# ghar1821/Chronoclust

Hardware: AMD Instinct MI355X
Metric: points clustered/sec (20-dim) (higher is better)
Workload: dtype f64; 1 GPU; C2: 1 timepoint, 1000000x20 synthetic blobs (seed 42+rank), 5000 microclusters; exact sequential semantics; online + offline phases per step; one independent st; points=1000000, dim=20, microclusters=5000, clusters=5000, streams=1

## Files before the change

### chronoclust_amd/_lib.py

```python
import ctypes as C
import os

import numpy as np

from . import build as _build

PCORE, OUTLIER = 0, 1
MAX_DIM = 1024

_ERRORS = {-1: "no HIP device / HIP runtime error", -2: "bad argument", -3: "non-finite input", -4: "out of memory",
           -5: "internal error", -6: "exchange between ranks failed"}


class ChronoclustHipError(RuntimeError):
    pass


class CcParams(C.Structure):
    _fields_ = [("eps_sq", C.c_double), ("delta_sq", C.c_double), ("k", C.c_double), ("beta", C.c_double),
                ("mu", C.c_double), ("omicron", C.c_double), ("ups_eps", C.c_double), ("ups_eps_sq", C.c_double),
                ("delta", C.c_double), ("pi", C.c_int32), ("pad", C.c_int32)]


class CcTuning(C.Structure):
    _fields_ = [("window", C.c_int32), ("rounds", C.c_int32), ("segments", C.c_int32),
                ("windows_per_sync", C.c_int32), ("time_kernels", C.c_int32), ("dirty_segments", C.c_int32),
                ("early_window", C.c_int32), ("lookahead", C.c_int32), ("sequential", C.c_int32)]


class CcStats(C.Structure):
    _fields_ = [("points", C.c_int64), ("windows", C.c_int64), ("rounds", C.c_int64), ("truncated", C.c_int64),
                ("scan_launches", C.c_int64), ("scan_ms", C.c_double), ("scan_pair_dims", C.c_double),
                ("run_ms", C.c_double), ("rows", C.c_int64), ("table_rows_scanned", C.c_int64),
                ("lookahead_windows", C.c_int64), ("sharded_windows", C.c_int64), ("comm_launches", C.c_int64),
                ("comm_ms", C.c_double), ("seq_points", C.c_int64), ("scan_u_launches", C.c_int64),
                ("scan_p_launches", C.c_int64), ("pruned_scan_rows", C.c_int64), ("pruned_scan_full_rows", C.c_int64),
                ("window", C.c_int64), ("long_chains", C.c_int64), ("long_chain_launches", C.c_int64),
                ("tiles", C.c_int64), ("dirty_tiles", C.c_int64),
                ("scan_launches_pruned", C.c_int64), ("scan_ms_pruned", C.c_double), ("scan_pair_dims_pruned", C.c_double),
                ("scan_g_launches", C.c_int64), ("missed_points", C.c_int64), ("probe_launches", C.c_int64),
                ("seq_r_points", C.c_int64), ("heavy_launches", C.c_int64),
                ("scan_lean_launches", C.c_int64), ("long_prepared", C.c_int64), ("long_replayed", C.c_int64),
                ("seq_g_points", C.c_int64), ("link_launches", C.c_int64),
                ("scan_p2_launches", C.c_int64),
                ("calib_allgather_us", C.c_double), ("calib_scan_ns_per_row_dim", C.c_double),
                ("split_threshold_row_dims", C.c_int64), ("split_threshold_row_dims_pruned", C.c_int64),
                ("missed_plain_launches", C.c_int64), ("seed16_launches", C.c_int64),
                ("pad_rows_launches", C.c_int64), ("assign_points", C.c_int64), ("assign_launches", C.c_int64)]


POLICY_MAX_ROUNDS = 8


class CcPolicyConfig(C.Structure):
    _fields_ = [(k, C.c_int32) for k in ("window", "rounds_max", "windows_per_sync", "early_window", "lookahead",
                                         "allow_nodirty", "prune_mode", "prune_applicable", "can_shard", "d", "resume",
                                         "allow_sparse", "allow_guess", "allow_probe")] + \
               [("shard_min_row_dims", C.c_int64), ("n_end", C.c_int64), ("shard_min_row_dims_pruned", C.c_int64),
                ("lookahead_pruned", C.c_int32), ("force_prune_rows", C.c_int32)]


class CcPolicyCarry(C.Structure):
    _fields_ = [(k, C.c_int32) for k in ("adapt_win", "clean_batches", "since_shrink", "pad")]


class CcPolicyObs(C.Structure):
    _fields_ = [("cursor", C.c_int64), ("m_rows", C.c_int32), ("stall_b", C.c_int32)] + \
               [(k, C.c_int64) for k in ("stat_windows", "stat_truncated", "stat_trunc_unknown", "stat_tiles",
                                         "stat_dirty_tiles", "stat_unsafe", "stat_missed")] + \
               [("round_hist", C.c_int64 * (POLICY_MAX_ROUNDS + 2)), ("prune_rows", C.c_uint64), ("prune_full", C.c_uint64),
                ("after_sequential", C.c_int32), ("tg_ok", C.c_int32)]


class CcPolicyDecision(C.Structure):
    _fields_ = [(k, C.c_int32) for k in ("win_cfg", "want", "rounds", "batch_windows", "lookahead", "nodirty", "prune",
                                         "shard", "restart", "bad", "stalled", "sparse", "probe", "pad")] + \
               [(k, C.c_int64) for k in ("wins", "pts", "trunc", "unk", "tiles", "dtiles", "grew", "prune_rows", "prune_full")]


class CcSeqEvent(C.Structure):
    _fields_ = [(k, C.c_int32) for k in ("chunk_event", "bad", "possible", "more", "seq_r_applies", "use_g", "allow_seq_g", "wide")] + \
               [("got", C.c_int64), ("chunk", C.c_int64), ("rate", C.c_double), ("rate_guess", C.c_double)]


class CcBatchInputs(C.Structure):
    _fields_ = [(k, C.c_int32) for k in ("window", "win_cfg", "S_cfg", "n_cus", "prune_now", "prune_wgs_per_cu", "plain_wgs_per_cu",
                                         "decide_threads", "chain_threads", "commit_threads", "allow_claims", "allow_long",
                                         "allow_heavy", "allow_prep", "m_rows", "n_heavy", "long_seen", "long_few")] + \
               [("long_avg", C.c_int64), ("batch_windows", C.c_int32), ("pad", C.c_int32), ("points_left", C.c_int64)]


LONG_NONE, LONG_ROWS_SPLIT, LONG_ROWS_SMALL, LONG_LIST_SPLIT, LONG_LIST_SMALL = range(5)


class CcBatchGeometry(C.Structure):
    _fields_ = [(k, C.c_int32) for k in ("gw", "S", "sparse_cap", "dblocks", "cblocks", "rblocks", "scan_rows", "long_rows",
                                         "long_listed", "heavy_on", "long_cap", "windows_now", "prep", "prep_form", "long_form",
                                         "pad")]


class CcRelaxedStats(C.Structure):
    _fields_ = [("super_steps", C.c_int64), ("minibatch_points", C.c_int64), ("deferred_points", C.c_int64),
                ("reserved", C.c_int64 * 5)]


_dp = C.POINTER(C.c_double)
_i64p = C.POINTER(C.c_int64)
_i32p = C.POINTER(C.c_int32)
_i8p = C.POINTER(C.c_int8)

SYMBOLS = {
    "cc_create": (C.c_int, [C.c_int, C.POINTER(C.c_void_p)]),
    "cc_destroy": (None, [C.c_void_p]),
    "cc_last_error": (C.c_char_p, [C.c_void_p]),
    "cc_set_tuning": (C.c_int, [C.c_void_p, C.POINTER(CcTuning)]),
    "cc_reset": (C.c_int, [C.c_void_p]),
    "cc_set_params": (C.c_int, [C.c_void_p, C.POINTER(CcParams)]),
    "cc_decay_downgrade": (C.c_int, [C.c_void_p, C.c_double]),
    "cc_points_upload": (C.c_int, [C.c_void_p, _dp, C.c_int64, C.c_int32]),
    "cc_points_prefetch": (C.c_int, [C.c_void_p, _dp, C.c_int64, C.c_int32, _dp, _dp]),
    "cc_online_run": (C.c_int, [C.c_void_p]),
    "cc_col_minmax": (C.c_int, [C.c_void_p, _dp, C.c_int64, C.c_int32, _dp, _dp]),
    "cc_points_upload_scaled": (C.c_int, [C.c_void_p, _dp, C.c_int64, C.c_int32, _dp, _dp]),
    "cc_points_download": (C.c_int, [C.c_void_p, _dp, _dp, _dp]),
    "cc_labels_download": (C.c_int, [C.c_void_p, _i64p, _i8p]),
    "cc_online": (C.c_int, [C.c_void_p, _dp, C.c_int64, C.c_int32, _i64p, _i8p]),
    "cc_assign": (C.c_int, [C.c_void_p, _dp, C.c_int64, C.c_int32, _i64p, _i8p, _dp]),
    "cc_count": (C.c_int, [C.c_void_p, C.c_int]),
    "cc_dim": (C.c_int, [C.c_void_p]),
    "cc_counters": (C.c_int, [C.c_void_p, _i64p, _i64p]),
    "cc_set_counters": (C.c_int, [C.c_void_p, C.c_int64, C.c_int64]),
    "cc_export": (C.c_int, [C.c_void_p, C.c_int, _i64p, _i64p, _dp, _dp, _dp, _dp, _dp]),
    "cc_inject_mc": (C.c_int, [C.c_void_p, C.c_int, C.c_int32, _dp, _dp, _dp, _dp, C.c_double, C.c_int64,
                               C.c_int64]),
    "cc_inject_bulk": (C.c_int, [C.c_void_p, C.c_int, C.c_int32, C.c_int32, _dp, _dp, _dp, _dp, _dp, _i64p, _i64p]),
    "cc_offline": (C.c_int, [C.c_void_p, _i32p, _i8p, _i32p, _i32p, _i32p]),
    "cc_num_core": (C.c_int, [C.c_void_p]),
    "cc_cluster_size": (C.c_int, [C.c_void_p, C.c_int32]),
    "cc_cluster_export": (C.c_int, [C.c_void_p, C.c_int32, _i64p, _dp, _dp, _dp, _dp, _dp]),
    "cc_clusters_total_members": (C.c_int, [C.c_void_p]),
    "cc_clusters_export": (C.c_int, [C.c_void_p, _i64p, _i32p, _dp, _dp, _dp, _dp, _dp]),
    "cc_assoc_argmin": (C.c_int, [C.c_void_p, _dp, _dp, C.c_int32, _dp, C.c_int32, C.c_int32, _i32p, _dp]),
    "cc_get_stats": (C.c_int, [C.c_void_p, C.POINTER(CcStats)]),
    "cc_sync": (C.c_int, [C.c_void_p]),
    "cc_policy_replay": (C.c_int, [C.POINTER(CcPolicyConfig), C.POINTER(CcPolicyCarry), C.c_int64, C.c_int32,
                                   C.POINTER(CcPolicyObs), C.c_int32, C.POINTER(CcPolicyDecision)]),
    "cc_point_clusters": (C.c_int, [C.c_void_p, _i32p]),
    "cc_format_points_csv": (C.c_int64, [_dp, C.c_int64, C.c_int32, C.c_int64, _i32p, C.c_char_p, _i32p, C.c_int32,
                                         C.c_void_p, C.c_int64]),
    "cc_comm_unique_id": (C.c_int, [C.c_char_p]),
    "cc_comm_init_rccl": (C.c_int, [C.c_void_p, C.c_char_p, C.c_int, C.c_int]),
    "cc_comm_init_local": (C.c_int, [C.POINTER(C.c_void_p), C.c_int]),
    "cc_comm_calibrate": (C.c_int, [C.c_void_p]),
    "cc_comm_destroy": (C.c_int, [C.c_void_p]),
    "cc_comm_info": (C.c_int, [C.c_void_p, _i32p, _i32p, _i32p]),
    "cc_comm_set_relaxed": (C.c_int, [C.c_void_p, C.c_int32]),
    "cc_get_relaxed_stats": (C.c_int, [C.c_void_p, C.POINTER(CcRelaxedStats)]),
    "cc_policy_seq_rate_guess": (C.c_double, [C.c_int32, C.c_int32, C.c_int32, C.c_int32]),
    "cc_seq_handover_replay": (C.c_int, [C.c_int32, C.c_int32, C.c_int32, C.POINTER(CcSeqEvent), C.c_int32, _i32p, _i64p]),
    "cc_batch_plan": (C.c_int, [C.POINTER(CcBatchInputs), C.POINTER(CcBatchGeometry)]),
    "cc_scan_width": (C.c_int, [C.c_int32, C.c_int32, C.c_int32, _i32p, _i32p, _i32p]),
    "cc_shard_rows": (C.c_int, [C.c_int32, C.c_int32, C.c_int32, C.c_int32, _i32p, _i32p]),
    "cc_set_shard_thresholds": (C.c_int, [C.c_void_p, C.c_int64, C.c_int32]),
}

COMM_ID_BYTES = 128

_lib = None


def load():
    global _lib
    if _lib is None:
        path = os.environ.get("CHRONOCLUST_HIP_LIB") or _build.LIB_PATH
        if not os.path.exists(path):
            raise ChronoclustHipError(
                "HIP library %s not built; run `python -m chronoclust_amd.build` (needs hipcc). "
                "chronoclust_amd has no CPU fallback." % path)
        if _build.is_stale(path) and os.environ.get("CHRONOCLUST_HIP_ALLOW_STALE") != "1":
            raise ChronoclustHipError(
                "HIP library %s was not built from the sources beside it (csrc/ or include/chronoclust_hip.h changed since, or "
                "its .sha256 stamp is missing); run `python -m chronoclust_amd.build`." % path)
        lib = C.CDLL(path)
        for name, (res, args) in SYMBOLS.items():
            fn = getattr(lib, name)
            fn.restype = res
            fn.argtypes = args
        _lib = lib
    return _lib


HOST_ONLY_SYMBOLS = ("cc_policy_replay", "cc_policy_seq_rate_guess", "cc_seq_handover_replay", "cc_batch_plan", "cc_shard_rows",
                     "cc_format_points_csv", "cc_scan_width")


def load_host_only(path):
    global _lib
    lib = C.CDLL(path)
    for name in HOST_ONLY_SYMBOLS:
        fn = getattr(lib, name)
        fn.restype, fn.argtypes = SYMBOLS[name]
    _lib = lib
    return lib


def _f64(a):
    return np.ascontiguousarray(np.asarray(a, dtype=np.float64))


def _ptr(a, typ=_dp):
    return None if a is None else a.ctypes.data_as(typ)


def comm_unique_id():
    buf = C.create_string_buffer(COMM_ID_BYTES)
    rc = load().cc_comm_unique_id(buf)
    if rc != 0:
        raise ChronoclustHipError("cc_comm_unique_id failed (%s): is librccl available?" % _ERRORS.get(rc, rc))
    return buf.raw


def comm_init_local(handles):
    arr = (C.c_void_p * len(handles))(*[h._h for h in handles])
    rc = load().cc_comm_init_local(arr, len(handles))
    if rc != 0:
        raise ChronoclustHipError("cc_comm_init_local failed: %s" % _ERRORS.get(rc, rc))


def format_points_csv(values, first_id, label_idx, labels, threads=8, chunk=65536, out=None):
    from concurrent.futures import ThreadPoolExecutor
    lib = load()
    values = _f64(values)
    if values.ndim != 2:
        raise ValueError("values must be a [n, d] array, got shape %r" % (values.shape,))
    n, d = values.shape
    label_idx = np.ascontiguousarray(label_idx, dtype=np.int32)
    if label_idx.shape != (n,):
        raise ValueError("label_idx must hold one entry per row: shape %r for %d rows" % (label_idx.shape, n))
    if len(labels) < 1:
        raise ValueError("labels must not be empty")
    enc = [s.encode() for s in labels]
    offs = np.zeros(len(enc) + 1, np.int32)
    offs[1:] = np.cumsum([len(e) for e in enc])
    blob = b"".join(enc)
    per_row = 25 + max(len(e) for e in enc) + 33 * d + 2

    def work(a):
        b = min(n, a + chunk)
        buf = np.empty(per_row * (b - a), np.uint8)
        got = lib.cc_format_points_csv(values[a:b].ctypes.data_as(_dp), b - a, d, first_id + a,
                                       label_idx[a:b].ctypes.data_as(_i32p), blob, offs.ctypes.data_as(_i32p), len(enc),
                                       buf.ctypes.data, buf.size)
        if got < 0:
            raise ChronoclustHipError("cc_format_points_csv failed: %s" % _ERRORS.get(got, got))
        return memoryview(buf)[:got]

    if n == 0:
        return 0 if out is not None else b""
    starts = list(range(0, n, chunk))
    workers = max(1, threads)
    with ThreadPoolExecutor(max_workers=workers) as ex:
        if out is None:
            return b"".join(ex.map(work, starts))
        total, pending, nxt = 0, [], 0
        while nxt < len(starts) or pending:
            while nxt < len(starts) and len(pending) < 2 * workers:
                pending.append(ex.submit(work, starts[nxt]))
                nxt += 1
            part = pending.pop(0).result()
            out.write(part)
            total += len(part)
        return total


def policy_replay(config, carry, start, observations):
    cfg = CcPolicyConfig(**{k: int(v) for k, v in config.items()})
    car = CcPolicyCarry(int(carry[0]), int(carry[1]), int(carry[2]), 0)
    n = len(observations)
    obs = (CcPolicyObs * max(n, 1))()
    for i, o in enumerate(observations):
        for k, v in o.items():
            if k == "round_hist":
                for r, x in enumerate(v):
                    obs[i].round_hist[r] = int(x)
            else:
                setattr(obs[i], k, int(v))
    out = (CcPolicyDecision * (n + 1))()
    rc = load().cc_policy_replay(C.byref(cfg), C.byref(car), int(start[0]), int(start[1]), obs, n, out)
    if rc != 0:
        raise ValueError("cc_policy_replay: %s" % _ERRORS.get(rc, rc))
    keys = [k for k, _ in CcPolicyDecision._fields_ if k != "pad"]
    return [{k: getattr(d, k) for k in keys} for d in out], (car.adapt_win, car.clean_batches, car.since_shrink)


def seq_handover_replay(mode, possible, sticky, events):
    n = len(events)
    ev = (CcSeqEvent * max(n, 1))(*[CcSeqEvent(**e) for e in events])
    out, stint = (C.c_int32 * (n + 1))(), (C.c_int64 * (n + 1))()
    rc = load().cc_seq_handover_replay(int(mode), int(possible), int(sticky), ev, n, out, stint)
    if rc != 0:
        raise ValueError("cc_seq_handover_replay: %s" % _ERRORS.get(rc, rc))
    return list(out), list(stint)


def batch_plan(**inputs):
    out = CcBatchGeometry()
    rc = load().cc_batch_plan(C.byref(CcBatchInputs(**inputs)), C.byref(out))
    if rc != 0:
        raise ValueError("cc_batch_plan(%r): %s" % (inputs, _ERRORS.get(rc, rc)))
    return {k: getattr(out, k) for k, _ in CcBatchGeometry._fields_ if k != "pad"}


SCAN_CHAINS = ("none", "common", "general")


def scan_width(d, filter_on, k_pow2):
    padded, scan_u, chain = C.c_int32(), C.c_int32(), C.c_int32()
    rc = load().cc_scan_width(int(d), int(bool(filter_on)), int(bool(k_pow2)), C.byref(padded), C.byref(scan_u), C.byref(chain))
    if rc != 0:
        raise ValueError("cc_scan_width(%r, %r, %r): %s" % (d, filter_on, k_pow2, _ERRORS.get(rc, rc)))
    return padded.value, bool(scan_u.value), SCAN_CHAINS[chain.value]


def shard_rows(n, world, rank, unit=1):
    lo, hi = C.c_int32(), C.c_int32()
    rc = load().cc_shard_rows(int(n), int(world), int(rank), int(unit), C.byref(lo), C.byref(hi))
    if rc != 0:
        raise ValueError("cc_shard_rows(%r, %r, %r, %r): %s" % (n, world, rank, unit, _ERRORS.get(rc, rc)))
    return lo.value, hi.value


class Handle(object):

    def __init__(self, device=0):
        self._lib = load()
        h = C.c_void_p()
        rc = self._lib.cc_create(int(device), C.byref(h))
        if rc != 0:
            raise ChronoclustHipError("cc_create(device=%d) failed: %s. chronoclust_amd needs an MI355X-class HIP "
                                      "device; there is no CPU fallback." % (device, _ERRORS.get(rc, rc)))
        self._h = h
        self.device = device
        self._prefetched = None

    def close(self):
        if getattr(self, "_h", None):
            self._lib.cc_destroy(self._h)
            self._h = None

    def __del__(self):
        try:
            self.close()
        except Exception:
            pass

    def _check(self, rc):
        if rc < 0:
            msg = self._lib.cc_last_error(self._h)
            exc = ValueError if rc in (-2, -3) else ChronoclustHipError
            raise exc("%s: %s" % (_ERRORS.get(rc, rc), msg.decode() if msg else ""))
        return rc

    def set_tuning(self, window=0, rounds=0, segments=0, windows_per_sync=0, time_kernels=0, dirty_segments=0,
                   lookahead=0, early_window=0, sequential=0):
        t = CcTuning(window, rounds, segments, windows_per_sync, time_kernels, dirty_segments, int(early_window),
                     int(lookahead), int(sequential))
        self._check(self._lib.cc_set_tuning(self._h, C.byref(t)))

    def reset(self):
        self._check(self._lib.cc_reset(self._h))

    def set_params(self, eps_sq, delta_sq, k, beta, mu, omicron, ups_eps, ups_eps_sq, delta, pi):
        p = CcParams(eps_sq, delta_sq, k, beta, mu, omicron, ups_eps, ups_eps_sq, delta, int(pi), 0)
        self._check(self._lib.cc_set_params(self._h, C.byref(p)))

    def decay_downgrade(self, factor):
        self._check(self._lib.cc_decay_downgrade(self._h, float(factor)))

    def points_upload(self, x):
        x = _f64(x)
        if x.ndim != 2:
            raise ValueError("points must be a 2-d array")
        try:
            self._check(self._lib.cc_points_upload(self._h, _ptr(x), x.shape[0], x.shape[1]))
        finally:
            self._prefetched = None
        self._n = x.shape[0]

    def points_prefetch(self, x, scale=None, min_=None):
        if not (isinstance(x, np.ndarray) and x.dtype == np.float64 and x.flags["C_CONTIGUOUS"] and x.ndim == 2):
            raise ValueError("points_prefetch needs a C-contiguous float64 [n, d] array (it is not copied)")
        if x.shape[0] == 0:
            return
        scale = None if scale is None else _f64(scale)
        min_ = None if min_ is None else _f64(min_)
        self._prefetched = (x, scale, min_)
        self._check(self._lib.cc_points_prefetch(self._h, _ptr(x), x.shape[0], x.shape[1], _ptr(scale), _ptr(min_)))

    def col_minmax(self, x):
        x = _f64(x)
        mn = np.empty(x.shape[1], dtype=np.float64)
        mx = np.empty(x.shape[1], dtype=np.float64)
        self._check(self._lib.cc_col_minmax(self._h, _ptr(x), x.shape[0], x.shape[1], _ptr(mn), _ptr(mx)))
        return mn, mx

    def points_upload_scaled(self, x, scale, min_):
        x, scale, min_ = _f64(x), _f64(scale), _f64(min_)
        if x.ndim != 2 or scale.shape != (x.shape[1],) or min_.shape != (x.shape[1],):
            raise ValueError("points must be [n, d], scale and min_ [d]")
        try:
            self._check(self._lib.cc_points_upload_scaled(self._h, _ptr(x), x.shape[0], x.shape[1], _ptr(scale),
                                                          _ptr(min_)))
        finally:
            self._prefetched = None
        self._n = x.shape[0]

    def points_download(self, d, scale=None, min_=None):
        out = np.empty((self._n, d), dtype=np.float64)
        if scale is None:
            self._check(self._lib.cc_points_download(self._h, _ptr(out), None, None))
        else:
            scale, min_ = _f64(scale), _f64(min_)
            self._check(self._lib.cc_points_download(self._h, _ptr(out), _ptr(scale), _ptr(min_)))
        return out

    def online_run(self):
        self._check(self._lib.cc_online_run(self._h))

    def labels_download(self, want_path=True):
        uid = np.empty(self._n, dtype=np.int64)
        path = np.empty(self._n, dtype=np.int8) if want_path else None
        self._check(self._lib.cc_labels_download(self._h, _ptr(uid, _i64p), _ptr(path, _i8p)))
        return uid, path

    def online(self, x):
        self.points_upload(x)
        self.online_run()
        return self.labels_download()

    def assign(self, x, want_path=True, want_dist=False):
        x = _f64(x)
        if x.ndim != 2:
            raise ValueError("points must be a 2-d array")
        n = x.shape[0]
        uid = np.empty(n, dtype=np.int64)
        path = np.empty(n, dtype=np.int8) if want_path else None
        dist = np.empty(n, dtype=np.float64) if want_dist else None
        self._check(self._lib.cc_assign(self._h, _ptr(x), n, x.shape[1], _ptr(uid, _i64p), _ptr(path, _i8p), _ptr(dist)))
        return uid, path, dist

    def count(self, kind):
        return self._check(self._lib.cc_count(self._h, kind))

    def dim(self):
        return self._check(self._lib.cc_dim(self._h))

    def counters(self):
        a, b = C.c_int64(), C.c_int64()
        self._check(self._lib.cc_counters(self._h, C.byref(a), C.byref(b)))
        return a.value, b.value

    def set_counters(self, pcore_last_id, outlier_last_id):
        self._check(self._lib.cc_set_counters(self._h, int(pcore_last_id), int(outlier_last_id)))

    def export(self, kind):
        n, d = self.count(kind), self.dim()
        out = dict(id=np.empty(n, np.int64), uid=np.empty(n, np.int64), w=np.empty(n, np.float64),
                   cf1=np.empty((n, d)), cf2=np.empty((n, d)), cen=np.empty((n, d)), pref=np.empty((n, d)))
        self._check(self._lib.cc_export(self._h, kind, _ptr(out["id"], _i64p), _ptr(out["uid"], _i64p), _ptr(out["w"]),
                                        _ptr(out["cf1"]), _ptr(out["cf2"]), _ptr(out["cen"]), _ptr(out["pref"])))
        return out

    def inject(self, kind, cf1, cf2, cen, pref, w, id, uid):
        cf1, cf2, cen, pref = _f64(cf1), _f64(cf2), _f64(cen), _f64(pref)
        self._check(self._lib.cc_inject_mc(self._h, kind, len(cf1), _ptr(cf1), _ptr(cf2), _ptr(cen), _ptr(pref),
                                           float(w), int(id), int(uid)))
# ... 95 lines not shown
```

### chronoclust_amd/csrc/cc_batch.h

```cpp
#pragma once
#include <algorithm>
#include <cmath>
#include <cstdint>

#include "../../include/chronoclust_hip.h"

namespace cc {

using BatchInputs = cc_batch_inputs;
using BatchPlan = cc_batch_geometry;

constexpr int kMaxWindow = 49152;
constexpr int kLongCap = 512;

constexpr int kScanWidths[8] = {4, 8, 14, 16, 20, 32, 40, 64};
struct ScanWidth {
    int padded = 0;
    bool scan_u = false;
    int chain = CC_CHAIN_NONE;
};
inline ScanWidth scan_width(int d, bool filter, bool pow2)
{
    ScanWidth w;
    w.padded = kScanWidths[7];
    for (int i = 7; i >= 0; --i)
        if (d <= kScanWidths[i]) w.padded = kScanWidths[i];
    const bool compiled = d == w.padded, common = !filter && pow2;
    w.scan_u = common && (compiled || (d > 8 && d < w.padded));
    if (w.scan_u && w.padded > 8) w.chain = CC_CHAIN_COMMON;
    else if (!common && compiled && w.padded > 8 && w.padded <= 40) w.chain = CC_CHAIN_GENERAL;
    return w;
}

inline int scan_partials_for(int tiles, int S, int resident)
{
    int best = S;
    double best_eff = 0.0;
    for (int s = S; s >= std::max(1, S / 2); --s) {
        const double x = (double)tiles * s / (double)resident;
        const double eff = x / std::ceil(x);
        if (eff > best_eff + 1e-9) { best_eff = eff; best = s; }
    }
    return best;
}

inline BatchPlan batch_plan(const BatchInputs& in)
{
    BatchPlan p{};
    const int gw = p.gw = std::max(64, std::min(in.window, in.win_cfg));
    p.S = in.prune_now ? std::max(1, std::min(in.S_cfg, (in.n_cus * in.prune_wgs_per_cu) / std::max(1, (gw + 63) / 64)))
                       : scan_partials_for((gw + 63) / 64, in.S_cfg, in.n_cus * in.plain_wgs_per_cu);
    p.sparse_cap = std::min(kMaxWindow / 16, std::max(64, ((gw / 16 + 63) / 64) * 64));
    p.dblocks = (gw + in.decide_threads / 32 - 1) / (in.decide_threads / 32);
    p.cblocks = (gw + in.chain_threads / 32 - 1) / (in.chain_threads / 32);
    p.rblocks = std::min((gw + in.commit_threads / 32 - 1) / (in.commit_threads / 32), 1024 * (256 / in.commit_threads));
    p.scan_rows = (in.allow_claims && in.m_rows > 0 && in.m_rows <= 1024) ? in.m_rows : 0;
    p.long_rows = in.allow_long ? p.scan_rows : 0;
    p.long_listed = (in.allow_long && p.scan_rows == 0 && in.long_seen) ? 1 : 0;
    p.heavy_on = (in.allow_heavy && p.scan_rows == 0 && in.n_heavy > 0) ? 1 : 0;
    p.long_cap = in.long_few ? (int)std::min<long long>(kLongCap, 2 * in.long_avg + 8) : kLongCap;
    const long long w = std::max(1, in.win_cfg);
    p.windows_now = (int)std::max<long long>(1, std::min<long long>(in.batch_windows, (in.points_left + w - 1) / w));
    p.prep = (in.allow_prep && ((p.long_rows > 0 && p.long_rows <= 64) || (p.long_listed && in.long_few))) ? 1 : 0;
    p.prep_form = !p.prep ? CC_LONG_NONE : p.long_rows > 0 ? CC_LONG_ROWS_SPLIT : CC_LONG_LIST_SPLIT;
    p.long_form = p.long_rows > 0 ? (p.long_rows <= 256 ? CC_LONG_ROWS_SPLIT : CC_LONG_ROWS_SMALL)
                  : p.long_listed ? (in.long_few ? CC_LONG_LIST_SPLIT : CC_LONG_LIST_SMALL)
                                  : CC_LONG_NONE;
    return p;
}

struct LongChains {
    long long prev = 0;
    long long rounds_prev = 0;
    bool seen = false;
    bool few = true;
    long long avg = 1;

    void after_batch(long long stat_long, long long stat_rounds)
    {
        seen = stat_long > prev;
        avg = (stat_long - prev) / std::max<long long>(1, stat_rounds - rounds_prev) + 1;
        few = avg <= 64;
        prev = stat_long;
        rounds_prev = stat_rounds;
    }
};

inline bool link_after_batch(bool allowed, long long rows_created, long long points)
{
    return allowed && rows_created * 256 >= std::max<long long>(1, points);
}

}
```

### chronoclust_amd/csrc/cc_handle.h

```cpp
#pragma once
#include "cc_knobs.h"

namespace {

struct HipErr {
    hipError_t e;
    const char* what;
};

#define HIPCHK(call)                                  \
    do {                                              \
        hipError_t _e = (call);                       \
        if (_e != hipSuccess) throw HipErr{_e, #call}; \
    } while (0)

template <typename T>
struct DevBuf {
    T* p = nullptr;
    size_t n = 0;
    void ensure(size_t count)
    {
        if (count <= n && p) return;
        release();
        size_t want = std::max<size_t>(count, 1);
// ... 283 lines not shown
{
    f();
}
template <typename F, typename... Rest>
void with_bools(F&& f, bool b, Rest... rest)
{
    if (b) with_bools([&](auto... c) { f(std::true_type{}, c...); }, rest...);
    else with_bools([&](auto... c) { f(std::false_type{}, c...); }, rest...);
}

struct CapacityErr {
    std::string what;
};

int fail(cc_handle* h, int code, const std::string& msg)
{
    if (h) h->err = msg;
    return code;
}

void group_lost(cc_handle* h)
{
    if (h && h->comm.active()) h->comm.fail_group();
}

template <typename F>
int guarded(cc_handle* h, F&& f)
{
    try {
        if (h) HIPCHK(hipSetDevice(h->device));
        const int rc = f();
        if (rc < 0) group_lost(h);
        return rc;
    } catch (const HipErr& e) {
        char buf[512];
        snprintf(buf, sizeof buf, "HIP error %d (%s) in %s", (int)e.e, hipGetErrorString(e.e), e.what);
        group_lost(h);
        return fail(h, e.e == hipErrorOutOfMemory ? CC_ERR_OOM : CC_ERR_NO_DEVICE, buf);
    } catch (const cc::CommErr& e) {
        group_lost(h);
        return fail(h, CC_ERR_COMM, "exchange between ranks failed: " + e.what);
    } catch (const std::bad_alloc&) {
        group_lost(h);
        return fail(h, CC_ERR_OOM, "host allocation failed");
    } catch (const CapacityErr& e) {
        group_lost(h);
        return fail(h, CC_ERR_OOM, e.what);
    }
}

void sync_stream(cc_handle* h, hipStream_t st)
{
    if (h->comm.rccl() || h->comm.broken) h->comm.wait_stream(st);
    else HIPCHK(hipStreamSynchronize(st));
}

bool is_pow2(double k)
{
    if (!(k > 0.0) || !std::isfinite(k)) return false;
    int e;
    double m = std::frexp(k, &e);
    return m == 0.5 && e > -1000 && e < 1000;
}

void refresh_ctl_params(cc_handle* h)
{
    Ctl& c = h->hc;
    const cc_params& p = h->par;
    c.eps_sq = p.eps_sq;
    c.delta_sq = p.delta_sq;
    c.k = p.k;
    c.pow2 = (is_pow2(p.k) && !h->tainted) ? 1 : 0;
    c.inv_k = c.pow2 ? 1.0 / p.k : 0.0;
    c.beta_mu = p.beta * p.mu;
    c.mu = p.mu;
    c.omicron = p.omicron;
    c.pi = p.pi;
    c.filter = (h->d > 0 && p.pi < h->d) ? 1 : 0;
    c.d = h->d;
}

void push_ctl(cc_handle* h)
{
    memset(h->hc.pstat, 0, sizeof(h->hc.pstat));
    h->hc.n_missed_all[0] = h->hc.n_missed_all[1] = 0;
    HIPCHK(hipMemcpyAsync(h->ctl.p, &h->hc, sizeof(Ctl), hipMemcpyHostToDevice, h->stream));
}
void pull_ctl(cc_handle* h)
{
    HIPCHK(hipMemcpyAsync(&h->hc, h->ctl.p, sizeof(Ctl), hipMemcpyDeviceToHost, h->stream));
    sync_stream(h, h->stream);
}
void pull_ctl_pinned(cc_handle* h)
{
    if (!h->hc_pin) { pull_ctl(h); return; }
    HIPCHK(hipMemcpyAsync(h->hc_pin, h->ctl.p, sizeof(Ctl), hipMemcpyDeviceToHost, h->stream));
    sync_stream(h, h->stream);
    memcpy(&h->hc, h->hc_pin, sizeof(Ctl));
}
void push_ctl_pinned(cc_handle* h)
{
    if (!h->hc_pin) { push_ctl(h); return; }
    memset(h->hc.pstat, 0, sizeof(h->hc.pstat));
    h->hc.n_missed_all[0] = h->hc.n_missed_all[1] = 0;
    memcpy(h->hc_pin + 1, &h->hc, sizeof(Ctl));
    HIPCHK(hipMemcpyAsync(h->ctl.p, h->hc_pin + 1, sizeof(Ctl), hipMemcpyHostToDevice, h->stream));
}

#define CC_MAX_TABLE_ELEMS ((size_t)INT_MAX - 1023)

void ensure_table(cc_handle* h, size_t rows)
{
    if (h->tab.cap >= rows && h->tab.d == h->d) return;
    const size_t max_rows = CC_MAX_TABLE_ELEMS / (size_t)std::max(h->d, 1);
    if (rows > max_rows)
        throw CapacityErr{"a table of " + std::to_string(rows) + " rows of " + std::to_string(h->d) + " dimensions: more than " +
                          std::to_string(max_rows) + " rows (" + std::to_string(CC_MAX_TABLE_ELEMS) + " elements) at this width"};
    size_t want = std::min(max_rows, std::max<size_t>(rows, std::max<size_t>(1024, h->tab.cap * 2)));
    TableStore nt;
    nt.alloc(want, h->d);
    const size_t m = (size_t)h->hc.m_rows;
    TableStore& old = h->tab;
    TableStore::for_each_column(h->d, [&](auto col, size_t per_row, TableStore::Grow grow) {
        auto& to = nt.*col;
        const size_t elem = sizeof(*to.p);
        if (grow == TableStore::CLEARED || grow == TableStore::CLEARED_KEPT)
            HIPCHK(hipMemsetAsync(to.p, 0, want * per_row * elem, h->stream));
        if ((grow == TableStore::KEPT || grow == TableStore::CLEARED_KEPT) && m > 0)
            HIPCHK(hipMemcpyAsync(to.p, (old.*col).p, m * per_row * elem, hipMemcpyDeviceToDevice, h->stream));
    });
    sync_stream(h, h->stream);
    std::swap(h->tab, nt);
}

int set_dim(cc_handle* h, int d)
{
    if (d <= 0 || d > CC_MAX_DIM) return fail(h, CC_ERR_BAD_ARG, "d must be in 1.." + std::to_string(CC_MAX_DIM));
    if (h->d == 0) h->d = d;
    if (h->d != d) {
        if (h->hc.m_rows == 0) h->d = d;
        else return fail(h, CC_ERR_BAD_ARG, "dimensionality differs from the microclusters already held");
    }
    return CC_OK;
}

void ensure_window_buffers(cc_handle* h, int win, int seg)
{
    if (win <= h->win_alloc && seg <= h->seg_alloc && h->d <= h->d_alloc) return;
    win = std::max(win, h->win_alloc);
    seg = std::max(seg, h->seg_alloc);
    const size_t w = (size_t)win, d = (size_t)std::max(h->d, h->d_alloc);
    h->v_cf1.ensure(w * d); h->v_cf2.ensure(w * d); h->v_cen.ensure(w * d); h->v_pref.ensure(w * d); h->v_scl.ensure(w * d); h->v_w.ensure(w);
    h->v_kind.ensure(w); h->v_key.ensure(w); h->v_next.ensure(w); h->v_upg.ensure(w); h->v_acc.ensure(w);
    h->v_dsq.ensure(w); h->v_tau.ensure(CC_TAU_STRIDE * w); h->v_tile_dsq.ensure(CC_DSQ_STRIDE * (w / 16 + 2));
    h->v_tgt.ensure(w);
    h->v_skip.ensure(w / 64 + 2); h->v_skip_car.ensure(w / 64 + 2); h->v_unsafe.ensure(w);
    h->part_stride = w * seg * 4;
    h->spart_stride = w * seg * 2;
    h->thr_stride = w * 2;
    h->spart.ensure(2 * h->spart_stride);
    h->thr.ensure(2 * h->thr_stride);
    h->thr32.ensure(2 * h->thr_stride);
    h->cmax.ensure(2);
    h->found.ensure(2 * (CC_MAX_WINDOW / 64));
    h->missed.ensure(2 * CC_MISSED_CAP);
    h->part.ensure(2 * h->part_stride); h->dpart.ensure(w * seg * 2); h->dpart2.ensure(w * seg * 2);
    h->clean.ensure(w * 4); h->dseed.ensure(w * 4);
    h->c_cf1v.ensure(w * d); h->c_cf2v.ensure(w * d); h->c_cenv.ensure(w * d); h->c_prefv.ensure(w * d);
    h->c_sclv.ensure(w * d); h->c_wv.ensure(w); h->c_c0.ensure(w * d); h->c_w0.ensure(w * d);
    h->c_kind.ensure(w); h->c_key.ensure(w); h->c_slot.ensure(w); h->c_kind0.ensure(w); h->c_dsq.ensure(w); h->c_tile_dsq.ensure(CC_DSQ_STRIDE * (w / 16 + 2));
    h->T0.ensure(w + 128); h->T1.ensure(w + 128);
    h->long_list.ensure(2 * CC_LONG_CAP);
    h->lstat.ensure(2 * CC_LSTAT_ROWS + 2);
    h->lprev.ensure(CC_MAX_WINDOW);
    h->dpath.ensure(w); h->rk.ensure(w); h->rec.ensure(1); h->sp_list.ensure(w); h->link_near.ensure(w);
    h->win_alloc = win; h->seg_alloc = seg; h->d_alloc = (int)d;
}

Carry carry_view(cc_handle* h)
{
    return Carry{h->c_cf1v.p, h->c_cf2v.p, h->c_cenv.p, h->c_prefv.p, h->c_sclv.p, h->c_wv.p, h->c_kind.p, h->c_key.p,
                 h->c_slot.p, h->c_c0.p, h->c_w0.p, h->c_kind0.p, h->c_dsq.p, h->c_tile_dsq.p};
}

void scan_copy_sync(cc_handle* h, ScanCopy (&out)[2])
{
    const size_t cap = h->tab.cap, d = (size_t)h->d, m = (size_t)h->hc.m_rows;
    const bool filter = h->hc.filter != 0;
    const TableStore& t = h->tab;
    for (int q = 0; q < 2; ++q) {
        h->sh_cen[q].ensure(cap * d); h->sh_scl[q].ensure(cap * d); h->sh_kind[q].ensure(cap); h->sh_key[q].ensure(cap);
        if (filter) { h->sh_cf1[q].ensure(cap * d); h->sh_cf2[q].ensure(cap * d); h->sh_w[q].ensure(cap); }
        if (m > 0) {
            HIPCHK(hipMemcpyAsync(h->sh_cen[q].p, t.cen.p, m * d * 8, hipMemcpyDeviceToDevice, h->stream));
            HIPCHK(hipMemcpyAsync(h->sh_scl[q].p, t.scl.p, m * d * 8, hipMemcpyDeviceToDevice, h->stream));
            HIPCHK(hipMemcpyAsync(h->sh_kind[q].p, t.kind.p, m * 4, hipMemcpyDeviceToDevice, h->stream));
            HIPCHK(hipMemcpyAsync(h->sh_key[q].p, t.key.p, m * 4, hipMemcpyDeviceToDevice, h->stream));
            if (filter) {
                HIPCHK(hipMemcpyAsync(h->sh_cf1[q].p, t.cf1.p, m * d * 8, hipMemcpyDeviceToDevice, h->stream));
                HIPCHK(hipMemcpyAsync(h->sh_cf2[q].p, t.cf2.p, m * d * 8, hipMemcpyDeviceToDevice, h->stream));
                HIPCHK(hipMemcpyAsync(h->sh_w[q].p, t.w.p, m * 8, hipMemcpyDeviceToDevice, h->stream));
            }
        }
        out[q] = ScanCopy{h->sh_cen[q].p, h->sh_scl[q].p, h->sh_cf1[q].p, h->sh_cf2[q].p, h->sh_w[q].p, h->sh_kind[q].p,
                          h->sh_key[q].p};
    }
}

Versions versions_view(cc_handle* h)
{
    return Versions{h->v_cf1.p, h->v_cf2.p, h->v_cen.p, h->v_pref.p, h->v_scl.p, h->v_w.p, h->v_kind.p,
                    h->v_key.p, h->v_next.p, h->v_upg.p, h->v_acc.p, h->v_tgt.p, h->v_dsq.p, h->v_tile_dsq.p,
                    h->v_tau.p, h->v_skip.p, h->v_skip_car.p, h->v_unsafe.p};
}

void ensure_prefix16(cc_handle* h)
{
    const size_t a16_rows = h->tab.cap + 2 * CC_P16_TM;
    if (h->a16_stride >= a16_rows * 4) return;
    sync_stream(h, h->stream);
    sync_stream(h, h->stream2);
    h->a16.ensure(2 * a16_rows * 4);
    h->a16_stride = a16_rows * 4;
    h->hdr16.ensure(2);
}

void ensure_pad_rows(cc_handle* h, int dp)
{
    const size_t stride = (h->tab.cap + CC_SCAN_TM) * (size_t)dp;
    if (h->pad_stride >= stride) return;
    sync_stream(h, h->stream);
    sync_stream(h, h->stream2);
    h->pad_cen.ensure(2 * stride);
    h->pad_scl.ensure(2 * stride);
    h->pad_stride = stride;
}

hipEvent_t get_event(cc_handle* h, size_t i)
{
    while (h->ev_pool.size() <= i) {
        hipEvent_t e;
        HIPCHK(hipEventCreateWithFlags(&e, h->light_sync_events ? hipEventReleaseToDevice : hipEventDefault));
        h->ev_pool.push_back(e);
    }
    return h->ev_pool[i];
}

hipEvent_t get_sync_event(cc_handle* h, size_t i)
{
    if (!h->light_sync_events) return get_event(h, i);
    while (h->sync_pool.size() <= i) {
        hipEvent_t e;
        HIPCHK(hipEventCreateWithFlags(&e, hipEventDisableTiming | hipEventReleaseToDevice));
        h->sync_pool.push_back(e);
    }
    return h->sync_pool[i];
}


}
```

### chronoclust_amd/csrc/cc_host.h

```cpp
#pragma once
#include <stdint.h>

#if defined(__HIPCC__) || defined(__HIP__)
#define CC_HOSTDEV __host__ __device__
#else
#define CC_HOSTDEV
#endif

CC_HOSTDEV inline int cc_shard_share(int n, int world, int unit)
{
    const long long units = ((long long)n + unit - 1) / unit;
    const long long share = ((units + world - 1) / world) * unit;
    return (int)(share < 0x7fffffffLL ? share : 0x7fffffffLL);
}
CC_HOSTDEV inline void cc_shard_range(int n, int world, int rank, int unit, int* lo, int* hi)
{
    const int share = cc_shard_share(n, world, unit);
    const long long a = (long long)rank * share;
    *lo = (int)(a < n ? a : n);
    const long long b = a + share;
    *hi = (int)(b < n ? b : n);
}

#define CC_SEQ_DOUBLES 6600
CC_HOSTDEV inline int cc_seq_cap_rows(int d) { return CC_SEQ_DOUBLES / (4 * d + 5); }
```

### chronoclust_amd/csrc/cc_host_abi.inc

```

int cc_shard_rows(int32_t n, int32_t world, int32_t rank, int32_t unit, int32_t* lo, int32_t* hi)
{
    if (n < 0 || world < 1 || rank < 0 || rank >= world || unit < 1 || !lo || !hi) return CC_ERR_BAD_ARG;
    int a = 0, b = 0;
    cc_shard_range(n, world, rank, unit, &a, &b);
    *lo = a;
    *hi = b;
    return CC_OK;
}

int64_t cc_format_points_csv(const double* values, int64_t n, int32_t d, int64_t first_id, const int32_t* label_idx,
                             const char* label_bytes, const int32_t* label_offsets, int32_t n_labels, char* out,
                             int64_t cap)
{
    if (!values || n < 0 || d < 0 || !label_idx || !label_bytes || !label_offsets || n_labels < 1 || !out) return CC_ERR_BAD_ARG;
    char* o = out;
    char* const end = out + cap;
    int max_label = 0;
    for (int i = 0; i < n_labels; ++i) max_label = std::max(max_label, label_offsets[i + 1] - label_offsets[i]);
    const int64_t row_max = 24 + 1 + max_label + (int64_t)d * 33 + 2;
    for (int64_t r = 0; r < n; ++r) {
        if (end - o < row_max) return CC_ERR_OOM;
        o += cc::format_i64(first_id + r, o);
        *o++ = ',';
        int li = label_idx[r];
        if (li < 0 || li >= n_labels) li = n_labels - 1;
        const int ll = label_offsets[li + 1] - label_offsets[li];
        memcpy(o, label_bytes + label_offsets[li], (size_t)ll);
        o += ll;
        const double* v = values + r * d;
        for (int i = 0; i < d; ++i) {
            *o++ = ',';
            if (v[i] == v[i]) o += cc::format_repr(v[i], o);
        }
        *o++ = '\n';
    }
    return (int64_t)(o - out);
}

int cc_policy_replay(const cc_policy_config* cfg, cc_policy_carry* carry, int64_t start_cursor, int32_t start_rows,
                     const cc_policy_obs* obs, int32_t n, cc_policy_decision* out)
{
    if (!cfg || !carry || n < 0 || (n > 0 && !obs) || !out) return CC_ERR_BAD_ARG;
    cc::WindowPolicy policy(*cfg, *carry);
    out[0] = policy.start(start_cursor, start_rows);
    for (int i = 0; i < n; ++i)
        out[i + 1] = obs[i].after_sequential ? policy.after_sequential(obs[i].cursor, obs[i].m_rows) : policy.after_batch(obs[i]);
    *carry = policy.carry();
    return CC_OK;
}

double cc_policy_seq_rate_guess(int32_t d, int32_t m_rows, int32_t allow_seq_r, int32_t allow_seq_g)
{
    if (d < 1 || d > CC_MAX_DIM || m_rows < 0) return -1.0;
    const int seq_cap = d > CC_WINDOW_MAX_DIM ? 0 : cc_seq_cap_rows(d);
    return cc::seq_rate_guess(d, m_rows, seq_cap, allow_seq_r != 0, allow_seq_g != 0);
}

int cc_seq_handover_replay(int32_t mode, int32_t possible, int32_t sticky, const cc_seq_event* ev, int32_t n, int32_t* outcome,
                           int64_t* stint_len)
{
    if (mode < 0 || mode > 2 || n < 0 || (n > 0 && !ev) || !outcome || !stint_len) return CC_ERR_BAD_ARG;
    cc::SeqHandover rule;
    outcome[0] = rule.start(mode, possible != 0, sticky != 0) ? 1 : 0;
    stint_len[0] = rule.stint_len();
    for (int i = 0; i < n; ++i) {
        const cc_seq_event& e = ev[i];
        outcome[i + 1] = e.chunk_event
                             ? (int32_t)rule.after_chunk(e.got, e.rate, e.chunk, e.use_g != 0, e.allow_seq_g != 0, e.possible != 0,
                                                         e.more != 0, e.wide != 0)
                             : (rule.after_batch(e.bad != 0, e.rate, e.possible != 0, e.more != 0, e.seq_r_applies != 0, e.rate_guess) ? 1 : 0);
        stint_len[i + 1] = rule.stint_len();
    }
    return CC_OK;
}

int cc_batch_plan(const cc_batch_inputs* in, cc_batch_geometry* out)
{
    if (!in || !out) return CC_ERR_BAD_ARG;
    for (int t : {in->decide_threads, in->chain_threads, in->commit_threads})
        if (t != 64 && t != 128 && t != 256) return CC_ERR_BAD_ARG;
    if (in->window < 1 || in->win_cfg < 0 || in->S_cfg < 1 || in->n_cus < 1 || in->prune_wgs_per_cu < 1 || in->plain_wgs_per_cu < 1 ||
        in->m_rows < 0 || in->long_avg < 0 || in->points_left < 0)
        return CC_ERR_BAD_ARG;
    *out = cc::batch_plan(*in);
    return CC_OK;
}

int cc_scan_width(int32_t d, int32_t filter_on, int32_t k_pow2, int32_t* padded, int32_t* scan_u, int32_t* chain)
{
    if (d < 1 || d > CC_MAX_DIM || !padded || !scan_u || !chain) return CC_ERR_BAD_ARG;
    const cc::ScanWidth w = cc::scan_width(d, filter_on != 0, k_pow2 != 0);
    *padded = w.padded;
    *scan_u = w.scan_u ? 1 : 0;
    *chain = w.chain;
    return CC_OK;
}
```

### chronoclust_amd/csrc/cc_online_run.h

```cpp
#pragma once

namespace {

struct PolicyTrace {
    FILE* f = nullptr;
    static void obs_json(FILE* f, const cc_policy_obs& o)
    {
        fprintf(f, "{\"cursor\": %lld, \"m_rows\": %d, \"stall_b\": %d, \"stat_windows\": %lld, \"stat_truncated\": %lld, "
                   "\"stat_trunc_unknown\": %lld, \"stat_tiles\": %lld, \"stat_dirty_tiles\": %lld, \"stat_unsafe\": %lld, \"stat_missed\": %lld, \"tg_ok\": %d, \"round_hist\": [",
                (long long)o.cursor, o.m_rows, o.stall_b, (long long)o.stat_windows, (long long)o.stat_truncated,
                (long long)o.stat_trunc_unknown, (long long)o.stat_tiles, (long long)o.stat_dirty_tiles, (long long)o.stat_unsafe,
                (long long)o.stat_missed, o.tg_ok);
        for (int r = 0; r < CC_POLICY_MAX_ROUNDS + 2; ++r) fprintf(f, "%s%lld", r ? ", " : "", (long long)o.round_hist[r]);
        fprintf(f, "], \"prune_rows\": %llu, \"prune_full\": %llu, \"after_sequential\": %d}", (unsigned long long)o.prune_rows,
                (unsigned long long)o.prune_full, o.after_sequential);
    }
    static void dec_json(FILE* f, const cc_policy_decision& d)
    {
        fprintf(f, "{\"win_cfg\": %d, \"want\": %d, \"rounds\": %d, \"batch_windows\": %d, \"lookahead\": %d, \"nodirty\": %d, "
                   "\"prune\": %d, \"shard\": %d, \"restart\": %d, \"bad\": %d, \"stalled\": %d, \"sparse\": %d, \"probe\": %d}",
                d.win_cfg, d.want, d.rounds, d.batch_windows, d.lookahead, d.nodirty, d.prune, d.shard, d.restart, d.bad, d.stalled, d.sparse, d.probe);
    }
    PolicyTrace(const cc_policy_config& c, const cc_policy_carry& k, long long cursor, int rows, const cc_policy_decision& d0,
                int rank)
    {
        const char* path = getenv("CHRONOCLUST_HIP_POLICY_TRACE");
        if (!path || !path[0]) return;
        const std::string name = rank >= 0 ? std::string(path) + ".rank" + std::to_string(rank) : std::string(path);
        f = fopen(name.c_str(), "a");
        if (!f) return;
        fprintf(f, "{\"call\": {\"config\": {\"window\": %d, \"rounds_max\": %d, \"windows_per_sync\": %d, \"early_window\": %d, "
                   "\"lookahead\": %d, \"allow_nodirty\": %d, \"prune_mode\": %d, \"prune_applicable\": %d, \"can_shard\": %d, \"d\": %d, "
                   "\"resume\": %d, \"allow_sparse\": %d, \"allow_guess\": %d, \"allow_probe\": %d, \"shard_min_row_dims\": %lld, \"n_end\": %lld, \"shard_min_row_dims_pruned\": %lld, \"lookahead_pruned\": %d, \"force_prune_rows\": %d}, \"carry\": [%d, %d, %d], \"start\": [%lld, %d], \"dec\": ",
                c.window, c.rounds_max, c.windows_per_sync, c.early_window, c.lookahead, c.allow_nodirty, c.prune_mode,
                c.prune_applicable, c.can_shard, c.d, c.resume, c.allow_sparse, c.allow_guess, c.allow_probe, (long long)c.shard_min_row_dims, (long long)c.n_end, (long long)c.shard_min_row_dims_pruned, c.lookahead_pruned, c.force_prune_rows,
                k.adapt_win, k.clean_batches, k.since_shrink, cursor, rows);
        dec_json(f, d0);
        fprintf(f, "}}\n");
    }
    void batch(const cc_policy_obs& o, const cc_policy_decision& d)
    {
        if (!f) return;
        fprintf(f, "{\"obs\": ");
        obs_json(f, o);
        fprintf(f, ", \"dec\": ");
        dec_json(f, d);
        fprintf(f, "}\n");
    }
    void sequential(long long cursor, int rows, const cc_policy_decision& d)
    {
        cc_policy_obs o{};
        o.cursor = cursor;
        o.m_rows = rows;
        o.after_sequential = 1;
        batch(o, d);
    }
    ~PolicyTrace()
    {
        if (f) fclose(f);
    }
    PolicyTrace(const PolicyTrace&) = delete;
    PolicyTrace& operator=(const PolicyTrace&) = delete;
};

void launch_link_scan(cc_handle* h, hipStream_t st, int win)
{
    const dim3 grid((win + 63) / 64, (win + 4 * CC_LINK_SUB - 1) / (4 * CC_LINK_SUB)), block(256);
    const int d = h->d;
#define CC_LINK_DP(DP) hipLaunchKernelGGL((k_link_scan<DP>), grid, block, 0, st, (const Ctl*)h->ctl.p, (const double*)h->X.p, \
                                          (const double*)h->Xt.p, (const int*)h->T0.p, h->link_near.p)
    if (d <= 4) CC_LINK_DP(4);
    else if (d <= 8) CC_LINK_DP(8);
    else if (d <= 14) CC_LINK_DP(14);
    else if (d <= 16) CC_LINK_DP(16);
    else if (d <= 20) CC_LINK_DP(20);
    else if (d <= 32) CC_LINK_DP(32);
    else if (d <= 40) CC_LINK_DP(40);
    else CC_LINK_DP(64);
#undef CC_LINK_DP
}

static_assert(cc::kMaxWindow == CC_MAX_WINDOW && cc::kLongCap == CC_LONG_CAP, "cc_batch.h repeats two constants of cc_common.h");

Rows rows_of_table(const Table& t)
{
    Rows r{};
    r.cen = t.cen; r.scl = t.scl; r.pref = t.pref; r.cf1 = t.cf1; r.cf2 = t.cf2; r.w = t.w; r.kind = t.kind; r.key = t.key;
    return r;
}
Rows rows_of_versions(const Versions& v)
{
    Rows r{};
    r.cen = v.cen; r.scl = v.scl; r.pref = v.pref; r.cf1 = v.cf1; r.cf2 = v.cf2; r.w = v.w; r.kind = v.kind; r.key = v.key;
    r.next = v.next; r.tile_dsq = v.tile_dsq; r.dsq = v.dsq; r.tau = v.tau; r.skip = v.skip;
    return r;
}
Rows rows_of_carry(const Carry& c, const Versions& v, const Table& t)
{
    Rows r{};
    r.cen = c.cen; r.scl = c.scl; r.pref = c.pref; r.cf1 = c.cf1; r.cf2 = c.cf2; r.w = c.w; r.kind = c.kind; r.key = c.key;
    r.tile_dsq = c.tile_dsq; r.dsq = c.dsq; r.tau = v.tau; r.skip = v.skip_car;
    r.slot = c.slot; r.touch = t.touch; r.cap = t.cap;
    return r;
}
Rows rows_of_scan_copy(const ScanCopy& s)
{
    Rows r{};
    r.cen = s.cen; r.scl = s.scl; r.cf1 = s.cf1; r.cf2 = s.cf2; r.w = s.w; r.kind = s.kind; r.key = s.key;
    return r;
}
Rows sparse_rows(Rows r, const int* plist)
{
    r.skip = nullptr;
    r.plist = plist;
    return r;
}

void reset_call_counters(Ctl& c)
{
    c.last_round = 0;
    c.fc[0] = 0;
    for (int i = 1; i < CC_MAX_ROUNDS + 2; ++i) c.fc[i] = CC_IDX_INF;
    c.stat_windows = c.stat_rounds = c.stat_truncated = 0;
    c.stat_lookahead = 0;
    c.stat_tiles = c.stat_dirty_tiles = 0;
    c.stat_unprovable = c.stat_unsafe = 0;
    c.stat_long = 0;
    for (int i = 0; i < CC_MAX_ROUNDS + 2; ++i) c.n_long[i] = 0;
    c.stat_trunc_unknown = 0;
    c.stat_table_rows = 0;
    c.stat_seq_points = 0;
    c.stat_seq_r_points = 0;
#ifdef CC_LONG_TIMERS
    for (int i = 0; i < 8; ++i) c.dbg_long[i] = 0;
#endif
#ifdef CC_ROUND_DEBUG
    for (int i = 0; i < CC_MAX_ROUNDS + 2; ++i)
        for (int q = 0; q < 6; ++q) c.dbg_round[i][q] = 0;
#endif
    c.n_heavy = c.n_heavy_new = 0;
    c.stat_seq_clk = c.stat_seq_wall = 0;
    c.stat_prune_rows = c.stat_prune_full = 0;
    c.stat_missed = 0;
    c.seed_at = -1;
    for (int q = 0; q < 2; ++q) {
        c.n_missed[q] = 0;
        for (int K = 0; K < 2; ++K) { c.tg[q][K] = 0.0; c.tg_ok[q][K] = 0; }
    }
    c.cen_absmax = 0ull;
    c.stat_pair_rows = 0.0;
    for (int i = 0; i < CC_MAX_ROUNDS + 2; ++i) c.round_hist[i] = 0;
}

struct OnlineRun {
    cc_handle* const h;
    const long long range_a, N;
    const bool no_create, resume;
    Ctl& c;

    int win = 0, R = 0;
    int S_cfg = 1, Sd_full = 1, Sd = 1;
    int world = 1, myrank = 0;
    bool grouped = false;
    size_t batch_max = 2;
    bool timing = false;
    int seq_cap = 0;
    Versions ver{};
    Carry car{};
    hipStream_t sA = nullptr, sB = nullptr;
    static constexpr size_t ev_base = 4;

    std::optional<cc::WindowPolicy> policy;
    std::optional<PolicyTrace> ptrace;
    cc_policy_decision dec{};
    bool nodirty = false;
    bool sparse_now = false;
    bool la_on = false;
    bool shard_on = false;
    bool link_now = false;
    int Rcur = 1;
    int batch_windows = 2;

    long long done = 0;
    int m_known = 0;
    unsigned long long seq_host = 0;
    long long cursor_prev = 0;
    double batch_t0 = 0.0;

    hipEvent_t ev0 = nullptr, ev1 = nullptr, evCommit = nullptr, evScan = nullptr;
    size_t ev_used = 2, ev_sync = ev_base;
    std::vector<std::pair<size_t, double>> timed;
    std::vector<size_t> timed_comm;
    double pair_rows_eff = 0.0, pair_rows_prev = 0.0;
    double pair_rows_pruned = 0.0;
    long long sharded_windows = 0;

    cc::SeqHandover seq;
    cc::LongChains longs;
    long long long_launches = 0;

    cc::BatchPlan bp{};
    Table tab{};
    Rows trows{}, vrows{}, crows{}, vrows_sp{}, crows_sp{}, srows[2] = {};
    ScanCopy scopy[2] = {};
    int* long_list = nullptr;
    int probe_left = 0;
    hipEvent_t scan_end = nullptr;

    OnlineRun(cc_handle* handle, long long a, long long e, bool no_create_, bool resume_)
        : h(handle), range_a(a), N(e), no_create(no_create_), resume(resume_), c(handle->hc) {}

    static double now_ms()
    {
        return std::chrono::duration<double, std::milli>(std::chrono::steady_clock::now().time_since_epoch()).count();
    }
    bool seq_r_applies() const { return h->allow_seq_r && h->d >= 2 && h->d <= 4; }
    bool wide() const { return h->d > CC_WINDOW_MAX_DIM; }
    size_t window_rows() const { return wide() ? 0 : (size_t)win * batch_max; }
    bool seq_g_applies() const { return h->allow_seq_g && h->hc.m_rows >= seq_cap; }
    double seq_rate_guess() const { return cc::seq_rate_guess(h->d, h->hc.m_rows, seq_cap, h->allow_seq_r, h->allow_seq_g); }
    bool seq_possible() const { return !h->comm.active() && !no_create && (h->hc.m_rows < seq_cap || h->allow_seq_g); }

    void set_lookahead(bool on)
    {
        la_on = on;
        c.la_on = on ? 1 : 0;
        c.stall_b = 0;
        c.mode = 0;
        c.car_n = 0;
        const int q = (int)((c.window_seq + 1ull) & 1ull);
        const long long c1 = c.cursor + c.win_b;
        const long long left1 = c.n_points - c1;
        c.la_cursor[q] = c1;
        c.la_b[q] = (on && left1 > 0) ? (int)std::min<long long>(left1, c.win_cfg) : 0;
        c.la_rows[q] = c.m_rows;
// ... 161 lines not shown
        in.prune_now = h->prune_now ? 1 : 0;
        in.decide_threads = h->decide_threads; in.chain_threads = h->chain_threads; in.commit_threads = h->commit_threads;
        in.allow_claims = h->allow_claims ? 1 : 0; in.allow_long = h->allow_long ? 1 : 0;
        in.allow_heavy = h->allow_heavy ? 1 : 0; in.allow_prep = h->allow_prep ? 1 : 0;
        in.m_rows = h->hc.m_rows; in.n_heavy = h->hc.n_heavy;
        in.long_seen = longs.seen ? 1 : 0; in.long_few = longs.few ? 1 : 0; in.long_avg = longs.avg;
        return in;
    }


    int* claims_of(int round) const { return (round & 1) ? h->T1.p : h->T0.p; }
    const ScanCopy& sc_now() const { return scopy[seq_host & 1ull]; }
    int quiet_ok() const { return h->allow_quiet ? 1 : 0; }
    bool sparse_round() const { return nodirty && sparse_now; }

    void exchange_missed(hipStream_t st, const Rows& rws, int mode, int round, int q, int srank, int sworld)
    {
        launch_scan<false>(h, st, bp.gw, rws, nullptr, h->part.p, bp.S, round, mode, srank, sworld, 1);
        Cand* const send2 = h->gsend2.p + (size_t)q * CC_MISSED_CAP * 4;
        Cand* const recv2 = h->gpart2.p + (size_t)q * sworld * CC_MISSED_CAP * 4;
        hipLaunchKernelGGL(k_merge_partials, dim3((CC_MISSED_CAP + 255) / 256), dim3(256), 0, st, h->ctl.p,
                           h->part.p, h->part_stride, bp.S, send2, (size_t)0, round, mode,
                           (const unsigned long long*)nullptr, 0, (const int*)h->missed.p);
        h->comm.all_gather(send2, recv2, (size_t)CC_MISSED_CAP * 4 * sizeof(Cand), st, st == h->stream2 ? 1 : 0);
        hipLaunchKernelGGL(k_scatter_missed, dim3((CC_MISSED_CAP * sworld + 255) / 256), dim3(256), 0, st,
                           (const Ctl*)h->ctl.p, (const int*)h->missed.p, (const Cand*)recv2, sworld,
                           h->gpart.p, h->gpart_stride, (size_t)bp.gw * 4 + 4, round, mode);
    }

    void snapshot_scan(hipStream_t st, int mode, int round)
    {
        const int gw = bp.gw, S = bp.S;
        const int q = (mode == 1) ? (round & 1) : (int)(seq_host & 1ull);
        const Rows& src = (mode == 1) ? srows[round & 1] : trows;
        const Rows rws = h->scan_plan.pad_rows ? padded_rows(h, st, src, q, round, mode) : src;
        h->probe_now = probe_left > 0 && !h->prune_now;
        if (h->probe_now) --probe_left;
        const int srank = shard_on ? myrank : 0, sworld = shard_on ? world : 1;
        h->group_guess_now = shard_on && (sworld > 1 || h->group_guess_always);
        scan_end = nullptr;
        if (timing) {
            hipEvent_t a = get_event(h, ev_used), b = get_event(h, ev_used + 1);
            HIPCHK(hipEventRecord(a, st));
            launch_scan<false>(h, st, gw, rws, nullptr, h->part.p, S, round, mode, srank, sworld);
            HIPCHK(hipEventRecord(b, st));
            timed.push_back({ev_used, h->prune_now ? 1.0 : 0.0});
            ev_used += 2;
            if (!shard_on) scan_end = b;
        } else {
            launch_scan<false>(h, st, gw, rws, nullptr, h->part.p, S, round, mode, srank, sworld);
        }
        if (!shard_on) return;
        if (timing) HIPCHK(hipEventRecord(get_event(h, ev_used), st));
        hipLaunchKernelGGL(k_merge_partials, dim3((gw + 255) / 256), dim3(256), 0, st, h->ctl.p, h->part.p,
                           h->part_stride, S, h->gsend.p, h->gsend_stride, round, mode,
                           (const unsigned long long*)h->pstat_p(), gw * 4,
                           (const int*)nullptr);
        h->comm.all_gather(h->gsend.p + (size_t)q * h->gsend_stride, h->gpart.p + (size_t)q * h->gpart_stride,
                           ((size_t)gw * 4 + 4) * sizeof(Cand), st, st == h->stream2 ? 1 : 0);
        if (h->prune_now && h->guess_now && h->group_guess_now && h->lean_now) ++h->stats.scan_lean_launches;
        if (h->prune_now && h->guess_now && h->group_guess_now && !h->lean_now) exchange_missed(st, rws, mode, round, q, srank, sworld);
        if (timing) {
            HIPCHK(hipEventRecord(get_event(h, ev_used + 1), st));
            timed_comm.push_back(ev_used);
            ev_used += 2;
        }
    }

    void launch_snapshot_scans(bool first_window)
    {
        if (!la_on) return snapshot_scan(sA, 0, 0);
        if (evScan) HIPCHK(hipStreamWaitEvent(sA, evScan, 0));
        HIPCHK(hipStreamWaitEvent(sB, evCommit, 0));
        snapshot_scan(sB, 1, (int)((seq_host + 1ull) & 1ull));
        if (scan_end) evScan = scan_end;
        else {
            evScan = get_sync_event(h, ev_sync++);
            HIPCHK(hipEventRecord(evScan, sB));
        }
        if (first_window && h->hc.mode == 0) snapshot_scan(sA, 0, 0);
    }

    void launch_decide(int round)
    {
        const bool first = round == 0;
        const Cand* const dec_part = shard_on ? h->gpart.p : h->part.p;
        const size_t dec_stride = shard_on ? h->gpart_stride : h->part_stride;
        const int dec_S = shard_on ? world : bp.S, dec_inner = shard_on ? 1 : bp.S;
        const size_t dec_outer = shard_on ? (size_t)bp.gw * 4 + 4 : 0;
        const int dec_tail = (first && shard_on) ? bp.gw * 4 : -1;
        const int ac_blocks = (first && la_on) ? bp.rblocks : 0;
        const int dirty_mode = (first || !nodirty) ? 0 : (sparse_round() ? 2 : 1);
        const int group = (h->d <= 32 && h->decide_group == 16) ? 16 : 32;
        const int per_wg = h->decide_threads / group;
        const dim3 grid((bp.gw + per_wg - 1) / per_wg + ac_blocks);
        hipLaunchKernelGGL(group == 16 ? k_decide<16> : k_decide<32>, grid, dim3(h->decide_threads), 0, sA, h->ctl.p, h->X.p, tab, ver, car,
                           dec_part, dec_stride, h->clean.p, h->dpart.p, h->dpart2.p, h->dseed.p,
                           first ? (const int*)nullptr : (const int*)claims_of(round - 1), claims_of(round), h->dpath.p, dec_S, Sd,
                           round, dirty_mode, bp.scan_rows, dec_inner, dec_outer,
                           first ? (const CommitRec*)h->rec.p : (const CommitRec*)nullptr, first ? sc_now() : ScanCopy{}, ac_blocks,
                           long_list, bp.long_cap, dec_tail, (!first && round == Rcur) ? 1 : 0, bp.heavy_on ? 1 : 0,
                           first ? 0 : quiet_ok(), (first && link_now) ? h->link_near.p : (int*)nullptr);
    }

    void launch_link()
    {
        launch_link_scan(h, sA, bp.gw);
        hipLaunchKernelGGL(k_link_apply, dim3((bp.gw + 255) / 256), dim3(256), 0, sA, h->ctl.p, tab, h->T0.p,
                           (const int*)h->link_near.p, h->dpath.p);
        ++h->stats.link_launches;
    }

    void launch_claims(int round)
    {
        if (bp.scan_rows > 0)
            hipLaunchKernelGGL(k_claims, dim3(bp.scan_rows), dim3(256), 0, sA, h->ctl.p, tab, (const int*)claims_of(round), round,
                               bp.scan_rows, round ? quiet_ok() : 0);
    }
    void launch_claims_heavy(int round)
    {
        if (!bp.heavy_on) return;
        ++h->stats.heavy_launches;
        hipLaunchKernelGGL(k_claims_heavy, dim3(CC_HEAVY_CAP), dim3(256), 0, sA, h->ctl.p, tab, (const int*)claims_of(round), round,
                           long_list, bp.long_cap, round ? quiet_ok() : 0);
    }

    void launch_chain_long(int form, bool prep_kernel, int round)
    {
        if (form == CC_LONG_NONE) return;
        const bool by_list = form == CC_LONG_LIST_SPLIT || form == CC_LONG_LIST_SMALL;
        const bool split = form == CC_LONG_ROWS_SPLIT || form == CC_LONG_LIST_SPLIT;
        if (prep_kernel) h->prep_launched = true;
        else if (by_list) ++long_launches;
        auto launch = [&](auto kernel) {
            hipLaunchKernelGGL(kernel, dim3(by_list ? bp.long_cap : bp.long_rows), dim3(split ? CC_LONG_THREADS : 256), 0, sA, h->ctl.p,
                               h->X.p, tab, ver, car, (const int*)claims_of(round - 1), round, by_list ? 0 : bp.long_rows,
                               by_list ? (const int*)long_list : (const int*)nullptr, bp.prep ? h->lstat.p : nullptr,
                               bp.prep ? h->lprev.p : nullptr);
        };
        if (prep_kernel) launch(k_chain_long<true, true>);
        else if (split) launch(k_chain_long<true, false>);
        else launch(k_chain_long<false, false>);
    }

    void launch_chain(int round)
    {
        hipLaunchKernelGGL(k_chain, dim3(bp.cblocks), dim3(h->chain_threads), 0, sA, h->ctl.p, h->X.p, tab, ver, car,
                           (const int*)claims_of(round - 1), round, bp.long_rows, (const unsigned long long*)(bp.prep ? h->lprev.p : nullptr),
                           bp.prep ? h->lstat.p : nullptr);
    }

    void launch_dseed(int round)
    {
        hipLaunchKernelGGL(k_dseed, dim3((bp.gw + 63) / 64), dim3(64), 0, sA, h->ctl.p, h->X.p, tab, ver, car,
                           h->clean.p, h->dseed.p, (const int*)claims_of(round - 1), round, (const int8_t*)h->dpath.p, h->sp_list.p,
                           sparse_round() ? bp.sparse_cap : 0);
    }

    void launch_dirty_scans(int round)
    {
        if (nodirty && !sparse_round()) return;
        const bool sp = nodirty;
        const int pts = sp ? bp.sparse_cap : bp.gw;
        launch_scan<true>(h, sA, pts, sp ? vrows_sp : vrows, h->dseed.p, h->dpart.p, Sd, round, 0);
        if (la_on) launch_scan<true>(h, sA, pts, sp ? crows_sp : crows, h->dseed.p, h->dpart2.p, Sd, round, 1);
    }

    void launch_commit()
    {
        hipLaunchKernelGGL(k_commit_a, dim3(1), dim3(1024), 0, sA, h->ctl.p, tab, ver, car, h->T0.p, h->T1.p,
                           h->rk.p, h->rec.p, (const Cand*)h->clean.p, (const int8_t*)h->dpath.p);
        hipLaunchKernelGGL(k_commit_b, dim3(bp.rblocks), dim3(h->commit_threads), 0, sA, h->rec.p, tab, ver, car, h->rk.p, h->dpath.p,
                           h->lab_uid.p, h->lab_path.p, h->d, sc_now(), h->hc.filter);
    }

    void enqueue_batch()
    {
        batch_t0 = now_ms();
        bp = cc::batch_plan(batch_inputs());
        trows = rows_of_table(tab);
        vrows = rows_of_versions(ver);
        crows = rows_of_carry(car, ver, tab);
        vrows_sp = sparse_rows(vrows, h->sp_list.p);
        crows_sp = sparse_rows(crows, h->sp_list.p);
        long_list = bp.long_listed ? h->long_list.p : nullptr;
        ev_sync = ev_base;
        scopy[0] = scopy[1] = ScanCopy{};
        if (la_on) scan_copy_sync(h, scopy);
        for (int q = 0; q < 2; ++q) srows[q] = rows_of_scan_copy(scopy[q]);
        evScan = nullptr;
        if (la_on) HIPCHK(hipEventRecord(evCommit, sA));
        probe_left = (dec.probe != 0) ? 1 : 0;
        for (int wv = 0; wv < bp.windows_now; ++wv, ++seq_host) {
            launch_snapshot_scans(wv == 0);
            launch_decide(0);
            if (link_now) launch_link();
            launch_claims(0);
            launch_claims_heavy(0);
            for (int r = 1; r <= Rcur; ++r) {
                if (bp.prep) launch_chain_long(bp.prep_form, true, r);
                launch_chain(r);
                launch_chain_long(bp.long_form, false, r);
                launch_dseed(r);
                launch_dirty_scans(r);
                launch_decide(r);
                if (r < Rcur) {
                    launch_claims(r);
                    launch_claims_heavy(r);
                }
            }
            launch_commit();
            if (la_on) {
                evCommit = get_sync_event(h, ev_sync++);
                HIPCHK(hipEventRecord(evCommit, sA));
            }
        }
    }

    int after_batch()
    {
        HIPCHK(hipGetLastError());
        pull_ctl_pinned(h);
        if (la_on) sync_stream(h, sB);
        seq_host = h->hc.window_seq;
        done = h->hc.cursor;
        const double dt = now_ms() - batch_t0;
        const long long pts_b = h->hc.cursor - cursor_prev;
        link_now = cc::link_after_batch(h->allow_link && !no_create, h->hc.m_rows - m_known, pts_b);
        m_known = h->hc.m_rows;
        cursor_prev = h->hc.cursor;
        longs.after_batch(h->hc.stat_long, h->hc.stat_rounds);
        const bool shard_was = shard_on;
        cc_policy_obs o{};
        o.cursor = h->hc.cursor;
        o.m_rows = h->hc.m_rows;
        o.stall_b = h->hc.stall_b;
        o.stat_windows = h->hc.stat_windows;
        o.stat_truncated = h->hc.stat_truncated;
        o.stat_trunc_unknown = h->hc.stat_trunc_unknown;
        o.stat_tiles = h->hc.stat_tiles;
        o.stat_dirty_tiles = h->hc.stat_dirty_tiles;
        o.stat_unsafe = h->hc.stat_unsafe;
        o.stat_missed = h->hc.stat_missed;
        o.tg_ok = (h->hc.tg_ok[0][0] != 0 && h->hc.tg_ok[1][0] != 0) ? 1 : 0;
        for (int r = 0; r < CC_MAX_ROUNDS + 2; ++r) o.round_hist[r] = h->hc.round_hist[r];
        o.prune_rows = h->hc.stat_prune_rows;
        o.prune_full = h->hc.stat_prune_full;
        dec = policy->after_batch(o);
        ptrace->batch(o, dec);
        const cc_policy_carry& k = policy->carry();
        h->adapt_win = k.adapt_win; h->clean_batches = k.clean_batches; h->since_shrink = k.since_shrink;
        if (dec.stalled)
            return fail(h, CC_ERR_INTERNAL, "the online phase made no progress in five consecutive batches of windows");
        if (h->trace && dec.prune_rows > 0)
            fprintf(stderr, "[cc] pruned scans of the batch%s (sample): %lld (wave, row) pairs, %.1f %% evaluated in full; points missed by guessed thresholds so far: %lld\n",
                    h->guess_now ? ", guessed thresholds" : "", (long long)dec.prune_rows,
                    100.0 * (double)dec.prune_full / (double)dec.prune_rows, (long long)h->hc.stat_missed);
        pair_rows_eff += (h->hc.stat_pair_rows - pair_rows_prev) / (shard_was ? (double)world : 1.0);
        if (h->prune_now) pair_rows_pruned += (h->hc.stat_pair_rows - pair_rows_prev) / (shard_was ? (double)world : 1.0);
        pair_rows_prev = h->hc.stat_pair_rows;
        if (shard_was) sharded_windows += dec.wins;
        Rcur = dec.rounds;
        Sd = Sd_full;
        nodirty = dec.nodirty != 0;
        sparse_now = dec.sparse != 0;
        shard_on = dec.shard != 0;
        h->set_prune(dec.prune);
        if (dec.restart) {
            h->hc.win_cfg = dec.win_cfg;
            h->hc.win_b = (int)std::min<long long>(dec.win_cfg, N - done);
            set_lookahead(dec.lookahead != 0);
            push_ctl_pinned(h);
        }
#ifdef CC_ROUND_DEBUG
        for (int r = 1; r <= CC_MAX_ROUNDS; ++r)
            if (h->hc.dbg_round[r][5] != 0)
                fprintf(stderr, "[cc]    round %d so far: %llu decisions, %llu refused, create->join new %llu, create->join row %llu, join->create %llu, other MC %llu | windows ended in round %d: %lld\n",
                        r, h->hc.dbg_round[r][5], h->hc.dbg_round[r][0], h->hc.dbg_round[r][1], h->hc.dbg_round[r][2], h->hc.dbg_round[r][3],
                        h->hc.dbg_round[r][4], r, (long long)h->hc.round_hist[r]);
#endif
        if (h->trace)
            fprintf(stderr, "[cc] %.2f ms done %lld rows %d | batch: %lld windows %lld points trunc %lld (%lld at an undecidable point) lookahead %lld dirty tiles %lld / %lld (points so far: %lld unlocated, %lld unsafe) | next window %d rounds %d\n",
                    now_ms() - batch_t0, done, h->hc.m_rows, (long long)dec.wins, (long long)dec.pts, (long long)dec.trunc, (long long)dec.unk, (long long)h->hc.stat_lookahead, (long long)dec.dtiles, (long long)dec.tiles,
                    (long long)h->hc.stat_unprovable, (long long)h->hc.stat_unsafe, dec.want, Rcur);
        batch_windows = dec.batch_windows;
        seq.after_batch(dec.bad != 0, pts_b > 0 ? (double)pts_b / std::max(dt, 1e-3) : 0.0, seq_possible(), done < N, seq_r_applies(),
                        seq_rate_guess());
        return (int)CC_OK;
    }

    void finish()
    {
        HIPCHK(hipEventRecord(ev1, h->stream));
        HIPCHK(hipEventSynchronize(ev1));
        float ms = 0.f;
        HIPCHK(hipEventElapsedTime(&ms, ev0, ev1));
        h->stats.run_ms += ms;
        h->stats.points += N - range_a;
        h->stats.windows += h->hc.stat_windows;
        h->stats.rounds += h->hc.stat_rounds;
        h->stats.truncated += h->hc.stat_truncated;
        h->stats.rows = h->hc.m_rows;
        h->stats.scan_pair_dims += pair_rows_eff * (double)h->d;
        h->stats.scan_pair_dims_pruned += pair_rows_pruned * (double)h->d;
        h->stats.sharded_windows += sharded_windows;
        h->stats.seq_points += h->hc.stat_seq_points;
        h->stats.seq_r_points += h->hc.stat_seq_r_points;
// ... 82 lines not shown
```

### chronoclust_amd/csrc/cc_validate.h

```cpp
#pragma once


#define CC_LSTAT_ROWS 1024

template <int GW = 32>
__device__ __forceinline__ unsigned cc_group_ballot(bool p)
{
    static_assert(GW == 16 || GW == 32, "groups of 16 or 32 lanes");
    const unsigned long long b = __builtin_amdgcn_ballot_w64(p);
    return (unsigned)(b >> (threadIdx.x & (64 - GW))) & (GW == 32 ? 0xFFFFFFFFu : 0xFFFFu);
}

template <int CTRL>
__device__ __forceinline__ double cc_dpp_f64(double x)
{
    int lo = __double2loint(x), hi = __double2hiint(x);
    lo = __builtin_amdgcn_update_dpp(0, lo, CTRL, 0xF, 0xF, false);
    hi = __builtin_amdgcn_update_dpp(0, hi, CTRL, 0xF, 0xF, false);
    return __hiloint2double(hi, lo);
}
__device__ __forceinline__ double cc_group_sum_any_order(double x)
{
    x += cc_dpp_f64<0xB1>(x);
    x += cc_dpp_f64<0x4E>(x);
    x += cc_dpp_f64<0x141>(x);
    x += cc_dpp_f64<0x140>(x);
    const int lo = __double2loint(x), hi = __double2hiint(x);
    const double r16 = __hiloint2double(__builtin_amdgcn_readlane(hi, 16), __builtin_amdgcn_readlane(lo, 16));
    const double r48 = __hiloint2double(__builtin_amdgcn_readlane(hi, 48), __builtin_amdgcn_readlane(lo, 48));
    return x + ((threadIdx.x & 32) ? r48 : r16);
}

struct GroupAdd {
    double c1[2], c2[2], pr[2];
    double cen[2];
    double r2;
    int gt1, ne1;
};

template <int GW = 32>
__device__ inline GroupAdd cc_group_add_regs(const double (&b1)[2], const double (&b2)[2], double bw,
                                             const double (&px)[2], int d, const Par& c)
{
    const int gl = threadIdx.x & (GW - 1);
    GroupAdd g;
    const double w1 = bw + 1.0;
    double term[2];
    bool gt[2], ne[2];
#pragma unroll
    for (int h = 0; h < 2; ++h) {
        const int i = gl + GW * h;
        g.c1[h] = 0.0; g.c2[h] = 0.0; g.pr[h] = 1.0; g.cen[h] = 0.0;
        term[h] = 0.0; gt[h] = false; ne[h] = false;
        if (i < d) {
            const double x = px[h];
            g.c1[h] = b1[h] + x;
            g.c2[h] = b2[h] + x * x;
            const double qa = g.c2[h] / w1;
            const double qb = g.c1[h] / w1;
            g.cen[h] = qb;
            const double var = qa - qb * qb;
            const double pr = (var <= c.delta_sq) ? c.k : 1.0;
            g.pr[h] = pr;
            term[h] = cc_div_pref(var, pr, c);
            gt[h] = pr > 1.0;
            ne[h] = pr != 1.0;
        }
    }
    g.gt1 = __builtin_popcount(cc_group_ballot<GW>(gt[0])) + __builtin_popcount(cc_group_ballot<GW>(gt[1]));
    g.ne1 = __builtin_popcount(cc_group_ballot<GW>(ne[0])) + __builtin_popcount(cc_group_ballot<GW>(ne[1]));
    __shared__ double s_term[(CC_GROUP_THREADS / GW)][2 * GW];
    double* const row = s_term[(threadIdx.x / GW) % (CC_GROUP_THREADS / GW)];
    CC_WAVE_SYNC();
    row[gl] = term[0];
    row[gl + GW] = term[1];
    CC_WAVE_SYNC();
    double r2 = 0.0;
    const int d8 = (d + 7) & ~7;
    for (int i = 0; i < d8; ++i) r2 = r2 + row[i];
    g.r2 = r2;
    return g;
}

template <int GW = 32>
__device__ inline GroupAdd cc_group_add(const double* bcf1, const double* bcf2, double bw, const double* p, int d,
                                        const Par& c)
{
    const int gl = threadIdx.x & (GW - 1);
    double b1[2] = {0.0, 0.0}, b2[2] = {0.0, 0.0}, px[2] = {0.0, 0.0};
#pragma unroll
    for (int h = 0; h < 2; ++h) {
        const int i = gl + GW * h;
        if (i < d) {
            px[h] = p[i];
            if (bcf1) { b1[h] = bcf1[i]; b2[h] = bcf2[i]; }
        }
    }
    return cc_group_add_regs<GW>(b1, b2, bw, px, d, c);
}

template <int CTRL>
__device__ __forceinline__ Cand cc_dpp_cand(const Cand& c)
{
    Cand o;
    o.dist = cc_dpp_f64<CTRL>(c.dist);
    o.key = __builtin_amdgcn_update_dpp(0, c.key, CTRL, 0xF, 0xF, false);
    o.slot = __builtin_amdgcn_update_dpp(0, c.slot, CTRL, 0xF, 0xF, false);
    return o;
}
template <typename F>
__device__ __forceinline__ void cc_row16_exchanges(F&& f)
{
    f(std::integral_constant<int, 0xB1>{});
    f(std::integral_constant<int, 0x4E>{});
    f(std::integral_constant<int, 0x141>{});
    f(std::integral_constant<int, 0x140>{});
}


__device__ __forceinline__ void cc_dsq_window_max(const unsigned long long* __restrict__ tile_dsq, int n,
                                                  unsigned long long (&m)[3])
{
    static_assert(CC_DSQ_STRIDE == 4, "a record is two 16-byte loads");
    constexpr int AHEAD = 8;
    const ulonglong2* const rec = reinterpret_cast<const ulonglong2*>(tile_dsq);
    for (int i0 = threadIdx.x; i0 < n; i0 += 64 * AHEAD) {
        ulonglong2 a[AHEAD], b[AHEAD];
#pragma unroll
        for (int q = 0; q < AHEAD; ++q) {
            const int i = min(i0 + 64 * q, n - 1);
            a[q] = rec[(size_t)i * 2];
            b[q] = rec[(size_t)i * 2 + 1];
        }
#pragma unroll
        for (int q = 0; q < AHEAD; ++q) {
            m[0] = a[q].x > m[0] ? a[q].x : m[0];
            m[1] = a[q].y > m[1] ? a[q].y : m[1];
            m[2] = b[q].x > m[2] ? b[q].x : m[2];
        }
    }
}

__global__ __launch_bounds__(64) void k_dseed(Ctl* __restrict__ ctl, const double* __restrict__ X, Table tab,
                                              Versions ver, Carry car, const Cand* __restrict__ clean,
                                              Cand* __restrict__ seed, const int* __restrict__ T, int round,
                                              const int8_t* __restrict__ dpath, int* __restrict__ sparse_list, int sparse_cap)
{
    CC_LATENCY_KERNEL();
    const int B = ctl->win_b;
    if (B == 0) return;
    if (ctl->fc[round - 1] >= B) return;
    const int j = blockIdx.x * blockDim.x + threadIdx.x;
    if (blockIdx.x * blockDim.x >= B) return;
    const bool la_mode = ctl->mode != 0;
    unsigned long long maxd[3] = {0ull, 0ull, 0ull}, maxd_car[3] = {0ull, 0ull, 0ull};
    {
        cc_dsq_window_max(ver.tile_dsq, (B + 15) / 16, maxd);
        if (la_mode) cc_dsq_window_max(car.tile_dsq, (ctl->car_n + 15) / 16, maxd_car);
#pragma unroll
        for (int K = 0; K < 3; ++K)
            for (int off = 32; off >= 1; off >>= 1) {
                const unsigned long long o = __shfl_xor(maxd[K], off), oc = __shfl_xor(maxd_car[K], off);
                maxd[K] = o > maxd[K] ? o : maxd[K];
                maxd_car[K] = oc > maxd_car[K] ? oc : maxd_car[K];
            }
    }
    bool flag_unprov = false, flag_unsafe = false, flag_n1skip = false;
    bool repeats = false;
    int flag_word = 0;
    double tau_w[3] = {CC_INF, CC_INF, CC_INF};
    bool need_ver = false, need_car = false;
    if (j < B) {
    const Par par = cc_load_par(ctl);
    const int d = par.d;
    const bool filter = par.filter != 0;
    const unsigned long long stamp = ctl->window_seq * 16ull + (unsigned long long)round;
    const double* p = X + (ctl->cursor + j) * d;
    Cand first0 = Cand{CC_INF, CC_IDX_INF, -1}, first1 = Cand{CC_INF, CC_IDX_INF, -1};
    double cap[2] = {CC_INF, CC_INF};
    bool lk_ok[2] = {par.k > 0.0, par.k > 0.0}, lbound[2] = {false, false};
    const double K = 1.0;

    const unsigned long long wseq = ctl->window_seq;
    Cand cq[4];
#pragma unroll
    for (int q = 0; q < 4; ++q) cq[q] = clean[(size_t)j * 4 + q];
    double d2v[2] = {CC_INF, CC_INF};
    bool have1[2];
    bool look[4];
#pragma unroll
    for (int kd = 0; kd < 2; ++kd) {
        if (cq[kd * 2 + 1].slot != -1) d2v[kd] = cq[kd * 2 + 1].dist;
        have1[kd] = cq[kd * 2].slot >= 0;
        lbound[kd] = cq[kd * 2].slot == CC_SLOT_BOUND;
        if (lbound[kd]) d2v[kd] = cq[kd * 2].dist;
        look[kd * 2] = have1[kd];
        look[kd * 2 + 1] = have1[kd] && cq[kd * 2 + 1].slot >= 0;
    }
    unsigned long long tcq[4], cwq[4], coq[4];
#pragma unroll
    for (int q = 0; q < 4; ++q) {
        const size_t sl = (size_t)(look[q] ? cq[q].slot : 0);
        tcq[q] = look[q] ? tab.touch[(size_t)(round & 1) * tab.cap + sl] : 0ull;
        cwq[q] = look[q] ? tab.cnt[sl] : 0ull;
        coq[q] = (look[q] && la_mode) ? tab.carry_of[sl] : 0ull;
    }
    int lv[4], n_memb[4];
    bool walk[4];
    int max_list = 0;
#pragma unroll
    for (int q = 0; q < 4; ++q) {
        const int head = 0xFFFFF - (int)(tcq[q] & 0xFFFFFull);
        lv[q] = -1;
        walk[q] = false;
        n_memb[q] = 0;
        if (!look[q]) continue;
        if ((tcq[q] >> 20) != stamp || head >= j) {
            if (la_mode && (coq[q] >> 20) == wseq) lv[q] = CC_CAR_BASE + (int)(coq[q] & 0xFFFFFull);
        } else {
            lv[q] = head;
            walk[q] = true;
            n_memb[q] = ((cwq[q] >> 24) == stamp) ? (int)(cwq[q] & 0xFFFFFFull) : 0;
            const int n_list = n_memb[q] < CC_CHAIN_MEMB ? n_memb[q] : CC_CHAIN_MEMB;
            max_list = n_list > max_list ? n_list : max_list;
        }
    }
    for (int pos = 0; pos * 4 < max_list; ++pos) {
        int4 mm[4];
#pragma unroll
        for (int q = 0; q < 4; ++q) {
            const bool on = walk[q] && pos * 4 < n_memb[q];
            mm[q] = on ? reinterpret_cast<const int4*>(tab.memb + (size_t)cq[q].slot * CC_CHAIN_MEMB)[pos] : make_int4(0, 0, 0, 0);
        }
#pragma unroll
        for (int q = 0; q < 4; ++q) {
            const int n_list = n_memb[q] < CC_CHAIN_MEMB ? n_memb[q] : CC_CHAIN_MEMB;
            const int e[4] = {mm[q].x, mm[q].y, mm[q].z, mm[q].w};
#pragma unroll
            for (int c = 0; c < 4; ++c) {
                const int m = e[c];
                if (walk[q] && pos * 4 + c < n_list && m < j && m > lv[q]) lv[q] = m;
            }
        }
    }
#pragma unroll
    for (int q = 0; q < 4; ++q)
        if (walk[q] && n_memb[q] > CC_CHAIN_MEMB) {
            const int clen = tab.clen[cq[q].slot];
            const int n = clen > CC_CHAIN_MEMB ? clen : CC_CHAIN_MEMB + 1;
            const int gap = B / n;
            const bool scan_first = (n - CC_CHAIN_MEMB) > gap / 8;
            int v = lv[q];
            int res = -2;
            for (int attempt = 0; attempt < 2 && res == -2; ++attempt) {
                if ((attempt == 0) == scan_first) {
                    const int want = cq[q].slot;
                    const int budget = min(16384, 16 * gap + 64);
                    for (int hi = j - 1, scanned = 0; res == -2 && scanned < budget; hi -= 32, scanned += 32) {
                        int tv[32];
#pragma unroll
                        for (int c = 0; c < 32; ++c) tv[c] = (hi - c > v) ? T[hi - c] : CC_T_UNKNOWN;
                        int hit = -1;
#pragma unroll
                        for (int c = 31; c >= 0; --c)
                            if (tv[c] == want) hit = hi - c;
                        if (hit < 0 && hi - 32 <= v) hit = v;
                        if (hit >= 0) res = hit;
                    }
                } else {
                    int w = v;
                    for (int steps = 0; steps < 64; ++steps) {
                        const int nxv = ver.next[w];
                        if (nxv >= j) { res = w; break; }
                        w = nxv;
                    }
                }
            }
            lv[q] = res;
        }
#pragma unroll
    for (int kd = 0; kd < 2; ++kd) {
        if (!have1[kd]) continue;
        const int v1 = lv[kd * 2];
        if (v1 == -1) cap[kd] = cq[kd * 2].dist;
        else {
            cap[kd] = d2v[kd];
            if (v1 < 0) lk_ok[kd] = false;
        }
        if (look[kd * 2 + 1] && lv[kd * 2 + 1] == -2) lk_ok[kd] = false;
    }
    bool sd[4];
    int kvq[4], keyq[4];
    const double* vcen[4];
    const double* vpref[4];
#pragma unroll
    for (int q = 0; q < 4; ++q) {
        sd[q] = look[q] && lv[q] >= 0;
        const bool cr = sd[q] && lv[q] >= CC_CAR_BASE;
        const size_t r = sd[q] ? (size_t)(cr ? lv[q] - CC_CAR_BASE : lv[q]) : 0;
        kvq[q] = sd[q] ? (cr ? car.kind[r] : ver.kind[r]) : CC_KIND_DEAD;
        keyq[q] = sd[q] ? (cr ? car.key[r] : ver.key[r]) : 0;
        vcen[q] = (cr ? car.cen : ver.cen) + r * d;
        vpref[q] = (cr ? car.pref : ver.pref) + r * d;
    }
#pragma unroll
    for (int q = 0; q < 4; ++q) sd[q] = sd[q] && kvq[q] != CC_KIND_DEAD;
    double accq[4] = {0.0, 0.0, 0.0, 0.0};
    for (int i0 = 0; i0 < d; i0 += 4) {
        double pv[4], cv[4][4], fv[4][4];
#pragma unroll
        for (int c = 0; c < 4; ++c) {
            const int i = (i0 + c < d) ? i0 + c : d - 1;
            pv[c] = p[i];
#pragma unroll
            for (int q = 0; q < 4; ++q) {
                cv[q][c] = sd[q] ? vcen[q][i] : 0.0;
                fv[q][c] = sd[q] ? vpref[q][i] : 1.0;
            }
        }
#pragma unroll
        for (int c = 0; c < 4; ++c) {
            if (i0 + c < d) {
#pragma unroll
                for (int q = 0; q < 4; ++q) {
                    double x = pv[c] - cv[q][c];
                    x = x * x;
                    accq[q] = accq[q] + cc_div_pref(x, fv[q][c], par);
                }
            }
        }
    }
#pragma unroll
    for (int q = 0; q < 4; ++q) {
        if (!sd[q]) continue;
        if (kvq[q] == 0 && filter) {
            const bool cr = lv[q] >= CC_CAR_BASE;
            const size_t r = (size_t)(cr ? lv[q] - CC_CAR_BASE : lv[q]);
            int ne1 = 0;
            cc_tentative_radius((cr ? car.cf1 : ver.cf1) + r * d, (cr ? car.cf2 : ver.cf2) + r * d,
                                cr ? car.w[r] : ver.w[r], p, d, par, nullptr, &ne1);
            if (ne1 > par.pi) continue;
        }
        if (kvq[q] == 0) {
            if (cand_less(accq[q], keyq[q], first0.dist, first0.key)) first0 = Cand{accq[q], keyq[q], lv[q]};
        } else {
            if (cand_less(accq[q], keyq[q], first1.dist, first1.key)) first1 = Cand{accq[q], keyq[q], lv[q]};
        }
    }
    seed[(size_t)j * 4 + 0] = first0;
    seed[(size_t)j * 4 + 1] = Cand{cap[0], 0, 0};
    seed[(size_t)j * 4 + 2] = first1;
    seed[(size_t)j * 4 + 3] = Cand{cap[1], 0, 0};

    double tau[3];
    for (int kd = 0; kd < 3; ++kd) {
        double t;
        const int list = (kd == 1) ? 1 : 0;
        const int from = (kd == 0) ? 0 : 1;
        if (list == 0 && filter) t = -CC_INF;
        else if (kd != 2 && !have1[kd]) t = CC_INF;
        else {
            const double fb = (list == 0) ? first0.dist : first1.dist;
            const double ce = fb < cap[list] ? fb : cap[list];
            t = (d2v[from] == CC_INF) ? CC_INF : (sqrt(d2v[from]) - sqrt(K * ce));
        }
        if (!lk_ok[list] || lbound[list] || (kd == 2 && !lk_ok[1])) t = -CC_INF;
        t = (t == CC_INF) ? CC_INF : t * (1.0 - 1e-9) - 1e-290;
        tau[kd] = t;
    }
    const bool need0 = true;
    const bool need1 = !(T[j] >= 0 && dpath[j] == 0);
    int flags = 0;
    if (!(cc_dsq_below(maxd[0], tau[0]) && cc_dsq_below(maxd[2], tau[2]))) flags |= CC_FLAG_U0;
    if (!cc_dsq_below(maxd[1], tau[1])) flags |= CC_FLAG_U1;
    if (la_mode && !(cc_dsq_below(maxd_car[0], tau[0]) && cc_dsq_below(maxd_car[2], tau[2]))) flags |= CC_FLAG_C0;
    if (la_mode && !cc_dsq_below(maxd_car[1], tau[1])) flags |= CC_FLAG_C1;
    need_ver = (need0 && (flags & CC_FLAG_U0)) || (need1 && (flags & CC_FLAG_U1));
    need_car = (need0 && (flags & CC_FLAG_C0)) || (need1 && (flags & CC_FLAG_C1));
    flag_unprov = !(lk_ok[0] && lk_ok[1]);
    flag_unsafe = need_ver || need_car;
    flag_n1skip = !need1;
    flag_word = flags;
#pragma unroll
    for (int kd = 0; kd < 3; ++kd) tau_w[kd] = tau[kd];
    {
        const int t = T[j];
        const Cand c1 = cq[0], c2 = cq[1];
        if (flags == 0 && t >= 0 && dpath[j] == 0 && c1.slot >= 0 && ver.tgt[j] == t && ver.acc[j] != 0) {
            const int head0 = 0xFFFFF - (int)(tcq[0] & 0xFFFFFull);
            const bool dirty0 = ((tcq[0] >> 20) == stamp && head0 < j) || (la_mode && (coq[0] >> 20) == wseq);
            if (!dirty0) {
                repeats = c1.slot == t && !(first0.slot >= 0 && cand_less(first0.dist, first0.key, c1.dist, c1.key));
            } else if (first0.slot >= 0 && (c2.slot == -1 || cand_less(first0.dist, first0.key, c2.dist, c2.key))) {
                if (first0.slot >= CC_CAR_BASE) repeats = car.slot[first0.slot - CC_CAR_BASE] == t;
                else repeats = ver.tgt[first0.slot] == t && ver.next[first0.slot] == j;
            }
        }
    }
    }
    if (sparse_cap > 0) {
        const unsigned long long m = __builtin_amdgcn_ballot_w64(flag_unsafe);
        if (m != 0ull) {
            int base = 0;
            if (threadIdx.x == (unsigned)__builtin_ctzll(m)) base = atomicAdd(&ctl->n_sparse, __builtin_popcountll(m));
            base = __shfl(base, __builtin_ctzll(m));
            const int idx = base + __builtin_popcountll(m & ((1ull << threadIdx.x) - 1ull));
            if (flag_unsafe && idx < sparse_cap) {
                sparse_list[idx] = j;
                flag_word |= CC_FLAG_SPARSE;
                flag_n1skip = false;
            }
        }
    }
    const unsigned long long any_v = __builtin_amdgcn_ballot_w64(need_ver), any_c = __builtin_amdgcn_ballot_w64(need_car);
    if (j < B) {
        if (flag_n1skip && any_v == 0ull && any_c == 0ull) { tau_w[1] = CC_INF; flag_word |= CC_FLAG_N1SKIP; }
#pragma unroll
        for (int kd = 0; kd < 3; ++kd) ver.tau[(size_t)j * CC_TAU_STRIDE + kd] = tau_w[kd];
        ver.unsafe[j] = flag_word;
    }
    if (__builtin_amdgcn_ballot_w64(j < B && !(repeats && any_v == 0ull && any_c == 0ull)) != 0ull && threadIdx.x == 0)
        ctl->rdiff[round] = 1;
    {
        const unsigned long long b1 = __builtin_amdgcn_ballot_w64(flag_unprov), b2 = __builtin_amdgcn_ballot_w64(flag_unsafe);
        if (threadIdx.x == 0 && b1) atomicAdd((unsigned long long*)&ctl->stat_unprovable, (unsigned long long)__builtin_popcountll(b1));
        if (threadIdx.x == 0 && b2) atomicAdd((unsigned long long*)&ctl->stat_unsafe, (unsigned long long)__builtin_popcountll(b2));
    }
    if (threadIdx.x == 0) {
        ver.skip[blockIdx.x] = any_v == 0ull ? 1 : 0;
        ver.skip_car[blockIdx.x] = (!la_mode || any_c == 0ull) ? 1 : 0;
    }
}

struct ScanCopy {
    double* cen;
    double* scl;
    double* cf1;
    double* cf2;
    double* w;
    int* kind;
    int* key;
};

struct CommitRec {
    int n;
    int M0;
    int pk0, ok0;
    long long pid0, oid0;
    const int* T;
    long long cursor;
    int carry;
    unsigned long long next_seq;
};

__device__ __forceinline__ void cc_apply_carry(const CommitRec* __restrict__ rec, const Carry& car, const ScanCopy& sc, int d,
                                               int filter, int part, int parts)
{
    if (rec->carry == 0) return;
    const int n = rec->n;
    const int gl = threadIdx.x & 31;
    const int groups = (parts * (int)blockDim.x) >> 5;
    for (int j = (part * (int)blockDim.x + (int)threadIdx.x) >> 5; j < n; j += groups) {
        const int kind = car.kind[j];
        if (kind == CC_KIND_DEAD) continue;
        const size_t row = (size_t)car.slot[j];
#pragma unroll
        for (int h = 0; h < 2; ++h) {
            const int i = gl + 32 * h;
            if (i >= d) continue;
            const size_t e = row * d + i, v = (size_t)j * d + i;
            sc.cen[e] = car.cen[v];
            sc.scl[e] = car.scl[v];
            if (filter) { sc.cf1[e] = car.cf1[v]; sc.cf2[e] = car.cf2[v]; }
        }
        if (gl == 0) {
            sc.kind[row] = kind;
            sc.key[row] = car.key[j];
            if (filter) sc.w[row] = car.w[j];
        }
    }
}


template <int GW>
__global__ __launch_bounds__(256) void k_decide(Ctl* __restrict__ ctl, const double* __restrict__ X, Table tab,
                                                Versions ver, Carry car, const Cand* __restrict__ part,
                                                size_t part_stride, Cand* __restrict__ clean,
                                                const Cand* __restrict__ dpart, const Cand* __restrict__ dpart2,
                                                const Cand* __restrict__ dseed,
                                                const int* __restrict__ Told, int* __restrict__ Tnew,
                                                int8_t* __restrict__ dpath, int S, int Sd, int round, int nodirty,
                                                int scan_rows, int part_inner, size_t part_outer,
                                                const CommitRec* __restrict__ ac_rec, ScanCopy ac_sc, int ac_blocks,
                                                int* __restrict__ long_list, int long_cap, int stat_tail, int last_round,
                                                int heavy_on, int quiet_ok, int* __restrict__ link_near)
{
    CC_LATENCY_KERNEL();
    if (ac_blocks > 0 && (int)blockIdx.x >= (int)gridDim.x - ac_blocks) {
        cc_apply_carry(ac_rec, car, ac_sc, ctl->d, ctl->filter, (int)blockIdx.x - ((int)gridDim.x - ac_blocks), ac_blocks);
        return;
    }
    const int B = ctl->win_b;
    if (B == 0) return;
    if (round == 0 && blockIdx.x == 0 && threadIdx.x == 0) {
        const int q = (int)(ctl->window_seq & 1ull);
        unsigned long long rows = 0ull, full = 0ull;
        if (stat_tail >= 0) {
            const Cand* g = part + (size_t)q * part_stride + (size_t)stat_tail;
            for (int r = 0; r < S; ++r) {
                rows += (unsigned long long)(unsigned)g[(size_t)r * part_outer].key;
                full += (unsigned long long)(unsigned)g[(size_t)r * part_outer].slot;
            }
        } else {
            rows = ctl->pstat[q][0];
            full = ctl->pstat[q][1];
        }
        ctl->pstat[q][0] = 0ull;
        ctl->pstat[q][1] = 0ull;
        ctl->stat_prune_rows += rows;
        ctl->stat_prune_full += full;
        if (ctl->n_missed_all[q] != 0) atomicAdd((unsigned long long*)&ctl->stat_missed, (unsigned long long)ctl->n_missed_all[q]);
        ctl->n_missed_all[q] = 0;
    }
    if (round > 0 && ctl->fc[round - 1] >= B) return;
    if (round > 0 && quiet_ok != 0 && ctl->rdiff[round] == 0) return;
    const int gl = threadIdx.x & (GW - 1);
    const int j = blockIdx.x * (blockDim.x / GW) + threadIdx.x / GW;
    if (j >= B) return;
    const Par par = cc_load_par(ctl);
    const int d = par.d;
    const Cand none = Cand{CC_INF, CC_IDX_INF, -1};

    Cand p1 = none, p2 = none, o1 = none, o2 = none;
    const unsigned long long wseq = ctl->window_seq;
    const bool la_mode = ctl->mode != 0;
    if (round == 0) {
        part += (size_t)(wseq & 1ull) * part_stride;
        for (int s = gl & 15; s < S; s += 16) {
            const Cand* q = part + (size_t)(s / part_inner) * part_outer + ((size_t)j * part_inner + (s % part_inner)) * 4;
            cc_top2_push(p1, p2, q[0]);
            cc_top2_push(p1, p2, q[1]);
            cc_top2_push(o1, o2, q[2]);
            cc_top2_push(o1, o2, q[3]);
        }
        cc_row16_exchanges([&](auto CT) {
            constexpr int C = decltype(CT)::value;
            const Cand a0 = cc_dpp_cand<C>(p1), a1 = cc_dpp_cand<C>(p2);
            const Cand a2 = cc_dpp_cand<C>(o1), a3 = cc_dpp_cand<C>(o2);
            cc_top2_push(p1, p2, a0);
            cc_top2_push(p1, p2, a1);
            cc_top2_push(o1, o2, a2);
            cc_top2_push(o1, o2, a3);
        });
        if (gl == 0) {
            Cand* out = clean + (size_t)j * 4;
            out[0] = p1; out[1] = p2; out[2] = o1; out[3] = o2;
        }
    } else {
        const Cand* in = clean + (size_t)j * 4;
        p1 = in[0]; p2 = in[1]; o1 = in[2]; o2 = in[3];
    }
    Cand dvp = none, dvo = none;
    const int flags = (round > 0) ? ver.unsafe[j] : 0;
    const bool on_list = nodirty == 2 && (flags & CC_FLAG_SPARSE) != 0;
    const bool ran = round > 0 && ((nodirty == 0 && ver.skip[j >> 6] == 0) || on_list);
    const bool ran_car = round > 0 && la_mode && ((nodirty == 0 && ver.skip_car[j >> 6] == 0) || on_list);
    if (round > 0) {
        Cand dummy = none;
        if (!ran && !ran_car) {
            dvp = dseed[(size_t)j * 4 + 0];
            dvo = dseed[(size_t)j * 4 + 2];
        } else {
        if ((gl & 15) == 0 && !(ran && (ran_car || !la_mode))) {
            dvp = dseed[(size_t)j * 4 + 0];
            dvo = dseed[(size_t)j * 4 + 2];
        }
        for (int s = gl & 15; s < Sd; s += 16) {
            if (ran) {
                const Cand* q = dpart + ((size_t)j * Sd + s) * 2;
                cc_top2_push(dvp, dummy, q[0]);
                cc_top2_push(dvo, dummy, q[1]);
            }
            if (ran_car) {
                const Cand* q2 = dpart2 + ((size_t)j * Sd + s) * 2;
                cc_top2_push(dvp, dummy, q2[0]);
                cc_top2_push(dvo, dummy, q2[1]);
            }
        }
        cc_row16_exchanges([&](auto CT) {
            constexpr int C = decltype(CT)::value;
            const Cand b0 = cc_dpp_cand<C>(dvp), b1 = cc_dpp_cand<C>(dvo);
            cc_top2_push(dvp, dummy, b0);
            cc_top2_push(dvo, dummy, b1);
        });
        }
    }

    const unsigned long long stamp = ctl->window_seq * 16ull + (unsigned long long)round;
    auto dirty = [&](int slot) -> bool {
        if (round == 0) return false;
        const unsigned long long t = tab.touch[(size_t)(round & 1) * tab.cap + slot];
        if ((t >> 20) == stamp && (0xFFFFF - (int)(t & 0xFFFFFull)) < j) return true;
        return la_mode && (tab.carry_of[slot] >> 20) == wseq;
    };

    const int M0 = ctl->m_rows;
    const double* p = X + (ctl->cursor + j) * d;
    int T = -1;
    int path = 2;
    auto run_stage = [&](const Cand& c1, const Cand& c2, const Cand& dd, int stage) {
        int state;
        Cand cb = none;
        if (c1.slot == -1) state = 0;
        else if (c1.slot == CC_SLOT_BOUND) {
            if (gl == 0 && round == 0) atomicAdd((unsigned long long*)&ctl->stat_missed, 1ull);
            T = CC_T_UNKNOWN;
            return;
        }
        else if (!dirty(c1.slot)) { state = 1; cb = c1; }
        else if (c2.slot == -1) state = 0;
        else if (c2.slot == CC_SLOT_BOUND) { state = 2; cb = c2; }
        else if (!dirty(c2.slot)) { state = 1; cb = c2; }
        else { state = 2; cb = c2; }

        int wkind = 0;
        int wrow = -1;
        if (state == 0) {
            if (dd.slot >= 0) { wkind = 2; wrow = dd.slot; }
        } else if (state == 1) {
            if (dd.slot >= 0 && cand_less(dd.dist, dd.key, cb.dist, cb.key)) { wkind = 2; wrow = dd.slot; }
            else { wkind = 1; wrow = cb.slot; }
        } else {
            if (dd.slot >= 0 && cand_less(dd.dist, dd.key, cb.dist, cb.key)) { wkind = 2; wrow = dd.slot; }
            else { T = CC_T_UNKNOWN; return; }
        }
        if (wkind == 0) return;
        const double *bcf1, *bcf2;
        double bw;
        int target;
        if (wkind == 1) {
            bcf1 = tab.cf1 + (size_t)wrow * d; bcf2 = tab.cf2 + (size_t)wrow * d; bw = tab.w[wrow];
            target = wrow;
        } else if (wrow >= CC_CAR_BASE) {
            const size_t r = (size_t)(wrow - CC_CAR_BASE);
            bcf1 = car.cf1 + r * d; bcf2 = car.cf2 + r * d; bw = car.w[r];
            target = car.slot[r];
        } else {
            bcf1 = ver.cf1 + (size_t)wrow * d; bcf2 = ver.cf2 + (size_t)wrow * d; bw = ver.w[wrow];
            target = ver.tgt[wrow];
        }
        bool known = false, fits = false;
        if (round > 0 && Told[j] == target && ver.tgt[j] == target) {
            known = (wkind == 2 && wrow < CC_CAR_BASE) ? (ver.next[wrow] == j) : true;
            fits = ver.acc[j] != 0;
        }
        if (!known) {
            const GroupAdd g = cc_group_add<GW>(bcf1, bcf2, bw, p, d, par);
            fits = g.r2 <= par.eps_sq;
        }
        if (fits) {
            T = target;
            path = stage;
        }
    };
    {
        const bool missing = ((flags & CC_FLAG_U0) != 0 && !ran) || ((flags & CC_FLAG_C0) != 0 && la_mode && !ran_car);
        if (missing) T = CC_T_UNKNOWN;
        else run_stage(p1, p2, dvp, 0);
    }
    if (T == -1) {
        const bool covers1 = (flags & CC_FLAG_N1SKIP) == 0;
        const bool missing = ((flags & CC_FLAG_U1) != 0 && !(ran && covers1)) ||
                             ((flags & CC_FLAG_C1) != 0 && la_mode && !(ran_car && covers1));
        if (missing) T = CC_T_UNKNOWN;
        else run_stage(o1, o2, dvo, 1);
    }
    if (T == -1) {
        if (ctl->no_create != 0) {
            T = CC_T_NONE;
            path = 8;
        } else {
            T = M0 + j;
            path = 2;
            if (gl == 0) ctl->any_new[round] = 1;
        }
    }
    if (gl == 0) {
        Tnew[j] = T;
        dpath[j] = (int8_t)path;
        if (link_near != nullptr) link_near[j] = CC_IDX_INF;
        if (round > 0 && (T == CC_T_UNKNOWN || T != Told[j])) atomicMin(&ctl->fc[round], j);
#ifdef CC_ROUND_DEBUG
        if (round > 0) {
            const int to = Told[j];
            atomicAdd(&ctl->dbg_round[round][5], 1ull);
            if (T == CC_T_UNKNOWN) atomicAdd(&ctl->dbg_round[round][0], 1ull);
            else if (T != to) {
                const int c = (to == M0 + j) ? (T >= M0 ? 1 : 2) : (T == M0 + j ? 3 : 4);
                atomicAdd(&ctl->dbg_round[round][c], 1ull);
            }
        }
#endif
        if ((j & 15) == 0) {
            ver.tile_dsq[(size_t)(j >> 4) * CC_DSQ_STRIDE] = 0ull;
            ver.tile_dsq[(size_t)(j >> 4) * CC_DSQ_STRIDE + 1] = 0ull;
            ver.tile_dsq[(size_t)(j >> 4) * CC_DSQ_STRIDE + 2] = 0ull;
        }
        if (last_round == 0 && T >= 0 && !(T < M0 && T < scan_rows) && !(heavy_on != 0 && T < M0 && tab.heavy[T] != 0) &&
            !(link_near != nullptr && T == M0 + j)) {
            const unsigned long long sn = (stamp + 1ull) << 20;
            const size_t wr = (size_t)((round + 1) & 1) * tab.cap + (size_t)T;
            atomicMax(&tab.touch[wr], sn | (unsigned long long)(0xFFFFF - j));
            atomicMax(&tab.last[wr], sn | (unsigned long long)j);
            const unsigned long long sc = (stamp + 1ull) << 24;
            unsigned long long* cw = tab.cnt + T;
            const unsigned long long old = __hip_atomic_load(cw, __ATOMIC_RELAXED, __HIP_MEMORY_SCOPE_AGENT);
            int pos = CC_CHAIN_MEMB + 1;
            if ((old & ~0xFFFFFFull) == sc) {
                if ((int)(old & 0xFFFFFFull) <= CC_CHAIN_MEMB) pos = (int)(atomicAdd(cw, 1ull) & 0xFFFFFFull);
            } else if (atomicCAS(cw, old, sc | 1ull) == old) {
                pos = 0;
            } else {
                pos = (int)(atomicAdd(cw, 1ull) & 0xFFFFFFull);
            }
            if (pos < CC_CHAIN_MEMB) tab.memb[(size_t)T * CC_CHAIN_MEMB + pos] = j;
            else if (pos == CC_CHAIN_MEMB && T < M0) {
                atomicAdd((unsigned long long*)&ctl->stat_long, 1ull);
                if (tab.heavy[T] == 0) {
                    const int hn = atomicAdd(&ctl->n_heavy_new, 1);
                    if (hn < CC_HEAVY_NEW) ctl->heavy_new[hn] = T;
                }
                if (long_list != nullptr) {
                    const int idx = atomicAdd(&ctl->n_long[round + 1], 1);
                    if (idx < long_cap) {
                        long_list[(size_t)((round + 1) & 1) * CC_LONG_CAP + idx] = T;
                        atomicOr(cw, CC_LONG_LISTED);
                    }
                }
            }
        }
    }
}


__global__ __launch_bounds__(256) void k_claims(const Ctl* __restrict__ ctl, Table tab, const int* __restrict__ T,
                                                int round, int scan_rows, int quiet_ok)
{
    CC_LATENCY_KERNEL();
    const int B = ctl->win_b;
    if (B == 0) return;
    if (round > 0 && ctl->fc[round - 1] >= B) return;
    if (round > 0 && quiet_ok != 0 && ctl->rdiff[round] == 0) return;
    const int M0 = ctl->m_rows;
    const int m = blockIdx.x;
    if (m >= M0 || m >= scan_rows) return;
    __shared__ int s_pos, s_cnt, s_first, s_last;
    if (threadIdx.x == 0) { s_pos = 0; s_cnt = 0; s_first = CC_IDX_INF; s_last = -1; }
    __syncthreads();
    int lmin = CC_IDX_INF, lmax = -1, mine = 0;
    volatile int* const pos_now = &s_pos;
    const int4* T4 = reinterpret_cast<const int4*>(T);
    constexpr int AHEAD = 8;
    for (int base0 = (int)threadIdx.x * 4; base0 < B; base0 += 256 * 4 * AHEAD) {
        int4 v[AHEAD];
#pragma unroll
        for (int q = 0; q < AHEAD; ++q) {
            const int base = base0 + q * 256 * 4;
            v[q] = T4[(base < B ? base : 0) >> 2];
        }
#pragma unroll
        for (int q = 0; q < AHEAD; ++q) {
            const int base = base0 + q * 256 * 4;
            const int e[4] = {v[q].x, v[q].y, v[q].z, v[q].w};
#pragma unroll
            for (int c = 0; c < 4; ++c) {
                const int j = base + c;
                if (j < B && e[c] == m) {
                    lmin = j < lmin ? j : lmin;
                    lmax = j > lmax ? j : lmax;
                    ++mine;
                    if (*pos_now < CC_CHAIN_MEMB) {
                        const int pos = atomicAdd(&s_pos, 1);
                        if (pos < CC_CHAIN_MEMB) tab.memb[(size_t)m * CC_CHAIN_MEMB + pos] = j;
                    }
                }
            }
        }
    }
    if (lmax >= 0) { atomicMin(&s_first, lmin); atomicMax(&s_last, lmax); atomicAdd(&s_cnt, mine); }
    __syncthreads();
    if (threadIdx.x == 0 && s_cnt > 0) {
        const unsigned long long stamp = ctl->window_seq * 16ull + (unsigned long long)round;
        const unsigned long long sn = (stamp + 1ull) << 20;
        const size_t wr = (size_t)((round + 1) & 1) * tab.cap + (size_t)m;
        tab.touch[wr] = sn | (unsigned long long)(0xFFFFF - s_first);
        tab.last[wr] = sn | (unsigned long long)s_last;
        tab.cnt[m] = ((stamp + 1ull) << 24) | (unsigned long long)s_cnt;
    }
}

__global__ __launch_bounds__(256) void k_claims_heavy(Ctl* __restrict__ ctl, Table tab, const int* __restrict__ T, int round,
                                                      int* __restrict__ long_list, int long_cap, int quiet_ok)
{
    CC_LATENCY_KERNEL();
    const int B = ctl->win_b;
    if (B == 0) return;
    if (round > 0 && ctl->fc[round - 1] >= B) return;
    if (round > 0 && quiet_ok != 0 && ctl->rdiff[round] == 0) return;
    if ((int)blockIdx.x >= ctl->n_heavy) return;
    const int m = ctl->heavy_list[blockIdx.x];
    if (m < 0 || m >= ctl->m_rows) return;
    __shared__ int s_pos, s_cnt, s_first, s_last;
    if (threadIdx.x == 0) { s_pos = 0; s_cnt = 0; s_first = CC_IDX_INF; s_last = -1; }
    __syncthreads();
    int lmin = CC_IDX_INF, lmax = -1, mine = 0;
    volatile int* const pos_now = &s_pos;
    const int4* T4 = reinterpret_cast<const int4*>(T);
    constexpr int AHEAD = 8;
    for (int base0 = (int)threadIdx.x * 4; base0 < B; base0 += 256 * 4 * AHEAD) {
        int4 v[AHEAD];
#pragma unroll
        for (int q = 0; q < AHEAD; ++q) {
            const int base = base0 + q * 256 * 4;
            v[q] = T4[(base < B ? base : 0) >> 2];
        }
#pragma unroll
        for (int q = 0; q < AHEAD; ++q) {
            const int base = base0 + q * 256 * 4;
            const int e[4] = {v[q].x, v[q].y, v[q].z, v[q].w};
#pragma unroll
            for (int c = 0; c < 4; ++c) {
                const int j = base + c;
                if (j < B && e[c] == m) {
                    lmin = j < lmin ? j : lmin;
                    lmax = j > lmax ? j : lmax;
                    ++mine;
                    if (*pos_now < CC_CHAIN_MEMB) {
                        const int pos = atomicAdd(&s_pos, 1);
                        if (pos < CC_CHAIN_MEMB) tab.memb[(size_t)m * CC_CHAIN_MEMB + pos] = j;
                    }
                }
            }
        }
    }
    if (lmax >= 0) { atomicMin(&s_first, lmin); atomicMax(&s_last, lmax); atomicAdd(&s_cnt, mine); }
    __syncthreads();
    if (threadIdx.x != 0) return;
    const int n_claims = s_cnt;
    if (n_claims > 0) {
        const unsigned long long stamp = ctl->window_seq * 16ull + (unsigned long long)round;
        const unsigned long long sn = (stamp + 1ull) << 20;
        const size_t wr = (size_t)((round + 1) & 1) * tab.cap + (size_t)m;
        tab.touch[wr] = sn | (unsigned long long)(0xFFFFF - s_first);
        tab.last[wr] = sn | (unsigned long long)s_last;
        unsigned long long cw = ((stamp + 1ull) << 24) | (unsigned long long)n_claims;
        if (n_claims > CC_CHAIN_MEMB) {
            atomicAdd((unsigned long long*)&ctl->stat_long, 1ull);
            if (long_list != nullptr) {
                const int idx = atomicAdd(&ctl->n_long[round + 1], 1);
                if (idx < long_cap) {
                    long_list[(size_t)((round + 1) & 1) * CC_LONG_CAP + idx] = m;
                    cw |= CC_LONG_LISTED;
                }
            }
        }
        tab.cnt[m] = cw;
    }
    if (round == 0 && n_claims <= CC_CHAIN_MEMB / 2) tab.heavy[m] = 2;
}


__global__ __launch_bounds__(256) void k_chain(Ctl* __restrict__ ctl, const double* __restrict__ X, Table tab,
                                               Versions ver, Carry car, const int* __restrict__ T, int round,
                                               int long_rows, const unsigned long long* __restrict__ lprev,
                                               unsigned long long* __restrict__ lstat)
{
    CC_LATENCY_KERNEL();
    const int B = ctl->win_b;
    if (B == 0) return;
    if (ctl->fc[round - 1] >= B) return;
    if (blockIdx.x == 0 && threadIdx.x == 0) {
        ctl->last_round = round;
        ctl->n_sparse = 0;
        ctl->rdiff[round] = 0;
    }
    const int gl = threadIdx.x & 31;
    const int j = blockIdx.x * (blockDim.x >> 5) + (threadIdx.x >> 5);
    if (j >= B) return;
    const int t = T[j];
    if (t < 0) {
        if (gl == 0) {
            ver.kind[j] = CC_KIND_DEAD; ver.next[j] = j; ver.tgt[j] = t; ver.acc[j] = 0; ver.upg[j] = -1;
        }
        return;
    }
    const unsigned long long stamp = ctl->window_seq * 16ull + (unsigned long long)round;
    if (lprev != nullptr) {
        const unsigned long long lp = lprev[j];
        if ((lp >> 27) == stamp) {
            const int pv = (int)(lp & 0x1FFFFull) - 1;
            const size_t lslot = (size_t)(round & 1) * CC_LSTAT_ROWS + (size_t)((lp >> 17) & 0x3FFull);
            const Par par = cc_load_par(ctl);
            const int d = par.d;
            double bc1[2] = {0.0, 0.0}, bc2[2] = {0.0, 0.0}, px[2] = {0.0, 0.0}, c0[2] = {0.0, 0.0}, w0[2] = {1.0, 1.0};
#pragma unroll
            for (int h = 0; h < 2; ++h) {
                const int i = gl + 32 * h;
                if (i < d) {
                    bc1[h] = (pv < 0) ? tab.cf1[(size_t)t * d + i] : ver.cf1[(size_t)pv * d + i];
                    bc2[h] = (pv < 0) ? tab.cf2[(size_t)t * d + i] : ver.cf2[(size_t)pv * d + i];
                    px[h] = X[(ctl->cursor + j) * d + i];
                    c0[h] = tab.cen[(size_t)t * d + i];
                    w0[h] = 1.0 / tab.pref[(size_t)t * d + i];
                }
            }
            const double bw = (pv < 0) ? tab.w[t] : ver.w[pv];
            const int bkind = tab.kind[t];
            int kind0 = bkind;
            if (ctl->mode != 0) {
                const unsigned long long co = tab.carry_of[t];
                if ((co >> 20) == ctl->window_seq) {
                    const size_t r = (size_t)(co & 0xFFFFFull);
                    kind0 = car.kind0[r];
#pragma unroll
                    for (int h = 0; h < 2; ++h) {
                        const int i = gl + 32 * h;
                        if (i < d) { c0[h] = car.c0[r * d + i]; w0[h] = car.w0[r * d + i]; }
                    }
                }
            }
            const GroupAdd g = cc_group_add_regs(bc1, bc2, bw, px, d, par);
            if (!(g.r2 <= par.eps_sq)) {
                if (gl == 0) atomicMin(&lstat[lslot], (stamp << 20) | (unsigned long long)j);
                return;
            }
            double dq = 0.0;
            bool mv = false;
#pragma unroll
            for (int h = 0; h < 2; ++h) {
                const int i = gl + 32 * h;
                if (i < d) {
                    ver.cen[(size_t)j * d + i] = g.cen[h]; ver.pref[(size_t)j * d + i] = g.pr[h];
                    ver.scl[(size_t)j * d + i] = par.pow2 ? (g.pr[h] == 1.0 ? 1.0 : par.inv_k) : g.pr[h];
                }
                const double df = g.cen[h] - c0[h];
                dq += df * df * w0[h];
                mv = mv || (1.0 / g.pr[h] != w0[h]);
            }
            dq = cc_group_sum_any_order(dq);
            const bool promoted = bkind == CC_KIND_PCORE && kind0 == CC_KIND_OUTLIER;
            if ((bkind != kind0 && !promoted) || !(dq >= 0.0) || cc_group_ballot(mv) != 0u) dq = CC_INF;
            if (gl == 0) {
                ver.tgt[j] = t; ver.kind[j] = bkind; ver.key[j] = tab.key[t]; ver.upg[j] = -1; ver.acc[j] = 1;
                int cls;
                ver.dsq[j] = cc_dsq_store(dq, bkind, kind0, &cls);
                atomicMax(&ver.tile_dsq[(size_t)(j >> 4) * CC_DSQ_STRIDE + cls], cc_dsq_code(dq));
            }
            return;
        }
    }
    const size_t rd = (size_t)(round & 1) * tab.cap + (size_t)t;
    const unsigned long long ft = tab.touch[rd], lt = tab.last[rd];
    if ((ft >> 20) != stamp || 0xFFFFF - (int)(ft & 0xFFFFFull) != j) return;
    const int last_j = ((lt >> 20) == stamp) ? (int)(lt & 0xFFFFFull) : j;
    const unsigned long long cw = tab.cnt[t];
    const int n_memb = ((cw >> 24) == stamp) ? (int)(cw & 0xFFFFFFull) : 0;
    const bool listed = n_memb <= CC_CHAIN_MEMB;
    if (!listed && ((t < long_rows && t < ctl->m_rows) || (cw & CC_LONG_LISTED) != 0ull)) return;
    int sorted_memb = CC_IDX_INF;
    if (listed) {
        const int mine = (gl < n_memb) ? tab.memb[(size_t)t * CC_CHAIN_MEMB + gl] : CC_IDX_INF;
        int rank = 0;
        for (int q = 0; q < n_memb; ++q) rank += (__shfl(mine, q, 32) < mine) ? 1 : 0;
        for (int q = 0; q < n_memb; ++q) {
            const int v = __shfl(mine, q, 32), r = __shfl(rank, q, 32);
            if (r == gl) sorted_memb = v;
        }
    }
    const int4* T4 = reinterpret_cast<const int4*>(T);
    int step = 0;
    int blk = -1;
    bool have_nb = false;
    int4 vb = make_int4(0, 0, 0, 0), vn = make_int4(0, 0, 0, 0);

    const Par par = cc_load_par(ctl);
    const int d = par.d;
    const int M0 = ctl->m_rows;
    const long long cursor = ctl->cursor;
    const int pk_base = ctl->n_pkeys;
    const bool isnew = t >= M0;
    const bool valid_chain = !isnew || (t == M0 + j);

    double bc1[2] = {0.0, 0.0}, bc2[2] = {0.0, 0.0}, bce[2] = {0.0, 0.0}, bpr[2] = {1.0, 1.0};
    double bw = 0.0;
    int bkind = CC_KIND_OUTLIER, bkey = ctl->n_okeys + j, bupg = -1;
    if (!isnew) {
#pragma unroll
        for (int h = 0; h < 2; ++h) {
            const int i = gl + 32 * h;
            if (i < d) {
                bc1[h] = tab.cf1[(size_t)t * d + i]; bc2[h] = tab.cf2[(size_t)t * d + i];
                bce[h] = tab.cen[(size_t)t * d + i]; bpr[h] = tab.pref[(size_t)t * d + i];
            }
        }
        bw = tab.w[t]; bkind = tab.kind[t]; bkey = tab.key[t];
    }
    double c0[2] = {bce[0], bce[1]};
    double w0[2] = {1.0 / bpr[0], 1.0 / bpr[1]};
    double binv[2] = {w0[0], w0[1]};
    int kind0 = bkind;
    if (!isnew && ctl->mode != 0) {
        const unsigned long long co = tab.carry_of[t];
        if ((co >> 20) == ctl->window_seq) {
            const size_t r = (size_t)(co & 0xFFFFFull);
            kind0 = car.kind0[r];
#pragma unroll
            for (int h = 0; h < 2; ++h) {
                const int i = gl + 32 * h;
                if (i < d) { c0[h] = car.c0[r * d + i]; w0[h] = car.w0[r * d + i]; }
            }
        }
    }
    constexpr int NB = CC_CHAIN_AHEAD;
    auto find_next = [&](const int after) -> int {
        int nx = CC_IDX_INF;
        for (int base = (after + 1) & ~127; base <= last_j && after < last_j; base += 128) {
            const int i = base + gl * 4;
            if (base != blk) {
                vb = (have_nb && base == blk + 128) ? vn : T4[(base >> 2) + gl];
                blk = base;
                have_nb = base + 128 <= last_j;
                if (have_nb) vn = T4[((base + 128) >> 2) + gl];
            }
            const int4 v = vb;
            const unsigned mm = ((i > after && i < B && v.x == t) ? 1u : 0u) | ((i + 1 > after && i + 1 < B && v.y == t) ? 2u : 0u) |
                                ((i + 2 > after && i + 2 < B && v.z == t) ? 4u : 0u) | ((i + 3 > after && i + 3 < B && v.w == t) ? 8u : 0u);
            const unsigned b = cc_group_ballot(mm != 0u);
            if (b) {
                const int l = __builtin_ctz(b);
                const unsigned ml = __shfl(mm, l, 32);
                nx = base + l * 4 + __builtin_ctz(ml);
                break;
            }
        }
        return nx;
    };
    int first = j;
    int walked = 0;
    while (first != CC_IDX_INF) {
        int mem[NB + 1];
        mem[0] = first;
#pragma unroll
        for (int q = 1; q <= NB; ++q) {
            int m = CC_IDX_INF;
            if (mem[q - 1] != CC_IDX_INF) {
                if (listed) m = (step + q < n_memb) ? __shfl(sorted_memb, (step + q) & 31, 32) : CC_IDX_INF;
                else m = find_next(mem[q - 1]);
            }
            mem[q] = m;
        }
        step += NB;
        double pxb[NB][2];
#pragma unroll
        for (int q = 0; q < NB; ++q)
#pragma unroll
            for (int h = 0; h < 2; ++h) {
                const int i = gl + 32 * h;
                pxb[q][h] = (valid_chain && mem[q] != CC_IDX_INF && i < d) ? X[(cursor + mem[q]) * d + i] : 0.0;
            }
        __builtin_amdgcn_s_waitcnt(0x0F70);
#pragma unroll
        for (int q = 0; q < NB; ++q) {
            if (mem[q] == CC_IDX_INF) break;
            ++walked;
            const int cur = mem[q];
            const int nx = mem[q + 1];
            const double px[2] = {pxb[q][0], pxb[q][1]};
            if (!valid_chain) {
                if (gl == 0) {
                    ver.tgt[cur] = t; ver.kind[cur] = CC_KIND_DEAD; ver.next[cur] = cur; ver.acc[cur] = 0; ver.upg[cur] = -1;
                }
            } else {
                const double w1 = bw + 1.0;
                const GroupAdd g = cc_group_add_regs(bc1, bc2, bw, px, d, par);
                const bool creates = isnew && cur == j;
                const bool ok = creates || (g.r2 <= par.eps_sq);
                if (ok) {
                    if (bkind == CC_KIND_OUTLIER && !creates && w1 >= par.beta_mu && g.gt1 <= par.pi) {
                        bkind = CC_KIND_PCORE; bkey = pk_base + cur; bupg = cur;
                        if (gl == 0) ctl->any_up[round] = 1;
                    }
#pragma unroll
                    for (int h = 0; h < 2; ++h) {
                        bc1[h] = g.c1[h]; bc2[h] = g.c2[h];
                        bce[h] = g.cen[h];
                        if (g.pr[h] != bpr[h]) binv[h] = 1.0 / g.pr[h];
                        bpr[h] = g.pr[h];
                    }
                    bw = w1;
                }
#pragma unroll
                for (int h = 0; h < 2; ++h) {
                    const int i = gl + 32 * h;
                    if (i < d) {
                        ver.cf1[(size_t)cur * d + i] = bc1[h]; ver.cf2[(size_t)cur * d + i] = bc2[h];
                        ver.cen[(size_t)cur * d + i] = bce[h]; ver.pref[(size_t)cur * d + i] = bpr[h];
                        ver.scl[(size_t)cur * d + i] = par.pow2 ? (bpr[h] == 1.0 ? 1.0 : par.inv_k) : bpr[h];
                    }
                }
                double dq = 0.0;
#pragma unroll
                for (int h = 0; h < 2; ++h) {
                    const double df = bce[h] - c0[h];
                    dq += df * df * w0[h];
                }
                dq = cc_group_sum_any_order(dq);
                bool mv = false;
#pragma unroll
                for (int h = 0; h < 2; ++h) mv = mv || (binv[h] != w0[h]);
                const bool promoted = bkind == CC_KIND_PCORE && kind0 == CC_KIND_OUTLIER;
                if (isnew || (bkind != kind0 && !promoted) || !(dq >= 0.0) || cc_group_ballot(mv) != 0u) dq = CC_INF;
                if (gl == 0) {
                    ver.w[cur] = bw;
                    ver.tgt[cur] = t; ver.kind[cur] = bkind; ver.key[cur] = bkey; ver.upg[cur] = bupg;
                    ver.acc[cur] = ok ? 1 : 0; ver.next[cur] = nx;
                    int cls;
                    ver.dsq[cur] = cc_dsq_store(dq, bkind, isnew ? CC_KIND_DEAD : kind0, &cls);
                    atomicMax(&ver.tile_dsq[(size_t)(cur >> 4) * CC_DSQ_STRIDE + cls], cc_dsq_code(dq));
                }
            }
        }
        first = mem[NB];
    }
    if (gl == 0 && !isnew) tab.clen[t] = walked;
}


#define CC_LONG_XY_DOUBLES 6144
#define CC_LONG_PAD_DIM 128
#define CC_LONG_QUEUE 2048
#define CC_LONG_THREADS 1024

#define CC_LPREV(stamp, slot, prev) (((unsigned long long)(stamp) << 27) | ((unsigned long long)(slot) << 17) | (unsigned long long)((prev) + 1))
template <bool SPLIT, bool PREP>
__global__ __launch_bounds__(SPLIT ? CC_LONG_THREADS : 256) void k_chain_long(Ctl* __restrict__ ctl, const double* __restrict__ X, Table tab,
                                                    Versions ver, Carry car, const int* __restrict__ T, int round,
                                                    int scan_rows, const int* __restrict__ long_list,
                                                    unsigned long long* __restrict__ lstat, unsigned long long* __restrict__ lprev)
{
    CC_LATENCY_KERNEL();
    const int B = ctl->win_b;
    if (B == 0) return;
    if (ctl->fc[round - 1] >= B) return;
    const int M0 = ctl->m_rows;
    int t;
    if (long_list == nullptr) {
        t = blockIdx.x;
        if (t >= scan_rows) return;
    } else {
        const int n_listed = min(ctl->n_long[round], (int)gridDim.x);
        if ((int)blockIdx.x >= n_listed) return;
        t = long_list[(size_t)(round & 1) * CC_LONG_CAP + blockIdx.x];
    }
    if (t >= M0) return;
    const unsigned long long stamp = ctl->window_seq * 16ull + (unsigned long long)round;
    const size_t rd = (size_t)(round & 1) * tab.cap + (size_t)t;
    const unsigned long long ft = tab.touch[rd], lt = tab.last[rd];
    if ((ft >> 20) != stamp) return;
    const unsigned long long cw = tab.cnt[t];
    const int n_memb = ((cw >> 24) == stamp) ? (int)(cw & 0xFFFFFFull) : 0;
    if (n_memb <= CC_CHAIN_MEMB) return;
    int head = 0xFFFFF - (int)(ft & 0xFFFFFull);
    const int last_j = ((lt >> 20) == stamp) ? (int)(lt & 0xFFFFFull) : head;
    const size_t lslot = (size_t)(round & 1) * CC_LSTAT_ROWS + (size_t)blockIdx.x;
    int resume_prev = -1;
    bool resumed = false;
    if constexpr (PREP) {
        if (tab.kind[t] != CC_KIND_PCORE) return;
        if (threadIdx.x == 0) {
            lstat[lslot] = (stamp << 20) | 0xFFFFFull;
            atomicAdd(&lstat[2 * CC_LSTAT_ROWS], 1ull);
        }
    } else {
        if (lstat != nullptr) {
            const unsigned long long ls = lstat[lslot];
            if ((ls >> 20) == stamp) {
                const int f = (int)(ls & 0xFFFFFull);
                if (f == 0xFFFFF) return;
                if (threadIdx.x == 0) atomicAdd(&lstat[2 * CC_LSTAT_ROWS + 1], 1ull);
                resumed = true;
                head = f;
                resume_prev = (int)(lprev[f] & 0x1FFFFull) - 1;
            }
        }
    }

    const Par par = cc_load_par(ctl);
    const int d = par.d;
    const int tid = threadIdx.x;
    const long long cursor = ctl->cursor;
    const int pk_base = ctl->n_pkeys;
    const int K = min(256, (CC_LONG_XY_DOUBLES / (2 * d)) & ~7);

    __shared__ __attribute__((aligned(16))) double s_xy[CC_LONG_XY_DOUBLES + 2 * CC_LONG_PAD_DIM];
    __shared__ double s_w[256], s_dq[256];
    __shared__ __attribute__((aligned(16))) double s_xy2[PREP && SPLIT ? CC_LONG_XY_DOUBLES + 2 * CC_LONG_PAD_DIM : 1];
    __shared__ double s_w2[PREP && SPLIT ? 256 : 1];
    __shared__ unsigned long long s_mask[256];
    __shared__ int s_flag[256];
    constexpr int PASS = (SPLIT ? CC_LONG_THREADS : 256) * 4;
    constexpr int QUEUE = SPLIT ? 4 * CC_LONG_QUEUE : CC_LONG_QUEUE;
    constexpr int SCAN_WAVES = PASS / 256;
    __shared__ int s_queue[QUEUE];
    __shared__ double s_b1[64], s_b2[64], s_bcen[64], s_bpref[64], s_c0[64], s_w0[64];
    __shared__ double s_bw, s_bdq;
    __shared__ unsigned long long s_m0, s_bmask;
    __shared__ int s_wsum[SCAN_WAVES];
    __shared__ int s_first_fail, s_first_up;
    __shared__ double s_term[SPLIT && !PREP ? CC_LONG_XY_DOUBLES / 2 : 1], s_dqt[SPLIT && !PREP ? CC_LONG_XY_DOUBLES / 2 : 1];
    __shared__ unsigned char s_pf[SPLIT && !PREP ? CC_LONG_XY_DOUBLES / 2 : 1];
    const int NT = (int)blockDim.x;
    const int Kp = K | 1;
    const bool one_wave = d <= 31;
    double* const xs = s_xy;
    double* const ys = s_xy + (size_t)Kp * d;
    auto at = [&](int k, int i) { return i * Kp + k; };

    int bkind = tab.kind[t], bkey = tab.key[t], bupg = -1;
    if (tid < d) {
        s_b1[tid] = tab.cf1[(size_t)t * d + tid]; s_b2[tid] = tab.cf2[(size_t)t * d + tid];
        s_bcen[tid] = tab.cen[(size_t)t * d + tid]; s_bpref[tid] = tab.pref[(size_t)t * d + tid];
    }
    if (tid == 0) s_bw = tab.w[t];
    __syncthreads();
    int kind0 = bkind;
    {
        bool from_carry = false;
        size_t r = 0;
        if (ctl->mode != 0) {
            const unsigned long long co = tab.carry_of[t];
            if ((co >> 20) == ctl->window_seq) {
                from_carry = true;
                r = (size_t)(co & 0xFFFFFull);
                kind0 = car.kind0[r];
            }
        }
        if (tid < d) {
            s_c0[tid] = from_carry ? car.c0[r * d + tid] : s_bcen[tid];
            s_w0[tid] = from_carry ? car.w0[r * d + tid] : 1.0 / s_bpref[tid];
        }
    }
    __syncthreads();
    if (resume_prev >= 0) {
        if (tid < d) {
            const size_t o = (size_t)resume_prev * d + tid;
            s_b1[tid] = ver.cf1[o]; s_b2[tid] = ver.cf2[o]; s_bcen[tid] = ver.cen[o]; s_bpref[tid] = ver.pref[o];
        }
        if (tid == 0) s_bw = ver.w[resume_prev];
        __syncthreads();
    }
    if (tid == 0) {
        double dq = 0.0;
        for (int i = 0; i < d; ++i) {
            const double df = s_bcen[i] - s_c0[i];
            dq += df * df * s_w0[i];
        }
        s_bdq = dq;
        unsigned long long m0 = 0ull, bm = 0ull;
        for (int i = 0; i < d; ++i) {
            m0 |= (s_w0[i] != 1.0) ? (1ull << i) : 0ull;
            bm |= (s_bpref[i] != 1.0) ? (1ull << i) : 0ull;
        }
        s_m0 = m0;
        s_bmask = bm;
    }

    const int4* T4 = reinterpret_cast<const int4*>(T);
    int qhead = 0, qcount = 0;
    int scan_pos = head & ~(PASS - 1);
    bool scan_done = false;
    int walked = 0;
// ... 214 lines not shown
            prefix_chain(xs + (size_t)tid * Kp, s_b1[tid], n);
        } else if (tid >= 64 && tid < 64 + d) {
            prefix_chain(ys + (size_t)(tid - 64) * Kp, s_b2[tid - 64], n);
        } else if (tid == 128) {
            double w = s_bw;
            int k = 0;
            for (; k + 16 <= n; k += 16) {
                double v[16];
#pragma unroll
                for (int u = 0; u < 16; ++u) {
                    w = w + 1.0;
                    v[u] = w;
                }
#pragma unroll
                for (int u = 0; u < 16; ++u) s_w[k + u] = v[u];
            }
            for (; k < n; ++k) {
                w = w + 1.0;
                s_w[k] = w;
            }
        }
        __syncthreads();
        CC_TICK(2);

        if constexpr (PREP) {
            for (int e = tid; e < n * d; e += NT) {
                const int k = e / d, i = e - k * d;
                const size_t o = (size_t)s_queue[(qhead + k) & (QUEUE - 1)] * d + i;
                ver.cf1[o] = xs[at(k, i)]; ver.cf2[o] = ys[at(k, i)];
            }
            if (tid < n) {
                const int k = tid;
                const int m = s_queue[(qhead + k) & (QUEUE - 1)];
                const int pv = (k > 0) ? s_queue[(qhead + k - 1) & (QUEUE - 1)] : prev_last;
                ver.w[m] = s_w[k];
                ver.next[m] = (k + 1 < qcount) ? s_queue[(qhead + k + 1) & (QUEUE - 1)] : CC_IDX_INF;
                lprev[m] = CC_LPREV(stamp, blockIdx.x, pv);
            }
            prev_last = s_queue[(qhead + n - 1) & (QUEUE - 1)];
            __syncthreads();
            CC_TICK(5);
            const int l = n - 1;
            if (tid < d) { s_b1[tid] = xs[at(l, tid)]; s_b2[tid] = ys[at(l, tid)]; }
            if (tid == 64) s_bw = s_w[l];
            qhead = (qhead + n) & (QUEUE - 1);
            qcount -= n;
            walked += n;
            pre_elems = pre_next;
            __syncthreads();
            CC_TICK(6);
#ifdef CC_LONG_TIMERS
            tk_acc[7] += 1ull;
#endif
            continue;
        }

        if constexpr (SPLIT) {
        for (int e = tid; e < n * d; e += NT) {
            const int k = e / d, i = e - k * d;
            const double w1 = s_w[k];
            const double qa = ys[at(k, i)] / w1;
            const double qb = xs[at(k, i)] / w1;
            const double var = qa - qb * qb;
            const bool prefd = var <= par.delta_sq;
            const double pr = prefd ? par.k : 1.0;
            s_term[e] = cc_div_pref(var, pr, par);
            s_pf[e] = prefd ? (unsigned char)1 : (unsigned char)0;
            const double df = qb - s_c0[i];
            s_dqt[e] = df * df * s_w0[i];
        }
        __syncthreads();
        CC_TICK(3);
        }
        if (tid < n) {
            const int k = tid;
            const double w1 = s_w[k];
            double r2 = 0.0, dq = 0.0;
            int gt1 = 0;
            unsigned long long mask = 0ull;
            for (int i = 0; i < d; ++i) {
                if constexpr (SPLIT) {
                    r2 = r2 + s_term[k * d + i];
                    dq += s_dqt[k * d + i];
                    const bool prefd = s_pf[k * d + i] != 0;
                    gt1 += (prefd && par.k > 1.0) ? 1 : 0;
                    mask |= prefd ? (1ull << i) : 0ull;
                } else {
                    const double qa = ys[at(k, i)] / w1;
                    const double qb = xs[at(k, i)] / w1;
                    const double var = qa - qb * qb;
                    const bool prefd = var <= par.delta_sq;
                    const double pr = prefd ? par.k : 1.0;
                    r2 = r2 + cc_div_pref(var, pr, par);
                    gt1 += (pr > 1.0) ? 1 : 0;
                    mask |= prefd ? (1ull << i) : 0ull;
                    const double df = qb - s_c0[i];
                    dq += df * df * s_w0[i];
                }
            }
            const bool ok = r2 <= par.eps_sq;
            const bool up = w1 >= par.beta_mu && gt1 <= par.pi;
            s_flag[k] = (ok ? 1 : 0) | (up ? 2 : 0);
            s_mask[k] = mask;
            s_dq[k] = dq;
            if (!ok) atomicMin(&s_first_fail, k);
            if (up) atomicMin(&s_first_up, k);
        }
        __syncthreads();
        CC_TICK(4);
        const int f = s_first_fail;
        const int n_ok = f < n ? f : n;
        const int n_rows = f < n ? f + 1 : n;
        int u = -1;
        if (bkind == CC_KIND_OUTLIER && s_first_up < n_ok) u = s_first_up;
        const int up_point = (u >= 0) ? s_queue[(qhead + u) & (QUEUE - 1)] : -1;

        for (int e = tid; e < n_rows * d; e += NT) {
            const int k = e / d, i = e - k * d;
            const int m = s_queue[(qhead + k) & (QUEUE - 1)];
            const int src = (k < n_ok) ? k : k - 1;
            double c1, c2, ce, pr;
            if (src >= 0) {
                c1 = xs[at(src, i)]; c2 = ys[at(src, i)];
                ce = c1 / s_w[src];
                pr = ((s_mask[src] >> i) & 1ull) ? par.k : 1.0;
            } else {
                c1 = s_b1[i]; c2 = s_b2[i]; ce = s_bcen[i]; pr = s_bpref[i];
            }
            const size_t o = (size_t)m * d + i;
            ver.cf1[o] = c1; ver.cf2[o] = c2; ver.cen[o] = ce; ver.pref[o] = pr;
            ver.scl[o] = par.pow2 ? (pr == 1.0 ? 1.0 : par.inv_k) : pr;
        }
        if (tid < n_rows) {
            const int k = tid;
            const int m = s_queue[(qhead + k) & (QUEUE - 1)];
            const int src = (k < n_ok) ? k : k - 1;
            const bool promoted = u >= 0 && k >= u;
            const int kind = promoted ? CC_KIND_PCORE : bkind;
            double dq = (src >= 0) ? s_dq[src] : s_bdq;
            const unsigned long long vmask = (src >= 0) ? s_mask[src] : s_bmask;
            const bool was_outlier = kind == CC_KIND_PCORE && kind0 == CC_KIND_OUTLIER;
            if ((kind != kind0 && !was_outlier) || !(dq >= 0.0) || vmask != s_m0) dq = CC_INF;
            const int nx = (k + 1 < qcount) ? s_queue[(qhead + k + 1) & (QUEUE - 1)] : CC_IDX_INF;
            ver.w[m] = (src >= 0) ? s_w[src] : s_bw;
            ver.tgt[m] = t;
            ver.kind[m] = kind;
            ver.key[m] = promoted ? pk_base + up_point : bkey;
            ver.upg[m] = promoted ? up_point : bupg;
            ver.acc[m] = (k < n_ok) ? 1 : 0;
            ver.next[m] = nx;
            int cls;
            ver.dsq[m] = cc_dsq_store(dq, kind, kind0, &cls);
            atomicMax(&ver.tile_dsq[(size_t)(m >> 4) * CC_DSQ_STRIDE + cls], cc_dsq_code(dq));
        }
        __syncthreads();
        CC_TICK(5);

        if (n_ok > 0) {
            const int l = n_ok - 1;
            if (tid < d) {
                s_b1[tid] = xs[at(l, tid)]; s_b2[tid] = ys[at(l, tid)];
                s_bcen[tid] = xs[at(l, tid)] / s_w[l];
                s_bpref[tid] = ((s_mask[l] >> tid) & 1ull) ? par.k : 1.0;
            }
            if (tid == 64) { s_bw = s_w[l]; s_bdq = s_dq[l]; s_bmask = s_mask[l]; }
        }
        if (u >= 0) {
            bkind = CC_KIND_PCORE; bkey = pk_base + up_point; bupg = up_point;
            promoted_any = true;
        }
        qhead = (qhead + n_rows) & (QUEUE - 1);
        qcount -= n_rows;
        walked += n_rows;
        pre_elems = (n_rows == n) ? pre_next : 0;
        __syncthreads();
        CC_TICK(6);
#ifdef CC_LONG_TIMERS
        tk_acc[7] += 1ull;
#endif
    }
#ifdef CC_LONG_TIMERS
    if (tid == 0 && blockIdx.x == 0)
        for (int i = 0; i < 8; ++i) atomicAdd(&ctl->dbg_long[i], tk_acc[i]);
#endif
    if (tid == 0) {
        if (!resumed) tab.clen[t] = walked;
        if (promoted_any) ctl->any_up[round] = 1;
    }
}


__global__ __launch_bounds__(1024) void k_commit_a(Ctl* __restrict__ ctl, Table tab, Versions ver, Carry car,
                                                   const int* __restrict__ Tbuf0, const int* __restrict__ Tbuf1,
                                                   int* __restrict__ rk, CommitRec* __restrict__ rec,
                                                   const Cand* __restrict__ clean, const int8_t* __restrict__ dpath)
{
    CC_LATENCY_KERNEL();
    const int B = ctl->win_b;
    if (B == 0) {
        if (threadIdx.x == 0) rec->n = 0;
        return;
    }
    __shared__ unsigned wsum[16];
    __shared__ unsigned tot;
    __shared__ int dirty_tiles;
    if (threadIdx.x >= 960 && (ctl->n_heavy > 0 || ctl->n_heavy_new > 0)) {
        const int lane = (int)threadIdx.x - 960;
        const unsigned long long below = (1ull << lane) - 1ull;
        const int n_h = min(ctl->n_heavy, CC_HEAVY_CAP);
        const int row = lane < n_h ? ctl->heavy_list[lane] : -1;
        const bool keep = row >= 0 && tab.heavy[row] == 1;
        if (row >= 0 && !keep) tab.heavy[row] = 0;
        const unsigned long long km = __builtin_amdgcn_ballot_w64(keep);
        const int n_keep = __builtin_popcountll(km);
        const int n_new = min(ctl->n_heavy_new, CC_HEAVY_NEW);
        const int nr = lane < n_new ? ctl->heavy_new[lane] : -1;
        bool add = nr >= 0 && atomicExch(&tab.heavy[nr], 1) == 0;
        const unsigned long long am = __builtin_amdgcn_ballot_w64(add);
        const int apos = n_keep + __builtin_popcountll(am & below);
        if (add && apos >= CC_HEAVY_CAP) {
            tab.heavy[nr] = 0;
            add = false;
        }
        if (keep) ctl->heavy_list[__builtin_popcountll(km & below)] = row;
        if (add) ctl->heavy_list[apos] = nr;
        if (lane == 0) {
            ctl->n_heavy = min(n_keep + __builtin_popcountll(am), CC_HEAVY_CAP);
            ctl->n_heavy_new = 0;
        }
    }
    const int r = ctl->last_round;
    const bool la_win = ctl->mode != 0;
    if (threadIdx.x == 0) dirty_tiles = 0;
    __syncthreads();
    const int n_tiles = (r >= 1) ? (B + 63) / 64 : 0;
    for (int i = threadIdx.x; i < n_tiles; i += 1024)
        if (ver.skip[i] == 0 || (la_win && ver.skip_car[i] == 0)) atomicAdd(&dirty_tiles, 1);
    const int* T = ((r - 1) & 1) ? Tbuf1 : Tbuf0;
    const int fcv = ctl->fc[r];
    const int n = fcv < B ? fcv : B;
    const int M0 = ctl->m_rows;
    const int tid = threadIdx.x;
    const long long cursor = ctl->cursor;
    const long long oid0 = ctl->outlier_last_id, pid0 = ctl->pcore_last_id;
    const int pk0 = ctl->n_pkeys, ok0 = ctl->n_okeys;
    const long long n_points = ctl->n_points;
    const int win_cfg = ctl->win_cfg;

    __shared__ unsigned char sflag[CC_MAX_WINDOW];
    const bool events = ctl->any_new[r - 1] != 0 || ctl->any_up[r] != 0;
    if (threadIdx.x == 0) tot = 0u;
    if (events) {
    for (int j = tid; j < B; j += 1024)
        sflag[j] = (j < n) ? (unsigned char)(((T[j] == M0 + j) ? 1 : 0) | ((ver.upg[j] == j) ? 2 : 0)) : (unsigned char)0;
    __syncthreads();
    const int per = (B + 1023) >> 10;
    unsigned mine = 0u;
    for (int q = 0; q < per; ++q) {
        const int j = tid * per + q;
        const unsigned f = (j < B) ? (unsigned)sflag[j] : 0u;
        mine += (f & 1u) | ((f & 2u) << 15);
    }
    unsigned v = mine;
    const int lane = tid & 63, wid = tid >> 6;
    for (int off = 1; off < 64; off <<= 1) {
        const unsigned o = __shfl_up(v, off);
        if (lane >= off) v += o;
    }
    if (lane == 63) wsum[wid] = v;
    __syncthreads();
    if (tid == 0) {
        unsigned run = 0u;
        for (int i = 0; i < 16; ++i) { const unsigned x = wsum[i]; wsum[i] = run; run += x; }
        tot = run;
    }
    __syncthreads();
    unsigned run = v - mine + wsum[wid];
    for (int q = 0; q < per; ++q) {
        const int j = tid * per + q;
        if (j < B) {
            rk[j] = (int)run;
            const unsigned f = (unsigned)sflag[j];
            run += (f & 1u) | ((f & 2u) << 15);
        }
    }
    }
    __syncthreads();
    const int tot_new = (int)(tot & 0xFFFFu), tot_up = (int)(tot >> 16);
    const unsigned long long seq = ctl->window_seq;
    const long long next_cursor = cursor + n;
    const long long left = n_points - next_cursor;
    const int next_b = (int)(left < (long long)win_cfg ? left : (long long)win_cfg);
    const int qn = (int)((seq + 1ull) & 1ull);
    const bool la_ok = ctl->la_on != 0 && n == B && next_b > 0 && ctl->la_b[qn] == next_b &&
                       ctl->la_cursor[qn] == next_cursor;
    if (la_ok)
        for (int i = tid; i < CC_DSQ_STRIDE * ((B + 15) / 16 + 1); i += 1024) car.tile_dsq[i] = 0ull;
    __shared__ double s_sum[2][16];
    __shared__ int s_cnt[2][16];
    {
        double sm[2] = {0.0, 0.0};
        int cn[2] = {0, 0};
        for (int j = tid * 8; j < n; j += 8192) {
            const int pth = dpath[j];
            if (T[j] >= 0 && (pth == 0 || pth == 1)) {
                const double dist = clean[(size_t)j * 4 + pth * 2].dist;
                if (dist < CC_INF) { sm[pth] += dist; cn[pth] += 1; }
            }
        }
#pragma unroll
        for (int K = 0; K < 2; ++K) {
            for (int off = 32; off >= 1; off >>= 1) {
                sm[K] += __shfl_xor(sm[K], off);
                cn[K] += __shfl_xor(cn[K], off);
            }
            if ((tid & 63) == 0) { s_sum[K][tid >> 6] = sm[K]; s_cnt[K][tid >> 6] = cn[K]; }
        }
    }
    __syncthreads();
    if (tid == 0) {
        const int slot = (int)(seq & 1ull);
        for (int K = 0; K < 2; ++K) {
            double sm = 0.0;
            int cn = 0;
            for (int i = 0; i < 16; ++i) { sm += s_sum[K][i]; cn += s_cnt[K][i]; }
            if (cn > 0) { ctl->tg[slot][K] = sm / (double)cn; ctl->tg_ok[slot][K] = 1; }
            else { ctl->tg[slot][K] = ctl->tg[slot ^ 1][K]; ctl->tg_ok[slot][K] = ctl->tg_ok[slot ^ 1][K]; }
        }
        rec->n = n; rec->M0 = M0; rec->pk0 = pk0; rec->ok0 = ok0; rec->pid0 = pid0; rec->oid0 = oid0; rec->T = T;
        rec->carry = la_ok ? 1 : 0;
        rec->cursor = cursor;
        rec->next_seq = seq + 1ull;
        ctl->mode = la_ok ? 1 : 0;
        ctl->car_n = la_ok ? B : 0;
        ctl->stat_lookahead += la_ok ? 1 : 0;
        const int q2 = (int)(seq & 1ull);
        const long long c2 = next_cursor + next_b;
        const long long left2 = n_points - c2;
        ctl->la_cursor[q2] = c2;
        ctl->la_b[q2] = (ctl->la_on != 0 && left2 > 0) ? (int)(left2 < (long long)win_cfg ? left2 : (long long)win_cfg) : 0;
        ctl->la_rows[q2] = M0 + tot_new;
        ctl->m_rows = M0 + tot_new;
        ctl->n_okeys = ok0 + tot_new;
        ctl->outlier_last_id = oid0 + tot_new;
        ctl->n_pkeys = pk0 + tot_up;
        ctl->pcore_last_id = pid0 + tot_up;
        ctl->cursor = cursor + n;
        ctl->stat_windows += 1;
        ctl->stat_rounds += r;
        ctl->round_hist[r] += 1;
        ctl->stat_truncated += (n < B) ? 1 : 0;
        ctl->stat_tiles += n_tiles;
        ctl->stat_dirty_tiles += dirty_tiles;
        ctl->stat_trunc_unknown += (n < B && T[n] == CC_T_UNKNOWN) ? 1 : 0;
        ctl->seed_at = (n < B && T[n] == CC_T_UNKNOWN) ? cursor + n : -1ll;
        ctl->stat_table_rows += M0;
        ctl->stat_pair_rows += (double)B * (double)M0;
        ctl->window_seq = seq + 1ull;
        if ((ctl->la_on != 0 && !la_ok && next_b > 0) || n == 0) {
            ctl->stall_b = next_b;
            ctl->win_b = 0;
            ctl->la_b[0] = 0;
            ctl->la_b[1] = 0;
        } else {
            ctl->win_b = next_b;
        }
        ctl->last_round = 0;
        ctl->fc[0] = 0;
        for (int i = 1; i < CC_MAX_ROUNDS + 2; ++i) ctl->fc[i] = CC_IDX_INF;
        for (int i = 0; i < CC_MAX_ROUNDS + 2; ++i) { ctl->any_new[i] = 0; ctl->any_up[i] = 0; ctl->n_long[i] = 0; }
    }
}

__global__ __launch_bounds__(256) void k_commit_b(const CommitRec* __restrict__ rec, Table tab, Versions ver,
                                                  Carry car, const int* __restrict__ rk,
                                                  const int8_t* __restrict__ dpath, long long* __restrict__ lab_uid,
                                                  int8_t* __restrict__ lab_path, int d, ScanCopy sc, int filter)
{
    CC_LATENCY_KERNEL();
    const int n = rec->n;
    if (n == 0) return;
    const int M0 = rec->M0;
    const int* T = rec->T;
    const bool carry = rec->carry != 0;
    const int gl = threadIdx.x & 31;
    const int groups = (gridDim.x * blockDim.x) >> 5;
    for (int j = (blockIdx.x * blockDim.x + threadIdx.x) >> 5; j < n; j += groups) {
        if (gl == 0) {
            const int tj = T[j];
            lab_uid[rec->cursor + j] = (tj < 0) ? -1ll : ((tj < M0) ? tab.uid[tj] : rec->oid0 + (rk[tj - M0] & 0xFFFF));
            lab_path[rec->cursor + j] = (int8_t)(dpath[j] | ((ver.upg[j] == j) ? 4 : 0));
        }
        if (ver.next[j] < n) {
            if (carry && gl == 0) { car.kind[j] = CC_KIND_DEAD; car.slot[j] = 0; }
            continue;
        }
        const int t = T[j];
        const int c = t - M0;
        const size_t row = (t < M0) ? (size_t)t : (size_t)(M0 + (rk[c] & 0xFFFF));
        const int u = ver.upg[j];
        const int kind = ver.kind[j];
        int key;
        if (u >= 0) key = rec->pk0 + (int)((unsigned)rk[u] >> 16);
        else if (t >= M0) key = rec->ok0 + (rk[c] & 0xFFFF);
        else key = tab.key[row];
        const int kind0 = (t < M0) ? tab.kind[row] : CC_KIND_DEAD;
        double dq = 0.0;
        bool metric_moved = false;
#pragma unroll
        for (int h = 0; h < 2; ++h) {
            const int i = gl + 32 * h;
            if (i >= d) continue;
            const size_t e = row * d + i, v = (size_t)j * d + i;
            const double ncen = ver.cen[v], npref = ver.pref[v], nscl = ver.scl[v], n1 = ver.cf1[v], n2 = ver.cf2[v];
            if (carry) {
                const double oc = (t < M0) ? tab.cen[e] : 0.0;
                const double ow = (t < M0) ? 1.0 / tab.pref[e] : 0.0;
                metric_moved = metric_moved || (t < M0 && npref != tab.pref[e]);
                car.c0[v] = oc; car.w0[v] = ow;
                car.cf1[v] = n1; car.cf2[v] = n2; car.cen[v] = ncen; car.pref[v] = npref; car.scl[v] = nscl;
                const double df = ncen - oc;
                dq += df * df * ow;
            }
            tab.cf1[e] = n1; tab.cf2[e] = n2; tab.cen[e] = ncen; tab.pref[e] = npref; tab.scl[e] = nscl;
            if (sc.cen) {
                sc.cen[e] = ncen; sc.scl[e] = nscl;
                if (filter) { sc.cf1[e] = n1; sc.cf2[e] = n2; }
            }
        }
        if (carry) {
            for (int off = 16; off >= 1; off >>= 1) dq += __shfl_xor(dq, off, 32);
            const bool promoted = kind == CC_KIND_PCORE && kind0 == CC_KIND_OUTLIER;
            if (kind0 == CC_KIND_DEAD || (kind != kind0 && !promoted) || !(dq >= 0.0) || cc_group_ballot(metric_moved) != 0u) dq = CC_INF;
        }
        if (gl == 0) {
            tab.w[row] = ver.w[j];
            tab.kind[row] = kind;
            if (u >= 0) {
                tab.key[row] = key;
                tab.id[row] = rec->pid0 + (long long)((unsigned)rk[u] >> 16);
            } else if (t >= M0) {
                tab.key[row] = key;
                tab.id[row] = rec->oid0 + (rk[c] & 0xFFFF);
            }
            if (t >= M0) tab.uid[row] = rec->oid0 + (rk[c] & 0xFFFF);
            if (sc.cen) {
                sc.kind[row] = kind;
                sc.key[row] = key;
                if (filter) sc.w[row] = ver.w[j];
            }
            if (carry) {
                car.w[j] = ver.w[j];
                car.kind[j] = kind;
                car.key[j] = key;
                car.slot[j] = (int)row;
                car.kind0[j] = kind0;
                int cls;
                car.dsq[j] = cc_dsq_store(dq, kind, kind0, &cls);
                atomicMax(&car.tile_dsq[(size_t)(j >> 4) * CC_DSQ_STRIDE + cls], cc_dsq_code(dq));
                tab.carry_of[row] = (rec->next_seq << 20) | (unsigned long long)j;
            }
        }
    }
}
```

### include/chronoclust_hip.h

```cpp
#ifndef CHRONOCLUST_HIP_H
#define CHRONOCLUST_HIP_H

#include <stdint.h>

#ifdef __cplusplus
extern "C" {
#endif

typedef struct cc_handle cc_handle;

enum cc_status {
    CC_OK = 0,
    CC_ERR_NO_DEVICE = -1,
    CC_ERR_BAD_ARG = -2,
    CC_ERR_NONFINITE = -3,
    CC_ERR_OOM = -4,
    CC_ERR_INTERNAL = -5,
    CC_ERR_COMM = -6
};

enum cc_kind { CC_PCORE = 0, CC_OUTLIER = 1 };

#define CC_MAX_DIM 1024
#define CC_WINDOW_MAX_DIM 64
// ... 101 lines not shown
int cc_inject_mc(cc_handle* h, int kind, int32_t d, const double* cf1, const double* cf2, const double* cen,
                 const double* pref, double w, int64_t id, int64_t uid);

int cc_inject_bulk(cc_handle* h, int kind, int32_t d, int32_t n, const double* cf1, const double* cf2,
                   const double* cen, const double* pref, const double* w, const int64_t* id, const int64_t* uid);

int cc_offline(cc_handle* h, int32_t* n_clusters, int8_t* out_core, int32_t* out_pdim, int32_t* out_nn,
               int32_t* out_nw);
int cc_num_core(cc_handle* h);
int cc_cluster_size(cc_handle* h, int32_t c);
int cc_cluster_export(cc_handle* h, int32_t c, int64_t* members, double* w, double* cf1, double* cf2,
                      double* cen, double* pref);

int cc_clusters_total_members(cc_handle* h);
int cc_clusters_export(cc_handle* h, int64_t* members, int32_t* offsets, double* w, double* cf1, double* cf2,
                       double* cen, double* pref);

int cc_col_minmax(cc_handle* h, const double* x, int64_t n, int32_t d, double* out_min, double* out_max);
int cc_points_upload_scaled(cc_handle* h, const double* x, int64_t n, int32_t d, const double* scale,
                            const double* min_);
int cc_points_download(cc_handle* h, double* out, const double* scale, const double* min_);

int cc_assoc_argmin(cc_handle* h, const double* cur_cen, const double* cur_pref, int32_t mc,
                    const double* prev_cen, int32_t mp, int32_t d, int32_t* out_idx, double* out_dist);

#define CC_COMM_ID_BYTES 128
int cc_comm_unique_id(void* out_id);
int cc_comm_init_rccl(cc_handle* h, const void* id_bytes, int rank, int world);
int cc_comm_init_local(cc_handle** handles, int world);
int cc_comm_calibrate(cc_handle* h);
int cc_comm_destroy(cc_handle* h);
int cc_comm_info(cc_handle* h, int32_t* rank, int32_t* world, int32_t* transport);
int cc_comm_set_relaxed(cc_handle* h, int32_t minibatch_points);
typedef struct cc_relaxed_stats {
    int64_t super_steps;
    int64_t minibatch_points;
    int64_t deferred_points;
    int64_t reserved[5];
} cc_relaxed_stats;
int cc_get_relaxed_stats(cc_handle* h, cc_relaxed_stats* out);
int cc_shard_rows(int32_t n, int32_t world, int32_t rank, int32_t unit, int32_t* lo, int32_t* hi);
int cc_set_shard_thresholds(cc_handle* h, int64_t min_row_dims, int32_t offline_min_rows);

int cc_point_clusters(cc_handle* h, int32_t* out_idx);

int64_t cc_format_points_csv(const double* values, int64_t n, int32_t d, int64_t first_id, const int32_t* label_idx,
                             const char* label_bytes, const int32_t* label_offsets, int32_t n_labels, char* out,
                             int64_t cap);

int cc_sync(cc_handle* h);

int cc_get_stats(cc_handle* h, cc_stats* out);

#define CC_POLICY_MAX_ROUNDS 8
typedef struct cc_policy_config {
    int32_t window, rounds_max, windows_per_sync, early_window;
    int32_t lookahead;
    int32_t allow_nodirty;
    int32_t prune_mode;
    int32_t prune_applicable;
    int32_t can_shard;
    int32_t d;
    int32_t resume;
    int32_t allow_sparse;
    int32_t allow_guess;
    int32_t allow_probe;
    int64_t shard_min_row_dims;
    int64_t n_end;
    int64_t shard_min_row_dims_pruned;
    int32_t lookahead_pruned;
    int32_t force_prune_rows;
} cc_policy_config;
typedef struct cc_policy_carry {
    int32_t adapt_win, clean_batches, since_shrink, pad;
} cc_policy_carry;
typedef struct cc_policy_obs {
    int64_t cursor;
    int32_t m_rows, stall_b;
    int64_t stat_windows, stat_truncated, stat_trunc_unknown, stat_tiles, stat_dirty_tiles;
    int64_t stat_unsafe;
    int64_t stat_missed;
    int64_t round_hist[CC_POLICY_MAX_ROUNDS + 2];
    uint64_t prune_rows, prune_full;
    int32_t after_sequential;
    int32_t tg_ok;
} cc_policy_obs;
typedef struct cc_policy_decision {
    int32_t win_cfg;
    int32_t want;
    int32_t rounds, batch_windows, lookahead, nodirty;
    int32_t prune;
    int32_t shard;
    int32_t restart;
    int32_t bad;
    int32_t stalled;
    int32_t sparse;
    int32_t probe;
    int32_t pad;
    int64_t wins, pts, trunc, unk, tiles, dtiles, grew, prune_rows, prune_full;
} cc_policy_decision;
int cc_policy_replay(const cc_policy_config* cfg, cc_policy_carry* carry, int64_t start_cursor, int32_t start_rows,
                     const cc_policy_obs* obs, int32_t n, cc_policy_decision* out);
double cc_policy_seq_rate_guess(int32_t d, int32_t m_rows, int32_t allow_seq_r, int32_t allow_seq_g);
typedef struct cc_seq_event {
    int32_t chunk_event;
    int32_t bad;
    int32_t possible;
    int32_t more;
    int32_t seq_r_applies;
    int32_t use_g;
    int32_t allow_seq_g, wide;
    int64_t got, chunk;
    double rate;
    double rate_guess;
} cc_seq_event;
int cc_seq_handover_replay(int32_t mode, int32_t possible, int32_t sticky, const cc_seq_event* ev, int32_t n, int32_t* outcome,
                           int64_t* stint_len);

typedef struct cc_batch_inputs {
    int32_t window, win_cfg;
    int32_t S_cfg;
    int32_t n_cus, prune_now;
    int32_t prune_wgs_per_cu, plain_wgs_per_cu;
    int32_t decide_threads, chain_threads, commit_threads;
    int32_t allow_claims, allow_long, allow_heavy, allow_prep;
    int32_t m_rows, n_heavy;
    int32_t long_seen, long_few;
    int64_t long_avg;
    int32_t batch_windows, pad;
    int64_t points_left;
} cc_batch_inputs;
enum { CC_LONG_NONE = 0, CC_LONG_ROWS_SPLIT = 1, CC_LONG_ROWS_SMALL = 2, CC_LONG_LIST_SPLIT = 3, CC_LONG_LIST_SMALL = 4 };
typedef struct cc_batch_geometry {
    int32_t gw;
    int32_t S;
    int32_t sparse_cap;
    int32_t dblocks, cblocks, rblocks;
    int32_t scan_rows;
    int32_t long_rows;
    int32_t long_listed;
    int32_t heavy_on;
    int32_t long_cap;
    int32_t windows_now;
    int32_t prep;
    int32_t prep_form;
    int32_t long_form;
    int32_t pad;
} cc_batch_geometry;
int cc_batch_plan(const cc_batch_inputs* in, cc_batch_geometry* out);

enum { CC_CHAIN_NONE = 0, CC_CHAIN_COMMON = 1, CC_CHAIN_GENERAL = 2 };
int cc_scan_width(int32_t d, int32_t filter_on, int32_t k_pow2, int32_t* padded, int32_t* scan_u, int32_t* chain);

#ifdef __cplusplus
}
#endif
#endif
```

Before: 77.02 million points/s.

## Add coarse per-1024-row dsq max records and spread k_dseed candidates over quad lanes

Adds a second level of per-class dsq maxima, one record per 1024 rows, kept up to date with extra atomicMax calls wherever the per-16-row tile maxima are written. k_dseed then reads one coarse record per lane and reduces with DPP instead of scanning every 16-row tile. k_dseed is also restructured to use four lanes per point, one per candidate, with 256-thread blocks, DPP quad broadcasts and block-wide __syncthreads_or in place of wave ballots. This trades extra atomics in the update kernels and a more complex seed kernel for a much cheaper window-max scan and more parallel candidate walks.

```diff
diff --git a/chronoclust_amd/_lib.py b/chronoclust_amd/_lib.py
--- a/chronoclust_amd/_lib.py
+++ b/chronoclust_amd/_lib.py
@@ -160,6 +160,7 @@
     "cc_seq_handover_replay": (C.c_int, [C.c_int32, C.c_int32, C.c_int32, C.POINTER(CcSeqEvent), C.c_int32, _i32p, _i64p]),
     "cc_batch_plan": (C.c_int, [C.POINTER(CcBatchInputs), C.POINTER(CcBatchGeometry)]),
     "cc_scan_width": (C.c_int, [C.c_int32, C.c_int32, C.c_int32, _i32p, _i32p, _i32p]),
+    "cc_dsq_coarse_layout": (C.c_int, [C.c_int32, C.c_int32, C.c_int32, _i32p, _i32p, _i32p, _i32p]),
     "cc_shard_rows": (C.c_int, [C.c_int32, C.c_int32, C.c_int32, C.c_int32, _i32p, _i32p]),
     "cc_set_shard_thresholds": (C.c_int, [C.c_void_p, C.c_int64, C.c_int32]),
 }
@@ -191,7 +192,7 @@
 
 
 HOST_ONLY_SYMBOLS = ("cc_policy_replay", "cc_policy_seq_rate_guess", "cc_seq_handover_replay", "cc_batch_plan", "cc_shard_rows",
-                     "cc_format_points_csv", "cc_scan_width")
+                     "cc_format_points_csv", "cc_scan_width", "cc_dsq_coarse_layout")
 
 
 def load_host_only(path):
@@ -322,6 +323,14 @@
     return padded.value, bool(scan_u.value), SCAN_CHAINS[chain.value]
 
 
+def dsq_coarse_layout(rows, row, cls):
+    first, word, records, words = C.c_int32(), C.c_int32(), C.c_int32(), C.c_int32()
+    rc = load().cc_dsq_coarse_layout(int(rows), int(row), int(cls), C.byref(first), C.byref(word), C.byref(records), C.byref(words))
+    if rc != 0:
+        raise ValueError("cc_dsq_coarse_layout(%r, %r, %r): %s" % (rows, row, cls, _ERRORS.get(rc, rc)))
+    return first.value, word.value, records.value, words.value
+
+
 def shard_rows(n, world, rank, unit=1):
     lo, hi = C.c_int32(), C.c_int32()
     rc = load().cc_shard_rows(int(n), int(world), int(rank), int(unit), C.byref(lo), C.byref(hi))
diff --git a/chronoclust_amd/csrc/cc_batch.h b/chronoclust_amd/csrc/cc_batch.h
--- a/chronoclust_amd/csrc/cc_batch.h
+++ b/chronoclust_amd/csrc/cc_batch.h
@@ -12,6 +12,7 @@
 
 constexpr int kMaxWindow = 49152;
 constexpr int kLongCap = 512;
+constexpr int kDsqStride = 4;
 
 constexpr int kScanWidths[8] = {4, 8, 14, 16, 20, 32, 40, 64};
 struct ScanWidth {
diff --git a/chronoclust_amd/csrc/cc_handle.h b/chronoclust_amd/csrc/cc_handle.h
--- a/chronoclust_amd/csrc/cc_handle.h
+++ b/chronoclust_amd/csrc/cc_handle.h
@@ -459,7 +459,7 @@
     const size_t w = (size_t)win, d = (size_t)std::max(h->d, h->d_alloc);
     h->v_cf1.ensure(w * d); h->v_cf2.ensure(w * d); h->v_cen.ensure(w * d); h->v_pref.ensure(w * d); h->v_scl.ensure(w * d); h->v_w.ensure(w);
     h->v_kind.ensure(w); h->v_key.ensure(w); h->v_next.ensure(w); h->v_upg.ensure(w); h->v_acc.ensure(w);
-    h->v_dsq.ensure(w); h->v_tau.ensure(CC_TAU_STRIDE * w); h->v_tile_dsq.ensure(CC_DSQ_STRIDE * (w / 16 + 2));
+    h->v_dsq.ensure(w); h->v_tau.ensure(CC_TAU_STRIDE * w); h->v_tile_dsq.ensure(cc_dsq_words(CC_MAX_WINDOW, CC_DSQ_STRIDE));
     h->v_tgt.ensure(w);
     h->v_skip.ensure(w / 64 + 2); h->v_skip_car.ensure(w / 64 + 2); h->v_unsafe.ensure(w);
     h->part_stride = w * seg * 4;
@@ -475,7 +475,7 @@
     h->clean.ensure(w * 4); h->dseed.ensure(w * 4);
     h->c_cf1v.ensure(w * d); h->c_cf2v.ensure(w * d); h->c_cenv.ensure(w * d); h->c_prefv.ensure(w * d);
     h->c_sclv.ensure(w * d); h->c_wv.ensure(w); h->c_c0.ensure(w * d); h->c_w0.ensure(w * d);
-    h->c_kind.ensure(w); h->c_key.ensure(w); h->c_slot.ensure(w); h->c_kind0.ensure(w); h->c_dsq.ensure(w); h->c_tile_dsq.ensure(CC_DSQ_STRIDE * (w / 16 + 2));
+    h->c_kind.ensure(w); h->c_key.ensure(w); h->c_slot.ensure(w); h->c_kind0.ensure(w); h->c_dsq.ensure(w); h->c_tile_dsq.ensure(cc_dsq_words(CC_MAX_WINDOW, CC_DSQ_STRIDE));
     h->T0.ensure(w + 128); h->T1.ensure(w + 128);
     h->long_list.ensure(2 * CC_LONG_CAP);
     h->lstat.ensure(2 * CC_LSTAT_ROWS + 2);
diff --git a/chronoclust_amd/csrc/cc_host.h b/chronoclust_amd/csrc/cc_host.h
--- a/chronoclust_amd/csrc/cc_host.h
+++ b/chronoclust_amd/csrc/cc_host.h
@@ -22,5 +22,17 @@
     *hi = (int)(b < n ? b : n);
 }
 
+#define CC_DSQ_COARSE_ROWS 1024
+CC_HOSTDEV constexpr int cc_dsq_coarse_at(int max_window, int stride) { return stride * (max_window / 16 + 2); }
+CC_HOSTDEV constexpr int cc_dsq_coarse_word(int max_window, int stride, int row, int cls)
+{
+    return cc_dsq_coarse_at(max_window, stride) + (row / CC_DSQ_COARSE_ROWS) * stride + cls;
+}
+CC_HOSTDEV constexpr int cc_dsq_coarse_records(int rows) { return (rows + CC_DSQ_COARSE_ROWS - 1) / CC_DSQ_COARSE_ROWS; }
+CC_HOSTDEV constexpr int cc_dsq_words(int max_window, int stride)
+{
+    return cc_dsq_coarse_at(max_window, stride) + stride * (cc_dsq_coarse_records(max_window) + 1);
+}
+
 #define CC_SEQ_DOUBLES 6600
 CC_HOSTDEV inline int cc_seq_cap_rows(int d) { return CC_SEQ_DOUBLES / (4 * d + 5); }
diff --git a/chronoclust_amd/csrc/cc_host_abi.inc b/chronoclust_amd/csrc/cc_host_abi.inc
--- a/chronoclust_amd/csrc/cc_host_abi.inc
+++ b/chronoclust_amd/csrc/cc_host_abi.inc
@@ -96,3 +96,16 @@
     *chain = w.chain;
     return CC_OK;
 }
+
+int cc_dsq_coarse_layout(int32_t rows, int32_t row, int32_t cls, int32_t* first_word, int32_t* word, int32_t* records,
+                         int32_t* buffer_words)
+{
+    if (rows < 1 || rows > cc::kMaxWindow || row < 0 || row >= rows || cls < 0 || cls > 2 || !first_word || !word || !records ||
+        !buffer_words)
+        return CC_ERR_BAD_ARG;
+    *first_word = cc_dsq_coarse_at(cc::kMaxWindow, cc::kDsqStride);
+    *word = cc_dsq_coarse_word(cc::kMaxWindow, cc::kDsqStride, row, cls);
+    *records = cc_dsq_coarse_records(rows);
+    *buffer_words = cc_dsq_words(cc::kMaxWindow, cc::kDsqStride);
+    return CC_OK;
+}
diff --git a/chronoclust_amd/csrc/cc_online_run.h b/chronoclust_amd/csrc/cc_online_run.h
--- a/chronoclust_amd/csrc/cc_online_run.h
+++ b/chronoclust_amd/csrc/cc_online_run.h
@@ -80,7 +80,8 @@
 #undef CC_LINK_DP
 }
 
-static_assert(cc::kMaxWindow == CC_MAX_WINDOW && cc::kLongCap == CC_LONG_CAP, "cc_batch.h repeats two constants of cc_common.h");
+static_assert(cc::kMaxWindow == CC_MAX_WINDOW && cc::kLongCap == CC_LONG_CAP && cc::kDsqStride == CC_DSQ_STRIDE,
+              "cc_batch.h repeats three constants of cc_common.h");
 
 Rows rows_of_table(const Table& t)
 {
@@ -548,7 +549,7 @@
 
     void launch_dseed(int round)
     {
-        hipLaunchKernelGGL(k_dseed, dim3((bp.gw + 63) / 64), dim3(64), 0, sA, h->ctl.p, h->X.p, tab, ver, car,
+        hipLaunchKernelGGL(k_dseed, dim3((bp.gw + 63) / 64), dim3(CC_DSEED_THREADS), 0, sA, h->ctl.p, h->X.p, tab, ver, car,
                            h->clean.p, h->dseed.p, (const int*)claims_of(round - 1), round, (const int8_t*)h->dpath.p, h->sp_list.p,
                            sparse_round() ? bp.sparse_cap : 0);
     }
diff --git a/chronoclust_amd/csrc/cc_validate.h b/chronoclust_amd/csrc/cc_validate.h
--- a/chronoclust_amd/csrc/cc_validate.h
+++ b/chronoclust_amd/csrc/cc_validate.h
@@ -1,5 +1,8 @@
 #pragma once
 
+
+#define CC_DSQ_COARSE_AT cc_dsq_coarse_at(CC_MAX_WINDOW, CC_DSQ_STRIDE)
+#define CC_DSQ_COARSE_WORD(row, cls) cc_dsq_coarse_word(CC_MAX_WINDOW, CC_DSQ_STRIDE, (row), (cls))
 
 #define CC_LSTAT_ROWS 1024
 
@@ -118,73 +121,90 @@
 }
 
 
-__device__ __forceinline__ void cc_dsq_window_max(const unsigned long long* __restrict__ tile_dsq, int n,
+__device__ __forceinline__ void cc_dsq_window_max(const unsigned long long* __restrict__ tile_dsq, int rows,
                                                   unsigned long long (&m)[3])
 {
     static_assert(CC_DSQ_STRIDE == 4, "a record is two 16-byte loads");
-    constexpr int AHEAD = 8;
-    const ulonglong2* const rec = reinterpret_cast<const ulonglong2*>(tile_dsq);
-    for (int i0 = threadIdx.x; i0 < n; i0 += 64 * AHEAD) {
-        ulonglong2 a[AHEAD], b[AHEAD];
-#pragma unroll
-        for (int q = 0; q < AHEAD; ++q) {
-            const int i = min(i0 + 64 * q, n - 1);
-            a[q] = rec[(size_t)i * 2];
-            b[q] = rec[(size_t)i * 2 + 1];
-        }
-#pragma unroll
-        for (int q = 0; q < AHEAD; ++q) {
-            m[0] = a[q].x > m[0] ? a[q].x : m[0];
-            m[1] = a[q].y > m[1] ? a[q].y : m[1];
-            m[2] = b[q].x > m[2] ? b[q].x : m[2];
-        }
+    static_assert(cc_dsq_coarse_records(CC_MAX_WINDOW) <= 64, "one coarse record per lane of a wave");
+    const int i = (int)(threadIdx.x & 63u);
+    if (i < cc_dsq_coarse_records(rows)) {
+        const ulonglong2* const rec = reinterpret_cast<const ulonglong2*>(tile_dsq + CC_DSQ_COARSE_AT) + (size_t)i * 2;
+        const ulonglong2 a = rec[0], b = rec[1];
+        m[0] = a.x; m[1] = a.y; m[2] = b.x;
     }
 }
 
-__global__ __launch_bounds__(64) void k_dseed(Ctl* __restrict__ ctl, const double* __restrict__ X, Table tab,
-                                              Versions ver, Carry car, const Cand* __restrict__ clean,
-                                              Cand* __restrict__ seed, const int* __restrict__ T, int round,
-                                              const int8_t* __restrict__ dpath, int* __restrict__ sparse_list, int sparse_cap)
+template <int CTRL>
+__device__ __forceinline__ unsigned long long cc_dpp_u64(unsigned long long x)
+{
+    int lo = (int)(unsigned)x, hi = (int)(unsigned)(x >> 32);
+    lo = __builtin_amdgcn_update_dpp(0, lo, CTRL, 0xF, 0xF, false);
+    hi = __builtin_amdgcn_update_dpp(0, hi, CTRL, 0xF, 0xF, false);
+    return ((unsigned long long)(unsigned)hi << 32) | (unsigned long long)(unsigned)lo;
+}
+__device__ __forceinline__ unsigned long long cc_wave_max_u64(unsigned long long x)
+{
+    cc_row16_exchanges([&](auto CT) {
+        constexpr int C = decltype(CT)::value;
+        const unsigned long long o = cc_dpp_u64<C>(x);
+        x = o > x ? o : x;
+    });
+    const int lo = (int)(unsigned)x, hi = (int)(unsigned)(x >> 32);
+    unsigned long long m = 0ull;
+#pragma unroll
+    for (int r = 0; r < 64; r += 16) {
+        const unsigned long long o = ((unsigned long long)(unsigned)__builtin_amdgcn_readlane(hi, r) << 32) |
+                                     (unsigned long long)(unsigned)__builtin_amdgcn_readlane(lo, r);
+        m = o > m ? o : m;
+    }
+    return m;
+}
+template <int K>
+__device__ __forceinline__ int cc_quad_bcast(int v) { return __builtin_amdgcn_update_dpp(0, v, K * 0x55, 0xF, 0xF, false); }
+template <int K>
+__device__ __forceinline__ double cc_quad_bcast(double v) { return cc_dpp_f64<K * 0x55>(v); }
+
+#define CC_DSEED_THREADS 256
+#define CC_DSEED_CHUNK 16
+
+__global__ __launch_bounds__(CC_DSEED_THREADS) void k_dseed(Ctl* __restrict__ ctl, const double* __restrict__ X, Table tab,
+                                                            Versions ver, Carry car, const Cand* __restrict__ clean,
+                                                            Cand* __restrict__ seed, const int* __restrict__ T, int round,
+                                                            const int8_t* __restrict__ dpath, int* __restrict__ sparse_list, int sparse_cap)
 {
     CC_LATENCY_KERNEL();
     const int B = ctl->win_b;
     if (B == 0) return;
     if (ctl->fc[round - 1] >= B) return;
-    const int j = blockIdx.x * blockDim.x + threadIdx.x;
-    if (blockIdx.x * blockDim.x >= B) return;
+    if ((int)blockIdx.x * (CC_DSEED_THREADS / 4) >= B) return;
+    const int lane = (int)(threadIdx.x & 63u);
+    const int q = (int)(threadIdx.x & 3u);
+    const int j = (int)blockIdx.x * (CC_DSEED_THREADS / 4) + (int)(threadIdx.x >> 2);
+    const bool live = j < B;
     const bool la_mode = ctl->mode != 0;
     unsigned long long maxd[3] = {0ull, 0ull, 0ull}, maxd_car[3] = {0ull, 0ull, 0ull};
     {
-        cc_dsq_window_max(ver.tile_dsq, (B + 15) / 16, maxd);
-        if (la_mode) cc_dsq_window_max(car.tile_dsq, (ctl->car_n + 15) / 16, maxd_car);
-#pragma unroll
-        for (int K = 0; K < 3; ++K)
-            for (int off = 32; off >= 1; off >>= 1) {
-                const unsigned long long o = __shfl_xor(maxd[K], off), oc = __shfl_xor(maxd_car[K], off);
-                maxd[K] = o > maxd[K] ? o : maxd[K];
-                maxd_car[K] = oc > maxd_car[K] ? oc : maxd_car[K];
-            }
-    }
-    bool flag_unprov = false, flag_unsafe = false, flag_n1skip = false;
-    bool repeats = false;
-    int flag_word = 0;
-    double tau_w[3] = {CC_INF, CC_INF, CC_INF};
-    bool need_ver = false, need_car = false;
-    if (j < B) {
+        cc_dsq_window_max(ver.tile_dsq, B, maxd);
+        if (la_mode) cc_dsq_window_max(car.tile_dsq, ctl->car_n, maxd_car);
+#pragma unroll
+        for (int K = 0; K < 3; ++K) {
+            maxd[K] = cc_wave_max_u64(maxd[K]);
+            if (la_mode) maxd_car[K] = cc_wave_max_u64(maxd_car[K]);
+        }
+    }
     const Par par = cc_load_par(ctl);
     const int d = par.d;
     const bool filter = par.filter != 0;
     const unsigned long long stamp = ctl->window_seq * 16ull + (unsigned long long)round;
-    const double* p = X + (ctl->cursor + j) * d;
+    const double* p = X + (ctl->cursor + (live ? j : 0)) * d;
     Cand first0 = Cand{CC_INF, CC_IDX_INF, -1}, first1 = Cand{CC_INF, CC_IDX_INF, -1};
     double cap[2] = {CC_INF, CC_INF};
     bool lk_ok[2] = {par.k > 0.0, par.k > 0.0}, lbound[2] = {false, false};
     const double K = 1.0;
 
     const unsigned long long wseq = ctl->window_seq;
-    Cand cq[4];
-#pragma unroll
-    for (int q = 0; q < 4; ++q) cq[q] = clean[(size_t)j * 4 + q];
+    const Cand cown = live ? clean[(size_t)j * 4 + q] : Cand{CC_INF, CC_IDX_INF, -1};
+    const Cand cq[4] = {cc_dpp_cand<0x00>(cown), cc_dpp_cand<0x55>(cown), cc_dpp_cand<0xAA>(cown), cc_dpp_cand<0xFF>(cown)};
     double d2v[2] = {CC_INF, CC_INF};
     bool have1[2];
     bool look[4];
@@ -197,162 +217,148 @@
         look[kd * 2] = have1[kd];
         look[kd * 2 + 1] = have1[kd] && cq[kd * 2 + 1].slot >= 0;
     }
-    unsigned long long tcq[4], cwq[4], coq[4];
-#pragma unroll
-    for (int q = 0; q < 4; ++q) {
-        const size_t sl = (size_t)(look[q] ? cq[q].slot : 0);
-        tcq[q] = look[q] ? tab.touch[(size_t)(round & 1) * tab.cap + sl] : 0ull;
-        cwq[q] = look[q] ? tab.cnt[sl] : 0ull;
-        coq[q] = (look[q] && la_mode) ? tab.carry_of[sl] : 0ull;
-    }
-    int lv[4], n_memb[4];
-    bool walk[4];
-    int max_list = 0;
-#pragma unroll
-    for (int q = 0; q < 4; ++q) {
-        const int head = 0xFFFFF - (int)(tcq[q] & 0xFFFFFull);
-        lv[q] = -1;
-        walk[q] = false;
-        n_memb[q] = 0;
-        if (!look[q]) continue;
-        if ((tcq[q] >> 20) != stamp || head >= j) {
-            if (la_mode && (coq[q] >> 20) == wseq) lv[q] = CC_CAR_BASE + (int)(coq[q] & 0xFFFFFull);
+    const bool lk = live && (q == 0 ? look[0] : q == 1 ? look[1] : q == 2 ? look[2] : look[3]);
+    const size_t sl = (size_t)(lk ? cown.slot : 0);
+    const unsigned long long tc = lk ? tab.touch[(size_t)(round & 1) * tab.cap + sl] : 0ull;
+    const unsigned long long cw = lk ? tab.cnt[sl] : 0ull;
+    const unsigned long long co = (lk && la_mode) ? tab.carry_of[sl] : 0ull;
+    int lv = -1, n_memb = 0;
+    bool walk = false;
+    if (lk) {
+        const int head = 0xFFFFF - (int)(tc & 0xFFFFFull);
+        if ((tc >> 20) != stamp || head >= j) {
+            if (la_mode && (co >> 20) == wseq) lv = CC_CAR_BASE + (int)(co & 0xFFFFFull);
         } else {
-            lv[q] = head;
-            walk[q] = true;
-            n_memb[q] = ((cwq[q] >> 24) == stamp) ? (int)(cwq[q] & 0xFFFFFFull) : 0;
-            const int n_list = n_memb[q] < CC_CHAIN_MEMB ? n_memb[q] : CC_CHAIN_MEMB;
-            max_list = n_list > max_list ? n_list : max_list;
-        }
-    }
-    for (int pos = 0; pos * 4 < max_list; ++pos) {
-        int4 mm[4];
-#pragma unroll
-        for (int q = 0; q < 4; ++q) {
-            const bool on = walk[q] && pos * 4 < n_memb[q];
-            mm[q] = on ? reinterpret_cast<const int4*>(tab.memb + (size_t)cq[q].slot * CC_CHAIN_MEMB)[pos] : make_int4(0, 0, 0, 0);
-        }
-#pragma unroll
-        for (int q = 0; q < 4; ++q) {
-            const int n_list = n_memb[q] < CC_CHAIN_MEMB ? n_memb[q] : CC_CHAIN_MEMB;
-            const int e[4] = {mm[q].x, mm[q].y, mm[q].z, mm[q].w};
-#pragma unroll
-            for (int c = 0; c < 4; ++c) {
-                const int m = e[c];
-                if (walk[q] && pos * 4 + c < n_list && m < j && m > lv[q]) lv[q] = m;
-            }
-        }
-    }
-#pragma unroll
-    for (int q = 0; q < 4; ++q)
-        if (walk[q] && n_memb[q] > CC_CHAIN_MEMB) {
-            const int clen = tab.clen[cq[q].slot];
-            const int n = clen > CC_CHAIN_MEMB ? clen : CC_CHAIN_MEMB + 1;
-            const int gap = B / n;
-            const bool scan_first = (n - CC_CHAIN_MEMB) > gap / 8;
-            int v = lv[q];
-            int res = -2;
-            for (int attempt = 0; attempt < 2 && res == -2; ++attempt) {
-                if ((attempt == 0) == scan_first) {
-                    const int want = cq[q].slot;
-                    const int budget = min(16384, 16 * gap + 64);
-                    for (int hi = j - 1, scanned = 0; res == -2 && scanned < budget; hi -= 32, scanned += 32) {
-                        int tv[32];
-#pragma unroll
-                        for (int c = 0; c < 32; ++c) tv[c] = (hi - c > v) ? T[hi - c] : CC_T_UNKNOWN;
-                        int hit = -1;
-#pragma unroll
-                        for (int c = 31; c >= 0; --c)
-                            if (tv[c] == want) hit = hi - c;
-                        if (hit < 0 && hi - 32 <= v) hit = v;
-                        if (hit >= 0) res = hit;
-                    }
-                } else {
-                    int w = v;
-                    for (int steps = 0; steps < 64; ++steps) {
-                        const int nxv = ver.next[w];
-                        if (nxv >= j) { res = w; break; }
-                        w = nxv;
-                    }
-                }
-            }
-            lv[q] = res;
-        }
+            lv = head;
+            walk = true;
+            n_memb = ((cw >> 24) == stamp) ? (int)(cw & 0xFFFFFFull) : 0;
+        }
+    }
+    {
+        const int n_list = n_memb < CC_CHAIN_MEMB ? n_memb : CC_CHAIN_MEMB;
+        const int4* const memb4 = reinterpret_cast<const int4*>(tab.memb + sl * CC_CHAIN_MEMB);
+        for (int pos0 = 0; pos0 * 4 < n_list; pos0 += 4) {
+            int4 mm[4];
+#pragma unroll
+            for (int u = 0; u < 4; ++u) mm[u] = ((pos0 + u) * 4 < n_list) ? memb4[pos0 + u] : make_int4(0, 0, 0, 0);
+#pragma unroll
+            for (int u = 0; u < 4; ++u) {
+                const int e[4] = {mm[u].x, mm[u].y, mm[u].z, mm[u].w};
+#pragma unroll
+                for (int c = 0; c < 4; ++c) {
+                    const int m = e[c];
+                    if ((pos0 + u) * 4 + c < n_list && m < j && m > lv) lv = m;
+                }
+            }
+        }
+    }
+    if (walk && n_memb > CC_CHAIN_MEMB) {
+        const int clen = tab.clen[sl];
+        const int n = clen > CC_CHAIN_MEMB ? clen : CC_CHAIN_MEMB + 1;
+        const int gap = B / n;
+        const bool scan_first = (n - CC_CHAIN_MEMB) > gap / 8;
+        const int v = lv;
+        int res = -2;
+        for (int attempt = 0; attempt < 2 && res == -2; ++attempt) {
+            if ((attempt == 0) == scan_first) {
+                const int want = cown.slot;
+                const int budget = min(16384, 16 * gap + 64);
+                for (int hi = j - 1, scanned = 0; res == -2 && scanned < budget; hi -= 32, scanned += 32) {
+                    int tv[32];
+#pragma unroll
+                    for (int c = 0; c < 32; ++c) tv[c] = (hi - c > v) ? T[hi - c] : CC_T_UNKNOWN;
+                    int hit = -1;
+#pragma unroll
+                    for (int c = 31; c >= 0; --c)
+                        if (tv[c] == want) hit = hi - c;
+                    if (hit < 0 && hi - 32 <= v) hit = v;
+                    if (hit >= 0) res = hit;
+                }
+            } else {
+                int w = v;
+                for (int steps = 0; steps < 64; ++steps) {
+                    const int nxv = ver.next[w];
+                    if (nxv >= j) { res = w; break; }
+                    w = nxv;
+                }
+            }
+        }
+        lv = res;
+    }
+    const int lvq[4] = {cc_quad_bcast<0>(lv), cc_quad_bcast<1>(lv), cc_quad_bcast<2>(lv), cc_quad_bcast<3>(lv)};
 #pragma unroll
     for (int kd = 0; kd < 2; ++kd) {
         if (!have1[kd]) continue;
-        const int v1 = lv[kd * 2];
+        const int v1 = lvq[kd * 2];
         if (v1 == -1) cap[kd] = cq[kd * 2].dist;
         else {
             cap[kd] = d2v[kd];
             if (v1 < 0) lk_ok[kd] = false;
         }
-        if (look[kd * 2 + 1] && lv[kd * 2 + 1] == -2) lk_ok[kd] = false;
-    }
-    bool sd[4];
-    int kvq[4], keyq[4];
-    const double* vcen[4];
-    const double* vpref[4];
-#pragma unroll
-    for (int q = 0; q < 4; ++q) {
-        sd[q] = look[q] && lv[q] >= 0;
-        const bool cr = sd[q] && lv[q] >= CC_CAR_BASE;
-        const size_t r = sd[q] ? (size_t)(cr ? lv[q] - CC_CAR_BASE : lv[q]) : 0;
-        kvq[q] = sd[q] ? (cr ? car.kind[r] : ver.kind[r]) : CC_KIND_DEAD;
-        keyq[q] = sd[q] ? (cr ? car.key[r] : ver.key[r]) : 0;
-        vcen[q] = (cr ? car.cen : ver.cen) + r * d;
-        vpref[q] = (cr ? car.pref : ver.pref) + r * d;
-    }
-#pragma unroll
-    for (int q = 0; q < 4; ++q) sd[q] = sd[q] && kvq[q] != CC_KIND_DEAD;
-    double accq[4] = {0.0, 0.0, 0.0, 0.0};
-    for (int i0 = 0; i0 < d; i0 += 4) {
-        double pv[4], cv[4][4], fv[4][4];
-#pragma unroll
-        for (int c = 0; c < 4; ++c) {
-            const int i = (i0 + c < d) ? i0 + c : d - 1;
-            pv[c] = p[i];
-#pragma unroll
-            for (int q = 0; q < 4; ++q) {
-                cv[q][c] = sd[q] ? vcen[q][i] : 0.0;
-                fv[q][c] = sd[q] ? vpref[q][i] : 1.0;
-            }
-        }
-#pragma unroll
-        for (int c = 0; c < 4; ++c) {
-            if (i0 + c < d) {
-#pragma unroll
-                for (int q = 0; q < 4; ++q) {
-                    double x = pv[c] - cv[q][c];
+        if (look[kd * 2 + 1] && lvq[kd * 2 + 1] == -2) lk_ok[kd] = false;
+    }
+    bool sd = lk && lv >= 0;
+    const bool cr = sd && lv >= CC_CAR_BASE;
+    const size_t r = sd ? (size_t)(cr ? lv - CC_CAR_BASE : lv) : 0;
+    const int kv = sd ? (cr ? car.kind[r] : ver.kind[r]) : CC_KIND_DEAD;
+    const int keyv = sd ? (cr ? car.key[r] : ver.key[r]) : 0;
+    sd = sd && kv != CC_KIND_DEAD;
+    double acc = 0.0;
+    if (sd) {
+        const double* const vcen = (cr ? car.cen : ver.cen) + r * d;
+        const double* const vpref = (cr ? car.pref : ver.pref) + r * d;
+        for (int i0 = 0; i0 < d; i0 += CC_DSEED_CHUNK) {
+            double pv[CC_DSEED_CHUNK], cv[CC_DSEED_CHUNK], fv[CC_DSEED_CHUNK];
+#pragma unroll
+            for (int c = 0; c < CC_DSEED_CHUNK; ++c) {
+                const int i = (i0 + c < d) ? i0 + c : d - 1;
+                pv[c] = p[i];
+                cv[c] = vcen[i];
+                fv[c] = vpref[i];
+            }
+#pragma unroll
+            for (int c = 0; c < CC_DSEED_CHUNK; ++c) {
+                if (i0 + c < d) {
+                    double x = pv[c] - cv[c];
                     x = x * x;
-                    accq[q] = accq[q] + cc_div_pref(x, fv[q][c], par);
-                }
-            }
-        }
-    }
-#pragma unroll
-    for (int q = 0; q < 4; ++q) {
-        if (!sd[q]) continue;
-        if (kvq[q] == 0 && filter) {
-            const bool cr = lv[q] >= CC_CAR_BASE;
-            const size_t r = (size_t)(cr ? lv[q] - CC_CAR_BASE : lv[q]);
+                    acc = acc + cc_div_pref(x, fv[c], par);
+                }
+            }
+        }
+        if (kv == 0 && filter) {
             int ne1 = 0;
-            cc_tentative_radius((cr ? car.cf1 : ver.cf1) + r * d, (cr ? car.cf2 : ver.cf2) + r * d,
-                                cr ? car.w[r] : ver.w[r], p, d, par, nullptr, &ne1);
-            if (ne1 > par.pi) continue;
-        }
-        if (kvq[q] == 0) {
-            if (cand_less(accq[q], keyq[q], first0.dist, first0.key)) first0 = Cand{accq[q], keyq[q], lv[q]};
-        } else {
-            if (cand_less(accq[q], keyq[q], first1.dist, first1.key)) first1 = Cand{accq[q], keyq[q], lv[q]};
-        }
-    }
-    seed[(size_t)j * 4 + 0] = first0;
-    seed[(size_t)j * 4 + 1] = Cand{cap[0], 0, 0};
-    seed[(size_t)j * 4 + 2] = first1;
-    seed[(size_t)j * 4 + 3] = Cand{cap[1], 0, 0};
+            cc_tentative_radius((cr ? car.cf1 : ver.cf1) + r * d, (cr ? car.cf2 : ver.cf2) + r * d, cr ? car.w[r] : ver.w[r], p, d,
+                                par, nullptr, &ne1);
+            if (ne1 > par.pi) sd = false;
+        }
+    }
+    {
+        const int sdi = sd ? 1 : 0;
+        auto fold = [&](auto QT) {
+            constexpr int Q = decltype(QT)::value;
+            const int on = cc_quad_bcast<Q>(sdi), kq = cc_quad_bcast<Q>(kv), keyq = cc_quad_bcast<Q>(keyv);
+            const double accq = cc_quad_bcast<Q>(acc);
+            const bool b0 = on != 0 && kq == 0 && cand_less(accq, keyq, first0.dist, first0.key);
+            const bool b1 = on != 0 && kq != 0 && cand_less(accq, keyq, first1.dist, first1.key);
+            first0.dist = b0 ? accq : first0.dist; first0.key = b0 ? keyq : first0.key; first0.slot = b0 ? lvq[Q] : first0.slot;
+            first1.dist = b1 ? accq : first1.dist; first1.key = b1 ? keyq : first1.key; first1.slot = b1 ? lvq[Q] : first1.slot;
+        };
+        fold(std::integral_constant<int, 0>{});
+        fold(std::integral_constant<int, 1>{});
+        fold(std::integral_constant<int, 2>{});
+        fold(std::integral_constant<int, 3>{});
+    }
+    if (live) {
+        const bool pc = q < 2, is_cap = (q & 1) != 0;
+        Cand out;
+        out.dist = is_cap ? (pc ? cap[0] : cap[1]) : (pc ? first0.dist : first1.dist);
+        out.key = is_cap ? 0 : (pc ? first0.key : first1.key);
+        out.slot = is_cap ? 0 : (pc ? first0.slot : first1.slot);
+        seed[(size_t)j * 4 + q] = out;
+    }
 
     double tau[3];
+#pragma unroll
     for (int kd = 0; kd < 3; ++kd) {
         double t;
         const int list = (kd == 1) ? 1 : 0;
@@ -368,27 +374,29 @@
         t = (t == CC_INF) ? CC_INF : t * (1.0 - 1e-9) - 1e-290;
         tau[kd] = t;
     }
+    const int tj = live ? T[j] : -1;
+    const int pj = live ? (int)dpath[j] : 0;
     const bool need0 = true;
-    const bool need1 = !(T[j] >= 0 && dpath[j] == 0);
+    const bool need1 = !(tj >= 0 && pj == 0);
     int flags = 0;
     if (!(cc_dsq_below(maxd[0], tau[0]) && cc_dsq_below(maxd[2], tau[2]))) flags |= CC_FLAG_U0;
     if (!cc_dsq_below(maxd[1], tau[1])) flags |= CC_FLAG_U1;
     if (la_mode && !(cc_dsq_below(maxd_car[0], tau[0]) && cc_dsq_below(maxd_car[2], tau[2]))) flags |= CC_FLAG_C0;
     if (la_mode && !cc_dsq_below(maxd_car[1], tau[1])) flags |= CC_FLAG_C1;
-    need_ver = (need0 && (flags & CC_FLAG_U0)) || (need1 && (flags & CC_FLAG_U1));
-    need_car = (need0 && (flags & CC_FLAG_C0)) || (need1 && (flags & CC_FLAG_C1));
-    flag_unprov = !(lk_ok[0] && lk_ok[1]);
-    flag_unsafe = need_ver || need_car;
-    flag_n1skip = !need1;
-    flag_word = flags;
-#pragma unroll
-    for (int kd = 0; kd < 3; ++kd) tau_w[kd] = tau[kd];
-    {
-        const int t = T[j];
+    const bool need_ver = live && ((need0 && (flags & CC_FLAG_U0)) || (need1 && (flags & CC_FLAG_U1)));
+    const bool need_car = live && ((need0 && (flags & CC_FLAG_C0)) || (need1 && (flags & CC_FLAG_C1)));
+    const bool rep = live && q == 0;
+    const bool flag_unprov = rep && !(lk_ok[0] && lk_ok[1]);
+    const bool flag_unsafe = rep && (need_ver || need_car);
+    bool flag_n1skip = !need1;
+    int flag_word = flags;
+    bool repeats = false;
+    if (rep) {
+        const int t = tj;
         const Cand c1 = cq[0], c2 = cq[1];
-        if (flags == 0 && t >= 0 && dpath[j] == 0 && c1.slot >= 0 && ver.tgt[j] == t && ver.acc[j] != 0) {
-            const int head0 = 0xFFFFF - (int)(tcq[0] & 0xFFFFFull);
-            const bool dirty0 = ((tcq[0] >> 20) == stamp && head0 < j) || (la_mode && (coq[0] >> 20) == wseq);
+        if (flags == 0 && t >= 0 && pj == 0 && c1.slot >= 0 && ver.tgt[j] == t && ver.acc[j] != 0) {
+            const int head0 = 0xFFFFF - (int)(tc & 0xFFFFFull);
+            const bool dirty0 = ((tc >> 20) == stamp && head0 < j) || (la_mode && (co >> 20) == wseq);
             if (!dirty0) {
                 repeats = c1.slot == t && !(first0.slot >= 0 && cand_less(first0.dist, first0.key, c1.dist, c1.key));
             } else if (first0.slot >= 0 && (c2.slot == -1 || cand_less(first0.dist, first0.key, c2.dist, c2.key))) {
@@ -397,14 +405,13 @@
             }
         }
     }
-    }
     if (sparse_cap > 0) {
         const unsigned long long m = __builtin_amdgcn_ballot_w64(flag_unsafe);
         if (m != 0ull) {
             int base = 0;
-            if (threadIdx.x == (unsigned)__builtin_ctzll(m)) base = atomicAdd(&ctl->n_sparse, __builtin_popcountll(m));
+            if (lane == __builtin_ctzll(m)) base = atomicAdd(&ctl->n_sparse, __builtin_popcountll(m));
             base = __shfl(base, __builtin_ctzll(m));
-            const int idx = base + __builtin_popcountll(m & ((1ull << threadIdx.x) - 1ull));
+            const int idx = base + __builtin_popcountll(m & ((1ull << lane) - 1ull));
             if (flag_unsafe && idx < sparse_cap) {
                 sparse_list[idx] = j;
                 flag_word |= CC_FLAG_SPARSE;
@@ -412,23 +419,22 @@
             }
         }
     }
-    const unsigned long long any_v = __builtin_amdgcn_ballot_w64(need_ver), any_c = __builtin_amdgcn_ballot_w64(need_car);
-    if (j < B) {
-        if (flag_n1skip && any_v == 0ull && any_c == 0ull) { tau_w[1] = CC_INF; flag_word |= CC_FLAG_N1SKIP; }
-#pragma unroll
-        for (int kd = 0; kd < 3; ++kd) ver.tau[(size_t)j * CC_TAU_STRIDE + kd] = tau_w[kd];
+    const bool any_v = __syncthreads_or(need_ver ? 1 : 0) != 0, any_c = __syncthreads_or(need_car ? 1 : 0) != 0;
+    if (rep) {
+        if (flag_n1skip && !any_v && !any_c) { tau[1] = CC_INF; flag_word |= CC_FLAG_N1SKIP; }
+#pragma unroll
+        for (int kd = 0; kd < 3; ++kd) ver.tau[(size_t)j * CC_TAU_STRIDE + kd] = tau[kd];
         ver.unsafe[j] = flag_word;
     }
-    if (__builtin_amdgcn_ballot_w64(j < B && !(repeats && any_v == 0ull && any_c == 0ull)) != 0ull && threadIdx.x == 0)
-        ctl->rdiff[round] = 1;
+    if (__builtin_amdgcn_ballot_w64(rep && !(repeats && !any_v && !any_c)) != 0ull && lane == 0) ctl->rdiff[round] = 1;
     {
         const unsigned long long b1 = __builtin_amdgcn_ballot_w64(flag_unprov), b2 = __builtin_amdgcn_ballot_w64(flag_unsafe);
-        if (threadIdx.x == 0 && b1) atomicAdd((unsigned long long*)&ctl->stat_unprovable, (unsigned long long)__builtin_popcountll(b1));
-        if (threadIdx.x == 0 && b2) atomicAdd((unsigned long long*)&ctl->stat_unsafe, (unsigned long long)__builtin_popcountll(b2));
+        if (lane == 0 && b1) atomicAdd((unsigned long long*)&ctl->stat_unprovable, (unsigned long long)__builtin_popcountll(b1));
+        if (lane == 0 && b2) atomicAdd((unsigned long long*)&ctl->stat_unsafe, (unsigned long long)__builtin_popcountll(b2));
     }
     if (threadIdx.x == 0) {
-        ver.skip[blockIdx.x] = any_v == 0ull ? 1 : 0;
-        ver.skip_car[blockIdx.x] = (!la_mode || any_c == 0ull) ? 1 : 0;
+        ver.skip[blockIdx.x] = !any_v ? 1 : 0;
+        ver.skip_car[blockIdx.x] = (!la_mode || !any_c) ? 1 : 0;
     }
 }
 
@@ -705,6 +711,11 @@
             ver.tile_dsq[(size_t)(j >> 4) * CC_DSQ_STRIDE] = 0ull;
             ver.tile_dsq[(size_t)(j >> 4) * CC_DSQ_STRIDE + 1] = 0ull;
             ver.tile_dsq[(size_t)(j >> 4) * CC_DSQ_STRIDE + 2] = 0ull;
+            if ((j & (CC_DSQ_COARSE_ROWS - 1)) == 0) {
+                ver.tile_dsq[CC_DSQ_COARSE_WORD(j, 0)] = 0ull;
+                ver.tile_dsq[CC_DSQ_COARSE_WORD(j, 1)] = 0ull;
+                ver.tile_dsq[CC_DSQ_COARSE_WORD(j, 2)] = 0ull;
+            }
         }
         if (last_round == 0 && T >= 0 && !(T < M0 && T < scan_rows) && !(heavy_on != 0 && T < M0 && tab.heavy[T] != 0) &&
             !(link_near != nullptr && T == M0 + j)) {
@@ -955,6 +966,7 @@
                 int cls;
                 ver.dsq[j] = cc_dsq_store(dq, bkind, kind0, &cls);
                 atomicMax(&ver.tile_dsq[(size_t)(j >> 4) * CC_DSQ_STRIDE + cls], cc_dsq_code(dq));
+                atomicMax(&ver.tile_dsq[CC_DSQ_COARSE_WORD(j, cls)], cc_dsq_code(dq));
             }
             return;
         }
@@ -1127,6 +1139,7 @@
                     int cls;
                     ver.dsq[cur] = cc_dsq_store(dq, bkind, isnew ? CC_KIND_DEAD : kind0, &cls);
                     atomicMax(&ver.tile_dsq[(size_t)(cur >> 4) * CC_DSQ_STRIDE + cls], cc_dsq_code(dq));
+                    atomicMax(&ver.tile_dsq[CC_DSQ_COARSE_WORD(cur, cls)], cc_dsq_code(dq));
                 }
             }
         }
@@ -1647,6 +1660,7 @@
             int cls;
             ver.dsq[m] = cc_dsq_store(dq, kind, kind0, &cls);
             atomicMax(&ver.tile_dsq[(size_t)(m >> 4) * CC_DSQ_STRIDE + cls], cc_dsq_code(dq));
+            atomicMax(&ver.tile_dsq[CC_DSQ_COARSE_WORD(m, cls)], cc_dsq_code(dq));
         }
         __syncthreads();
         CC_TICK(5);
@@ -1790,7 +1804,10 @@
     const bool la_ok = ctl->la_on != 0 && n == B && next_b > 0 && ctl->la_b[qn] == next_b &&
                        ctl->la_cursor[qn] == next_cursor;
     if (la_ok)
+    {
         for (int i = tid; i < CC_DSQ_STRIDE * ((B + 15) / 16 + 1); i += 1024) car.tile_dsq[i] = 0ull;
+        if (tid < CC_DSQ_STRIDE * (cc_dsq_coarse_records(B) + 1)) car.tile_dsq[CC_DSQ_COARSE_AT + tid] = 0ull;
+    }
     __shared__ double s_sum[2][16];
     __shared__ int s_cnt[2][16];
     {
@@ -1953,6 +1970,7 @@
                 int cls;
                 car.dsq[j] = cc_dsq_store(dq, kind, kind0, &cls);
                 atomicMax(&car.tile_dsq[(size_t)(j >> 4) * CC_DSQ_STRIDE + cls], cc_dsq_code(dq));
+                atomicMax(&car.tile_dsq[CC_DSQ_COARSE_WORD(j, cls)], cc_dsq_code(dq));
                 tab.carry_of[row] = (rec->next_seq << 20) | (unsigned long long)j;
             }
         }
diff --git a/include/chronoclust_hip.h b/include/chronoclust_hip.h
--- a/include/chronoclust_hip.h
+++ b/include/chronoclust_hip.h
@@ -277,6 +277,9 @@
 enum { CC_CHAIN_NONE = 0, CC_CHAIN_COMMON = 1, CC_CHAIN_GENERAL = 2 };
 int cc_scan_width(int32_t d, int32_t filter_on, int32_t k_pow2, int32_t* padded, int32_t* scan_u, int32_t* chain);
 
+int cc_dsq_coarse_layout(int32_t rows, int32_t row, int32_t cls, int32_t* first_word, int32_t* word, int32_t* records,
+                         int32_t* buffer_words);
+
 #ifdef __cplusplus
 }
 #endif
```

Measured after the change: 69.18 million points/s. 10.2% lower.
